# SCUT-CCNL/3DSIFT

Hardware: AMD Instinct MI355X
Metric: Mvoxels/s end-to-end KpSiftAlgorithm on 512^3 fp32 (higher is better)
Workload: dtype f32

## Files before the change

### 3dsift_amd/capi.py

```python
import ctypes as C
import os

import numpy as np

HERE = os.path.dirname(os.path.abspath(__file__))
LIB_PATH = os.environ.get("S3D_LIB") or os.path.join(HERE, "libsift3d_hip.so")
DESC = 768

KP_DTYPE = np.dtype(
    [
        ("x", "<f4"), ("y", "<f4"), ("z", "<f4"),
        ("scale", "<f4"),
        ("octave", "<i4"), ("level", "<i4"),
        ("rx", "<f4"), ("ry", "<f4"), ("rz", "<f4"),
        ("win", "<f4", (3,)),
        ("eigvalue", "<f4", (3,)),
        ("eigvector", "<f4", (9,)),
        ("Rotation", "<f4", (9,)),
        ("str_tensor", "<f4", (9,)),
    ]
)
assert KP_DTYPE.itemsize == 168

SYMBOLS = [
    "sift3d_default_params", "sift3d_create", "sift3d_destroy", "sift3d_run", "sift3d_run_async", "sift3d_run_async_after", "sift3d_wait", "sift3d_run_stages",
    "sift3d_stage_times", "sift3d_num_keypoints", "sift3d_get_keypoints", "sift3d_device_results",
    "sift3d_num_octaves", "sift3d_level_info", "sift3d_copy_level", "sift3d_copy_input", "sift3d_num_extrema",
    "sift3d_get_extrema", "sift3d_get_orientation_codes", "sift3d_gaussian_smooth", "sift3d_downsample", "sift3d_dog_sub", "sift3d_conv_axis",
    "sift3d_orient_keypoint", "sift3d_describe_keypoint", "sift3d_match",
    "sift3d_match_handles",
    "sift3d_default_detect_options", "sift3d_set_detect_options", "sift3d_get_detect_options", "sift3d_get_refined",
    "sift3d_default_ransac_options", "sift3d_fit_affine", "sift3d_fit_affine_local",
    "sift3d_fit_rigid", "sift3d_fit_rigid_local", "sift3d_fit_rotation",
    "sift3d_predict_positions", "sift3d_match_guided",
    "sift3d_default_icgn_options", "sift3d_icgn_init_from_fits", "sift3d_icgn",
    "sift3d_bspline_prefilter", "sift3d_icgn_bspline",
    "sift3d_icgn2_init_from_icgn", "sift3d_icgn2", "sift3d_strain_input_from_icgn2",
    "sift3d_default_search_options", "sift3d_zncc_search", "sift3d_icgn_init_from_search",
    "sift3d_default_strain_options", "sift3d_strain_input_from_icgn", "sift3d_strain",
    "sift3d_default_validate_options", "sift3d_validate_input_from_icgn", "sift3d_validate_input_from_icgn2", "sift3d_validate_displacements",
    "sift3d_validate_keep", "sift3d_icgn_init_from_validation", "sift3d_validate_stage_capacity",
    "sift3d_default_subset_options", "sift3d_subset_quality", "sift3d_subset_group_by_radius",
    "sift3d_icgn_masked", "sift3d_mask_from_level",
    "sift3d_device_count", "sift3d_error_string", "sift3d_last_error",
    "sift3d_dtype_bytes", "sift3d_create_typed", "sift3d_volume_to_device", "sift3d_test_ingest_launch",
    "sift3d_slab_min_halo", "sift3d_slab_arena_floats", "sift3d_slab_create", "sift3d_slab_buffer", "sift3d_slab_upload",
    "sift3d_slab_input_absmax", "sift3d_slab_input_scale", "sift3d_slab_level", "sift3d_slab_level_hw", "sift3d_slab_halo_planes",
    "sift3d_slab_sync", "sift3d_slab_get_dogmax", "sift3d_slab_set_dogmax", "sift3d_slab_detect", "sift3d_slab_describe",
    "sift3d_slab_decimate", "sift3d_slab_admits", "sift3d_slab_set_ghost", "sift3d_slab_min_halo_ghost", "sift3d_create_seeded", "sift3d_seed_upload", "sift3d_set_describe_partition",
    "sift3d_export_device", "sift3d_import_descriptors_device", "sift3d_run_partial_orientation",
    "sift3d_export_orientation_device", "sift3d_import_orientation_device", "sift3d_run_describe",
    "sift3d_set_stream", "sift3d_slab_export_dogmax_device", "sift3d_slab_import_dogmax_device", "sift3d_slab_decimate_async",
    "sift3d_slab_set_desc_partial", "sift3d_slab_min_halo_partial", "sift3d_slab_record_bytes", "sift3d_slab_desc_reach", "sift3d_slab_orient",
    "sift3d_slab_export_records", "sift3d_slab_describe_partial", "sift3d_slab_describe_finish", "sift3d_slab_orient_launch",
    "sift3d_slab_orient_count",
    "sift3d_slab_keypoints_launch", "sift3d_slab_keypoints_count", "sift3d_slab_describe_finish_launch", "sift3d_slab_describe_finish_count",
    "sift3d_seed_buffer", "sift3d_sharded_plan", "sift3d_slab_describe_launch", "sift3d_sharded_traffic",
    "sift3d_sharded_create", "sift3d_sharded_create_ex", "sift3d_sharded_run", "sift3d_sharded_num_keypoints", "sift3d_sharded_get_keypoints", "sift3d_sharded_info",
    "sift3d_sharded_error", "sift3d_sharded_destroy",
    "sift3d_test_hook", "sift3d_debug_counters", "sift3d_debug_face_lookup", "sift3d_match_times", "sift3d_debug_copy_bandwidth",
    "sift3d_match_warmup", "sift3d_test_staging_slice", "sift3d_test_slab_plan", "sift3d_test_sharded_time_rank",
]
HOOKS = {"dog_eager": 0, "glast_eager": 1, "det_serial": 2, "separable": 3, "desc_nocache": 4, "match_nodma": 5, "one_stream": 6,
         "desc_mass_shift": 7, "list_cap": 8, "peer_copy": 9, "desc_nosplit": 10, "march_tiles": 11, "desc_exact_cells": 12, "lazy_generic": 13, "sharded_fail_rank": 14,
         "ori_grid": 15}
ORIENT_WORDS = 34
DTYPES = {"float32": 0, "uint8": 1, "int8": 2, "uint16": 3, "int16": 4}
SHARDED_PARTIAL_WINDOWS = 1
SHARDED_WHOLE_WINDOWS = 2
SHARDED_COPY_TRANSPORT = 4
SHARDED_GHOST_OCTAVE0 = 8


class Params(C.Structure):
    _fields_ = [("num_kp_levels", C.c_int), ("sigma_default", C.c_float), ("sigma_n_default", C.c_float),
                ("peak_thresh", C.c_float), ("max_eig_thres", C.c_float), ("corner_thresh", C.c_float)]


class DetectOptions(C.Structure):
    _fields_ = [("neighbours", C.c_int), ("refine", C.c_int), ("max_offset", C.c_float), ("contrast_thresh", C.c_float),
                ("edge_ratio", C.c_float), ("reserved", C.c_int * 3)]


assert C.sizeof(DetectOptions) == 32

REFINED_DTYPE = np.dtype([("rx", "<f4"), ("ry", "<f4"), ("rz", "<f4"), ("scale", "<f4"), ("offset", "<f4", (4,)), ("contrast", "<f4")])
assert REFINED_DTYPE.itemsize == 36


class RansacOptions(C.Structure):
    _fields_ = [("iterations", C.c_int), ("inlier_thresh", C.c_float), ("seed", C.c_uint), ("refine", C.c_int), ("min_det", C.c_float),
                ("reserved", C.c_int * 3)]


assert C.sizeof(RansacOptions) == 32

FIT_DTYPE = np.dtype([("A", "<f8", (12,)), ("hyp", "<f8", (12,)), ("status", "<i4"), ("candidates", "<i4"), ("best_hypothesis", "<i4"),
                      ("best_count", "<i4"), ("inliers", "<i4"), ("rms", "<f4"), ("reserved", "<i4", (2,))])
assert FIT_DTYPE.itemsize == 224


class IcgnOptions(C.Structure):
    _fields_ = [("subset_radius", C.c_int), ("max_iterations", C.c_int), ("tolerance", C.c_float), ("interpolation", C.c_int),
                ("reserved", C.c_int * 4)]


assert C.sizeof(IcgnOptions) == 32

ICGN_DTYPE = np.dtype([("p", "<f8", (12,)), ("zncc", "<f8"), ("last_step", "<f8"), ("iterations", "<i4"), ("status", "<i4"),
                       ("reserved", "<i4", (2,))])
assert ICGN_DTYPE.itemsize == 128
ICGN2_DTYPE = np.dtype([("p", "<f8", (30,)), ("zncc", "<f8"), ("last_step", "<f8"), ("iterations", "<i4"), ("status", "<i4"),
                        ("reserved", "<i4", (2,))])
assert ICGN2_DTYPE.itemsize == 272


class SearchOptions(C.Structure):
    _fields_ = [("subset_radius", C.c_int), ("search_radius", C.c_int), ("reserved", C.c_int * 6)]


assert C.sizeof(SearchOptions) == 32

SEARCH_DTYPE = np.dtype([("d", "<i4", (3,)), ("status", "<i4"), ("zncc", "<f8"), ("zncc_second", "<f8"), ("candidates", "<i4"),
                         ("reserved", "<i4", (3,))])
assert SEARCH_DTYPE.itemsize == 48


class StrainOptions(C.Structure):
    _fields_ = [("radius", C.c_int), ("min_neighbours", C.c_int), ("measure", C.c_int), ("reserved", C.c_int * 5)]


assert C.sizeof(StrainOptions) == 32

STRAIN_DTYPE = np.dtype([("disp", "<f8", (3,)), ("G", "<f8", (9,)), ("E", "<f8", (6,)), ("principal", "<f8", (3,)), ("equivalent", "<f8"),
                         ("rms", "<f8"), ("neighbours", "<i4"), ("status", "<i4")])
assert STRAIN_DTYPE.itemsize == 192


class ValidateOptions(C.Structure):
    _fields_ = [("radius", C.c_int), ("min_neighbours", C.c_int), ("passes", C.c_int), ("reserved0", C.c_int), ("threshold", C.c_double),
                ("eps", C.c_double), ("reserved", C.c_int * 4)]


assert C.sizeof(ValidateOptions) == 48

VALIDATE_DTYPE = np.dtype([("median", "<f8", (3,)), ("mad", "<f8", (3,)), ("score", "<f8"), ("neighbours", "<i4"), ("status", "<i4"),
                           ("flagged", "<i4"), ("pass", "<i4")])
assert VALIDATE_DTYPE.itemsize == 72


class SubsetOptions(C.Structure):
    _fields_ = [("r_min", C.c_int), ("r_max", C.c_int), ("criterion", C.c_int), ("reserved0", C.c_int), ("threshold", C.c_double),
                ("level", C.c_double), ("fraction_min", C.c_double), ("reserved", C.c_int * 2)]


assert C.sizeof(SubsetOptions) == 48

SUBSET_DTYPE = np.dtype([("mean", "<f8"), ("dR", "<f8"), ("G", "<f8", (6,)), ("eig", "<f8", (3,)), ("radius", "<i4"), ("status", "<i4"),
                         ("feasible", "<i4"), ("material", "<i4")])
assert SUBSET_DTYPE.itemsize == 104


class SlabDesc(C.Structure):
    _fields_ = [("nx", C.c_int), ("ny", C.c_int), ("nz", C.c_int), ("z0", C.c_int), ("z1", C.c_int), ("halo", C.c_int),
                ("noct_total", C.c_int), ("octave", C.c_int)]


class Sift3dError(RuntimeError):
    pass


_lib = None
_fp = C.POINTER(C.c_float)
_ip = C.POINTER(C.c_int)


def lib():
    global _lib
    if _lib is None:
        if not os.path.exists(LIB_PATH):
            raise Sift3dError(f"{LIB_PATH} is missing: build it with `make -C 3dsift_amd/csrc` "
                              f"(or __graft_entry__.build()); there is no CPU fallback")
        try:
            import torch
        except ImportError:
            pass
        L = C.CDLL(LIB_PATH)
        L.sift3d_create.argtypes = [C.POINTER(C.c_void_p), C.c_void_p, C.c_int, C.c_int, C.c_int, C.POINTER(Params), C.c_int, C.c_int]
        L.sift3d_create_typed.argtypes = [C.POINTER(C.c_void_p), C.c_void_p, C.c_int, C.c_int, C.c_int, C.c_int, C.POINTER(Params), C.c_int, C.c_int]
        L.sift3d_dtype_bytes.argtypes = [C.c_int, _ip]
        L.sift3d_volume_to_device.argtypes = [C.c_void_p, C.c_int, C.c_int, C.c_int, C.c_int, C.c_int, C.c_int, C.c_void_p, C.POINTER(C.c_double)]
        L.sift3d_test_ingest_launch.argtypes = [C.c_int, _ip, _ip, _ip, _ip]
        L.sift3d_destroy.argtypes = [C.c_void_p]
        L.sift3d_run.argtypes = [C.c_void_p]
        L.sift3d_run_async.argtypes = [C.c_void_p]
        L.sift3d_wait.argtypes = [C.c_void_p]
        L.sift3d_run_stages.argtypes = [C.c_void_p, C.c_int]
        L.sift3d_stage_times.argtypes = [C.c_void_p, C.POINTER(C.c_double)]
        L.sift3d_num_keypoints.argtypes = [C.c_void_p, _ip]
        L.sift3d_get_keypoints.argtypes = [C.c_void_p, C.c_void_p, _fp]
        L.sift3d_device_results.argtypes = [C.c_void_p, C.POINTER(C.c_void_p), C.POINTER(C.c_void_p), _ip]
        L.sift3d_num_octaves.argtypes = [C.c_void_p, _ip]
        L.sift3d_level_info.argtypes = [C.c_void_p, C.c_int, C.c_int, _ip, _fp, _fp]
        L.sift3d_copy_level.argtypes = [C.c_void_p, C.c_int, C.c_int, _fp]
        L.sift3d_copy_input.argtypes = [C.c_void_p, _fp]
        L.sift3d_num_extrema.argtypes = [C.c_void_p, _ip]
        L.sift3d_get_extrema.argtypes = [C.c_void_p, C.c_void_p]
        L.sift3d_get_orientation_codes.argtypes = [C.c_void_p, _ip]
        L.sift3d_gaussian_smooth.argtypes = [_fp, C.c_int, C.c_int, C.c_int, C.c_float, _fp, C.c_int]
        L.sift3d_downsample.argtypes = [_fp, C.c_int, C.c_int, C.c_int, _fp, C.c_int, C.c_int, C.c_int, C.c_int]
        L.sift3d_dog_sub.argtypes = [_fp, _fp, C.c_size_t, _fp, C.c_int]
        L.sift3d_conv_axis.argtypes = [_fp, C.c_int, C.c_int, C.c_int, C.c_int, _fp, C.c_int, _fp, C.c_int]
        L.sift3d_orient_keypoint.argtypes = [_fp, C.c_int, C.c_int, C.c_int, C.c_float, C.c_void_p, C.c_float, C.c_float, C.c_float, C.c_int, _ip]
        L.sift3d_describe_keypoint.argtypes = [_fp, C.c_int, C.c_int, C.c_int, C.c_float, C.c_void_p, _fp, C.c_int]
        L.sift3d_match.argtypes = [C.c_void_p, C.c_void_p, C.c_int, C.c_void_p, C.c_void_p, C.c_int, C.c_double, C.c_int,
                                   C.c_int, C.c_int, _ip, _ip, _fp, _fp, _fp, _ip, C.POINTER(C.c_double)]
        L.sift3d_match_handles.argtypes = [C.c_void_p, C.c_void_p, C.c_double, C.c_int, _ip, _ip, _fp, _fp, _fp, _ip, C.POINTER(C.c_double)]
        L.sift3d_device_count.argtypes = [_ip]
        L.sift3d_default_detect_options.argtypes = [C.POINTER(DetectOptions)]
        L.sift3d_default_detect_options.restype = None
        L.sift3d_set_detect_options.argtypes = [C.c_void_p, C.POINTER(DetectOptions)]
        L.sift3d_get_detect_options.argtypes = [C.c_void_p, C.POINTER(DetectOptions)]
        L.sift3d_get_refined.argtypes = [C.c_void_p, C.c_void_p]
        L.sift3d_default_ransac_options.argtypes = [C.POINTER(RansacOptions)]
        L.sift3d_default_ransac_options.restype = None
        L.sift3d_fit_affine.argtypes = [C.c_void_p, C.c_int, C.POINTER(RansacOptions), C.c_int, C.c_int, C.c_void_p, C.c_void_p,
                                        C.POINTER(C.c_double)]
        L.sift3d_fit_affine_local.argtypes = [C.c_void_p, C.c_int, C.c_void_p, C.c_int, C.c_int, C.c_float, C.POINTER(RansacOptions), C.c_int,
                                              C.c_int, C.c_void_p, C.c_void_p, C.POINTER(C.c_double)]
        L.sift3d_fit_rigid.argtypes = [C.c_void_p, C.c_int, C.c_int, C.POINTER(RansacOptions), C.c_int, C.c_int, C.c_void_p, C.c_void_p,
                                       C.POINTER(C.c_double)]
        L.sift3d_fit_rigid_local.argtypes = [C.c_void_p, C.c_int, C.c_void_p, C.c_int, C.c_int, C.c_float, C.c_int, C.POINTER(RansacOptions),
                                             C.c_int, C.c_int, C.c_void_p, C.c_void_p, C.POINTER(C.c_double)]
        L.sift3d_fit_rotation.argtypes = [C.c_void_p, C.c_int, C.c_void_p, C.c_void_p, C.c_void_p]
        L.sift3d_predict_positions.argtypes = [C.c_void_p, C.c_int, C.c_void_p, C.c_int, C.c_void_p]
        L.sift3d_match_guided.argtypes = [C.c_void_p, C.c_void_p, C.c_int, C.c_void_p, C.c_void_p, C.c_int, C.c_void_p, C.c_float, C.c_double,
                                          C.c_int, C.c_int, C.c_int, _ip, _ip, _fp, _fp, _ip, _fp, _ip, C.POINTER(C.c_double)]
        L.sift3d_default_icgn_options.argtypes = [C.POINTER(IcgnOptions)]
        L.sift3d_default_icgn_options.restype = None
        L.sift3d_icgn_init_from_fits.argtypes = [C.c_void_p, C.c_void_p, C.c_int, C.c_void_p]
        L.sift3d_icgn.argtypes = [C.c_void_p, C.c_int, C.c_int, C.c_int, C.c_void_p, C.c_int, C.c_int, C.c_int, C.c_void_p, C.c_int, C.c_void_p,
                                  C.POINTER(IcgnOptions), C.c_int, C.c_int, C.c_void_p, C.POINTER(C.c_double)]
        L.sift3d_bspline_prefilter.argtypes = [C.c_void_p, C.c_int, C.c_int, C.c_int, C.c_void_p, C.c_int, C.c_int, C.POINTER(C.c_double)]
        L.sift3d_icgn_bspline.argtypes = [C.c_void_p, C.c_int, C.c_int, C.c_int, C.c_void_p, C.c_int, C.c_int, C.c_int, C.c_void_p, C.c_int,
                                          C.c_void_p, C.POINTER(IcgnOptions), C.c_int, C.c_int, C.c_int, C.c_void_p, C.POINTER(C.c_double)]
        L.sift3d_default_search_options.argtypes = [C.POINTER(SearchOptions)]
        L.sift3d_default_search_options.restype = None
        L.sift3d_zncc_search.argtypes = [C.c_void_p, C.c_int, C.c_int, C.c_int, C.c_void_p, C.c_int, C.c_int, C.c_int, C.c_void_p, C.c_int,
                                         C.c_void_p, C.POINTER(SearchOptions), C.c_int, C.c_int, C.c_void_p, C.POINTER(C.c_double)]
        L.sift3d_icgn2_init_from_icgn.argtypes = [C.c_void_p, C.c_int, C.c_void_p]
        L.sift3d_icgn2.argtypes = [C.c_void_p, C.c_int, C.c_int, C.c_int, C.c_void_p, C.c_int, C.c_int, C.c_int, C.c_void_p, C.c_int, C.c_void_p,
                                   C.POINTER(IcgnOptions), C.c_int, C.c_int, C.c_int, C.c_void_p, C.POINTER(C.c_double)]
        L.sift3d_strain_input_from_icgn2.argtypes = [C.c_void_p, C.c_int, C.c_double, C.c_int, C.c_void_p, C.c_void_p]
        L.sift3d_icgn_init_from_search.argtypes = [C.c_void_p, C.c_int, C.c_int, C.c_void_p]
        L.sift3d_default_strain_options.argtypes = [C.POINTER(StrainOptions)]
        L.sift3d_default_strain_options.restype = None
        L.sift3d_strain_input_from_icgn.argtypes = [C.c_void_p, C.c_int, C.c_double, C.c_int, C.c_void_p, C.c_void_p]
        L.sift3d_strain.argtypes = [C.c_void_p, C.c_void_p, C.c_void_p, C.c_int, C.POINTER(StrainOptions), C.c_int, C.c_int, C.c_void_p,
                                    C.POINTER(C.c_double)]
        L.sift3d_default_validate_options.argtypes = [C.POINTER(ValidateOptions)]
        L.sift3d_default_validate_options.restype = None
        L.sift3d_validate_input_from_icgn.argtypes = [C.c_void_p, C.c_int, C.c_double, C.c_int, C.c_void_p, C.c_void_p, C.c_void_p]
        L.sift3d_validate_input_from_icgn2.argtypes = [C.c_void_p, C.c_int, C.c_double, C.c_int, C.c_void_p, C.c_void_p, C.c_void_p]
        L.sift3d_validate_displacements.argtypes = [C.c_void_p, C.c_void_p, C.c_void_p, C.c_void_p, C.c_int, C.POINTER(ValidateOptions), C.c_int,
                                                    C.c_int, C.c_void_p, C.POINTER(C.c_double)]
        L.sift3d_validate_keep.argtypes = [C.c_void_p, C.c_void_p, C.c_int, C.c_void_p]
        L.sift3d_default_subset_options.argtypes = [C.POINTER(SubsetOptions)]
        L.sift3d_default_subset_options.restype = None
        L.sift3d_subset_quality.argtypes = [C.c_void_p, C.c_int, C.c_int, C.c_int, C.c_void_p, C.c_int, C.POINTER(SubsetOptions), C.c_int,
                                            C.c_int, C.c_void_p, C.POINTER(C.c_double)]
        L.sift3d_subset_group_by_radius.argtypes = [C.c_void_p, C.c_int, C.c_int, C.c_int, C.c_void_p, C.c_void_p, C.POINTER(C.c_int)]
        L.sift3d_icgn_init_from_validation.argtypes = [C.c_void_p, C.c_int, C.c_void_p, _ip]
        L.sift3d_icgn_masked.argtypes = [C.c_void_p, C.c_int, C.c_int, C.c_int, C.c_void_p, C.c_int, C.c_int, C.c_int, C.c_void_p, C.c_void_p,
                                         C.c_int, C.c_void_p, C.POINTER(IcgnOptions), C.c_float, C.c_int, C.c_int, C.c_int, C.c_void_p,
                                         C.c_void_p, C.POINTER(C.c_double)]
        L.sift3d_mask_from_level.argtypes = [C.c_void_p, C.c_int, C.c_int, C.c_int, C.c_double, C.c_void_p, C.c_int, C.c_int,
                                             C.POINTER(C.c_double)]
        L.sift3d_validate_stage_capacity.argtypes = [_ip]
        _sz = C.POINTER(C.c_size_t)
        L.sift3d_slab_min_halo.argtypes = [C.POINTER(Params), _ip]
        L.sift3d_slab_arena_floats.argtypes = [C.POINTER(SlabDesc), C.POINTER(Params), _sz]
        L.sift3d_slab_create.argtypes = [C.POINTER(C.c_void_p), C.POINTER(SlabDesc), C.POINTER(Params), C.c_int, C.c_void_p, C.c_size_t]
        L.sift3d_slab_buffer.argtypes = [C.c_void_p, C.c_int, C.c_int, _sz, _ip, _ip]
        L.sift3d_slab_upload.argtypes = [C.c_void_p, C.c_void_p, C.c_int, C.c_int, C.c_int]
        L.sift3d_slab_input_absmax.argtypes = [C.c_void_p, _fp]
        L.sift3d_slab_input_scale.argtypes = [C.c_void_p, C.c_float]
        L.sift3d_slab_level.argtypes = [C.c_void_p, C.c_int]
        L.sift3d_slab_halo_planes.argtypes = [C.c_void_p, C.c_int, _ip]
        L.sift3d_slab_level_hw.argtypes = [C.c_void_p, C.c_int, _ip]
        L.sift3d_slab_sync.argtypes = [C.c_void_p]
        L.sift3d_slab_get_dogmax.argtypes = [C.c_void_p, _fp]
        L.sift3d_slab_set_dogmax.argtypes = [C.c_void_p, _fp]
        L.sift3d_slab_detect.argtypes = [C.c_void_p]
        L.sift3d_slab_describe.argtypes = [C.c_void_p]
        L.sift3d_slab_set_desc_partial.argtypes = [C.c_void_p, C.c_int]
        L.sift3d_slab_min_halo_partial.argtypes = [C.POINTER(Params), _ip]
        L.sift3d_slab_record_bytes.argtypes = [_ip]
        L.sift3d_slab_desc_reach.argtypes = [C.c_void_p, _ip]
        L.sift3d_slab_orient.argtypes = [C.c_void_p]
        L.sift3d_slab_export_records.argtypes = [C.c_void_p, C.c_void_p]
        L.sift3d_slab_describe_partial.argtypes = [C.c_void_p, C.c_int, C.POINTER(C.c_void_p), _ip, C.POINTER(C.c_void_p), C.POINTER(C.c_void_p),
                                                   C.POINTER(C.c_void_p), _ip, _ip]
        L.sift3d_slab_describe_finish.argtypes = [C.c_void_p, C.c_void_p, C.c_int, C.c_int, C.POINTER(C.c_void_p), C.POINTER(C.c_void_p), C.c_void_p,
                                                  C.c_int, C.c_void_p, C.c_void_p, _ip]
        L.sift3d_slab_orient_launch.argtypes = [C.c_void_p]
        L.sift3d_slab_orient_count.argtypes = [C.c_void_p, _ip]
        L.sift3d_slab_decimate.argtypes = [C.c_void_p, C.c_void_p]
        L.sift3d_slab_decimate_async.argtypes = [C.c_void_p, C.c_void_p]
        L.sift3d_set_stream.argtypes = [C.c_void_p, C.c_void_p]
        L.sift3d_slab_export_dogmax_device.argtypes = [C.c_void_p, C.c_void_p]
        L.sift3d_slab_import_dogmax_device.argtypes = [C.c_void_p, C.c_void_p]
        L.sift3d_create_seeded.argtypes = [C.POINTER(C.c_void_p), C.c_int, C.c_int, C.c_int, C.c_int, C.c_int, C.POINTER(Params), C.c_int]
        L.sift3d_seed_upload.argtypes = [C.c_void_p, C.c_void_p, C.c_int]
        L.sift3d_set_describe_partition.argtypes = [C.c_void_p, C.c_int, C.c_int]
        L.sift3d_export_device.argtypes = [C.c_void_p, C.c_void_p, C.c_void_p]
        L.sift3d_run_partial_orientation.argtypes = [C.c_void_p]
        L.sift3d_export_orientation_device.argtypes = [C.c_void_p, C.c_void_p]
        L.sift3d_import_orientation_device.argtypes = [C.c_void_p, C.c_void_p]
        L.sift3d_run_describe.argtypes = [C.c_void_p]
        L.sift3d_import_descriptors_device.argtypes = [C.c_void_p, C.c_void_p]
        L.sift3d_sharded_create.argtypes = [C.POINTER(C.c_void_p), C.c_void_p, C.c_int, C.c_int, C.c_int, C.POINTER(Params), _ip, C.c_int, C.c_int, C.c_int]
        L.sift3d_sharded_create_ex.argtypes = [C.POINTER(C.c_void_p), C.c_void_p, C.c_int, C.c_int, C.c_int, C.POINTER(Params), _ip, C.c_int, C.c_int, C.c_int, C.c_uint]
        L.sift3d_sharded_run.argtypes = [C.c_void_p]
        L.sift3d_sharded_num_keypoints.argtypes = [C.c_void_p, _ip]
        L.sift3d_sharded_get_keypoints.argtypes = [C.c_void_p, C.c_void_p, _fp]
        L.sift3d_sharded_info.argtypes = [C.c_void_p, _ip, _ip, _ip, C.POINTER(C.c_double)]
        L.sift3d_sharded_error.argtypes = [C.c_void_p]
        L.sift3d_sharded_error.restype = C.c_char_p
        L.sift3d_sharded_destroy.argtypes = [C.c_void_p]
        L.sift3d_sharded_plan.argtypes = [C.c_void_p, _ip, _ip, _ip, _ip]
        L.sift3d_test_hook.argtypes = [C.c_int, C.c_int]
        L.sift3d_debug_counters.argtypes = [C.c_void_p, _ip]
        L.sift3d_debug_face_lookup.argtypes = [_fp, C.c_int, C.c_int, _ip, _fp, C.c_int]
        L.sift3d_debug_copy_bandwidth.argtypes = [C.c_size_t, C.c_int, C.c_int, C.POINTER(C.c_double)]
        L.sift3d_match_times.argtypes = [C.POINTER(C.c_double), C.POINTER(C.c_double)]
        L.sift3d_error_string.argtypes = [C.c_int]
        L.sift3d_error_string.restype = C.c_char_p
        L.sift3d_last_error.restype = C.c_char_p
        _lib = L
        for item in filter(None, os.environ.get("S3D_HOOKS", "").split(",")):
            k, _, v = item.partition("=")
            L.sift3d_test_hook(HOOKS[k.strip()], int(v or 1))
    return _lib


def _check(rc):
    if rc != 0:
        L = lib()
        raise Sift3dError(f"{L.sift3d_error_string(rc).decode()}: {L.sift3d_last_error().decode()}")


def _f(a):
    return a.ctypes.data_as(_fp)


def kernel_source_sha():
    import glob
    import hashlib
    h = hashlib.sha256()
    root = os.path.dirname(os.path.dirname(os.path.abspath(__file__)))
    files = sorted(glob.glob(os.path.join(root, "3dsift_amd", "csrc", "*.hip")) + glob.glob(os.path.join(root, "3dsift_amd", "csrc", "*.h")) +
                   glob.glob(os.path.join(root, "include", "*.h")))
    for f in files:
        h.update(os.path.basename(f).encode())
        h.update(open(f, "rb").read())
    return h.hexdigest()[:16]


class hook:

    def __init__(self, name, value):
        self.which, self.value = HOOKS[name], int(value)

    def __enter__(self):
        self.prev = lib().sift3d_test_hook(self.which, self.value)
        return self

    def __exit__(self, *exc):
        lib().sift3d_test_hook(self.which, self.prev)
        return False


def copy_bandwidth(nbytes=1 << 30, iters=5, device=0):
    g = C.c_double(0)
    _check(lib().sift3d_debug_copy_bandwidth(nbytes, iters, device, C.byref(g)))
    return g.value


def face_lookup(grad3, route=0, device=0):
    g = np.ascontiguousarray(grad3, np.float32).reshape(-1, 3)
    face = np.zeros(len(g), np.int32); bary = np.zeros((len(g), 3), np.float32)
    _check(lib().sift3d_debug_face_lookup(_f(g), len(g), int(route), face.ctypes.data_as(_ip), _f(bary), device))
    return face, bary


def default_detect_options():
    o = DetectOptions()
    lib().sift3d_default_detect_options(C.byref(o))
    return _options_dict(o)


def _options_dict(o):
    return {"neighbours": o.neighbours, "refine": bool(o.refine), "max_offset": o.max_offset, "contrast_thresh": o.contrast_thresh,
            "edge_ratio": o.edge_ratio}


def _options(cls, default_fn_name, names, what, opts):
    o = cls()
    getattr(lib(), default_fn_name)(C.byref(o))
    for k, v in opts.items():
        if k not in names:
            raise TypeError(f"unknown {what} option {k!r}")
        setattr(o, k, v)
    return o


RANSAC_OPTIONS = ("iterations", "inlier_thresh", "seed", "refine", "min_det")


def default_ransac_options():
    o = _ransac_options({})
    return {k: getattr(o, k) for k in RANSAC_OPTIONS}


def _ransac_options(opts):
    return _options(RansacOptions, "sift3d_default_ransac_options", RANSAC_OPTIONS, "RANSAC", opts)


def _is_dev(a):
    return hasattr(a, "data_ptr") and getattr(a, "is_cuda", False)


def _p(a):
    return C.c_void_p(a.ctypes.data)


def _table(a, dtype, width, like):
    if a is None:
        return None, 0, None
    shape = (-1, width) if width else (-1,)
    if _is_dev(like):
        import torch

        t = torch.as_tensor(a, dtype=getattr(torch, np.dtype(dtype).name), device=like.device).reshape(shape).contiguous()
        return C.c_void_p(t.data_ptr()), t.shape[0], t
    h = np.ascontiguousarray(a, dtype).reshape(shape)
    return _p(h), len(h), h


def _rows(a, width, name):
    if _is_dev(a):
        if str(a.dtype) != "torch.float32" or not a.is_contiguous() or (a.numel() and a.shape[-1] != width):
            raise ValueError(f"{name}: a contiguous float32 (n, {width}) device tensor is needed")
        return C.c_void_p(a.data_ptr()), a.numel() // width, a, 1
    h = np.ascontiguousarray(a, np.float32).reshape(-1, width)
    return _p(h), len(h), h, 0


def _volume(a, name, on_dev):
    if on_dev:
        if str(a.dtype) != "torch.float32" or not a.is_contiguous() or a.dim() != 3:
            raise ValueError(f"{name}: a contiguous float32 (nz, ny, nx) device tensor is needed")
        return C.c_void_p(a.data_ptr()), a
    h = np.ascontiguousarray(a, np.float32)
    if h.ndim != 3:
        raise ValueError(f"{name}: a (nz, ny, nx) volume is needed")
    return _p(h), h


def _dtype_code(dtype):
    if isinstance(dtype, (int, np.integer)):
        return int(dtype)
    name = str(dtype).replace("torch.", "")
    try:
        name = np.dtype(name).name
    except TypeError:
        pass
    if name not in DTYPES:
        raise ValueError(f"dtype {dtype}: one of {sorted(DTYPES)} is needed")
    return DTYPES[name]


def ingest_launch(dtype):
    v = [C.c_int(0) for _ in range(4)]
    _check(lib().sift3d_test_ingest_launch(_dtype_code(dtype), *[C.byref(x) for x in v]))
# ... 520 lines not shown

    def __init__(self, volume, num_kp_levels=3, sigma_default=1.6, sigma_n_default=1.15, peak_thresh=0.1,
                 max_eig_thres=0.9, corner_thresh=0.4, device=0, device_ptr=None, shape=None, keep_dtype=False, dtype=None):
        L = lib()
        self._h = C.c_void_p()
        p = Params(num_kp_levels, sigma_default, sigma_n_default, peak_thresh, max_eig_thres, corner_thresh)
        self.levels = num_kp_levels
        if device_ptr is not None:
            nz, ny, nx = shape
            self.shape = tuple(shape)
            if dtype is not None:
                _check(L.sift3d_create_typed(C.byref(self._h), C.c_void_p(device_ptr), _dtype_code(dtype), nx, ny, nz, C.byref(p), device, 1))
            else:
                _check(L.sift3d_create(C.byref(self._h), C.c_void_p(device_ptr), nx, ny, nz, C.byref(p), device, 1))
        elif keep_dtype and isinstance(volume, np.ndarray) and volume.dtype.name in DTYPES:
            vol = np.ascontiguousarray(volume)
            nz, ny, nx = vol.shape
            self.shape = vol.shape
            _check(L.sift3d_create_typed(C.byref(self._h), vol.ctypes.data_as(C.c_void_p), DTYPES[vol.dtype.name], nx, ny, nz, C.byref(p), device, 0))
        else:
            vol = np.ascontiguousarray(volume, dtype=np.float32)
            nz, ny, nx = vol.shape
            self.shape = vol.shape
            _check(L.sift3d_create(C.byref(self._h), vol.ctypes.data_as(C.c_void_p), nx, ny, nz, C.byref(p), device, 0))

    def set_stream(self, stream_handle):
        _check(lib().sift3d_set_stream(self._h, C.c_void_p(int(stream_handle or 0))))

    def close(self):
        if getattr(self, "_h", None) and self._h.value:
            lib().sift3d_destroy(self._h)
            self._h = C.c_void_p()

    def __del__(self):
        try:
            self.close()
        except Exception:
            pass

    def KpSiftAlgorithm(self):
        _check(lib().sift3d_run(self._h))
        return self

    def KpSiftAlgorithmAsync(self, after=None):
        if after is not None:
            _check(lib().sift3d_run_async_after(self._h, after._h))
        else:
            _check(lib().sift3d_run_async(self._h))
        return self

    def Wait(self):
        _check(lib().sift3d_wait(self._h))
        return self

    def run_stages(self, upto):
        _check(lib().sift3d_run_stages(self._h, int(upto)))
        return self

    def GetKeypoints(self, with_desc=True, out=None):
        n = C.c_int(0)
        _check(lib().sift3d_num_keypoints(self._h, C.byref(n)))
        if out is not None:
            kp, desc = out
            assert kp.dtype == KP_DTYPE and kp.shape == (n.value,) and desc.dtype == np.float32 and desc.shape == (n.value, DESC)
            assert kp.flags.c_contiguous and desc.flags.c_contiguous
        else:
            kp = np.zeros(n.value, KP_DTYPE)
            desc = np.zeros((n.value, DESC), np.float32)
        if n.value:
            _check(lib().sift3d_get_keypoints(self._h, kp.ctypes.data, _f(desc) if with_desc else None))
        return kp, desc

    @property
    def m_timer(self):
        t = (C.c_double * 8)()
        _check(lib().sift3d_stage_times(self._h, t))
        keys = ["d_TotalTime", "d_Allocation", "d_BuildGSS", "d_BuildDOG", "d_Detect", "d_AssignOrientation", "d_Extraction", "d_release"]
        return dict(zip(keys, list(t)))

    @property
    def num_octaves(self):
        n = C.c_int(0)
        _check(lib().sift3d_num_octaves(self._h, C.byref(n)))
        return n.value

    def level_info(self, is_dog, idx):
        d = np.zeros(3, np.int32); u = np.zeros(3, np.float32); s = np.zeros(1, np.float32)
        _check(lib().sift3d_level_info(self._h, int(is_dog), idx, d.ctypes.data_as(_ip), _f(u), _f(s)))
        return tuple(int(v) for v in d), tuple(float(v) for v in u), float(s[0])

    def level(self, is_dog, idx):
        (nx, ny, nz), _, _ = self.level_info(is_dog, idx)
        out = np.empty((nz, ny, nx), np.float32)
        _check(lib().sift3d_copy_level(self._h, int(is_dog), idx, _f(out)))
        return out

    def gss(self, octave, i):
        return self.level(0, octave * (self.levels + 3) + i)

    def dog(self, octave, i):
        return self.level(1, octave * (self.levels + 2) + i)

    def input(self):
        out = np.empty(self.shape, np.float32)
        _check(lib().sift3d_copy_input(self._h, _f(out)))
        return out

    def extrema(self):
        n = C.c_int(0)
        _check(lib().sift3d_num_extrema(self._h, C.byref(n)))
        out = np.zeros(n.value, KP_DTYPE)
        if n.value:
            _check(lib().sift3d_get_extrema(self._h, out.ctypes.data))
        return out

    def orientation_codes(self):
        n = C.c_int(0)
        _check(lib().sift3d_num_extrema(self._h, C.byref(n)))
        out = np.zeros(n.value, np.int32)
        if n.value:
            _check(lib().sift3d_get_orientation_codes(self._h, out.ctypes.data_as(_ip)))
        return out

    def device_results(self):
        d = C.c_void_p(); x = C.c_void_p(); n = C.c_int(0)
        _check(lib().sift3d_device_results(self._h, C.byref(d), C.byref(x), C.byref(n)))
        return d.value, x.value, n.value

    def export_device(self, desc_ptr, xyz_ptr=None):
        _check(lib().sift3d_export_device(self._h, C.c_void_p(int(desc_ptr)), C.c_void_p(int(xyz_ptr)) if xyz_ptr else None))

    def set_detect_options(self, neighbours=8, refine=False, max_offset=0.5, contrast_thresh=0.0, edge_ratio=0.0):
        o = DetectOptions(int(neighbours), int(refine), float(max_offset), float(contrast_thresh), float(edge_ratio))
        _check(lib().sift3d_set_detect_options(self._h, C.byref(o)))
        return self

    def detect_options(self):
        o = DetectOptions()
        _check(lib().sift3d_get_detect_options(self._h, C.byref(o)))
        return _options_dict(o)

    def refined(self):
        n = C.c_int(0)
        _check(lib().sift3d_num_keypoints(self._h, C.byref(n)))
        out = np.zeros(max(n.value, 1), REFINED_DTYPE)
        _check(lib().sift3d_get_refined(self._h, out.ctypes.data))
        return out[:n.value]

    def debug_counters(self):
        a = (C.c_int * 4)()
        _check(lib().sift3d_debug_counters(self._h, a))
        return {"list_regrows": a[0], "desc_second_passes": a[1], "match_exact_rows": a[2]}


def _params(kw):
    return Params(kw.get("num_kp_levels", 3), kw.get("sigma_default", 1.6), kw.get("sigma_n_default", 1.15),
                  kw.get("peak_thresh", 0.1), kw.get("max_eig_thres", 0.9), kw.get("corner_thresh", 0.4))


def slab_min_halo(**kw):
    p = _params(kw); h = C.c_int(0)
    _check(lib().sift3d_slab_min_halo(C.byref(p), C.byref(h)))
    return h.value


def slab_admits(nx, ny, nz, first_octave=True, **kw):
    p = _params(kw); ok = C.c_int(0)
    lib().sift3d_slab_admits.argtypes = [C.POINTER(Params), C.c_int, C.c_int, C.c_int, C.c_int, C.POINTER(C.c_int)]
    _check(lib().sift3d_slab_admits(C.byref(p), int(nx), int(ny), int(nz), int(bool(first_octave)), C.byref(ok)))
    return bool(ok.value)


def slab_min_halo_partial(**kw):
    p = _params(kw); h = C.c_int(0)
    _check(lib().sift3d_slab_min_halo_partial(C.byref(p), C.byref(h)))
    return h.value


def slab_record_words():
    n = C.c_int(0)
    _check(lib().sift3d_slab_record_bytes(C.byref(n)))
    assert n.value % 4 == 0
    return n.value // 4


class SeededCSIFT3D(CSIFT3D):

    def __init__(self, shape, octave_base, noct_total, device=0, **kw):
        self._h = C.c_void_p()
        p = _params(kw)
        self.levels = p.num_kp_levels
        self.shape = tuple(shape)
        nz, ny, nx = shape
        _check(lib().sift3d_create_seeded(C.byref(self._h), nx, ny, nz, octave_base, noct_total, C.byref(p), device))

    def seed(self, ptr, on_device=True):
        _check(lib().sift3d_seed_upload(self._h, C.c_void_p(int(ptr)), int(bool(on_device))))

    def seed_host(self, vol):
        vol = np.ascontiguousarray(vol, np.float32)
        _check(lib().sift3d_seed_upload(self._h, vol.ctypes.data_as(C.c_void_p), 0))

    def set_partition(self, rank, world):
        _check(lib().sift3d_set_describe_partition(self._h, rank, world))

    def run_partial_orientation(self):
        _check(lib().sift3d_run_partial_orientation(self._h))

    def export_orientation(self, ptr):
        _check(lib().sift3d_export_orientation_device(self._h, C.c_void_p(int(ptr))))

    def import_orientation(self, ptr):
        _check(lib().sift3d_import_orientation_device(self._h, C.c_void_p(int(ptr))))

    def run_describe(self):
        _check(lib().sift3d_run_describe(self._h))

    def num_extrema(self):
        n = C.c_int(0)
        _check(lib().sift3d_num_extrema(self._h, C.byref(n)))
        return n.value

    def import_descriptors(self, desc_ptr):
        _check(lib().sift3d_import_descriptors_device(self._h, C.c_void_p(int(desc_ptr))))


class SlabCSIFT3D(CSIFT3D):

    @staticmethod
    def arena_floats(nx, ny, nz, z0, z1, halo, noct_total, octave=0, **kw):
        d = SlabDesc(nx, ny, nz, z0, z1, halo, noct_total, octave); p = _params(kw); n = C.c_size_t(0)
        _check(lib().sift3d_slab_arena_floats(C.byref(d), C.byref(p), C.byref(n)))
        return n.value

    def __init__(self, nx, ny, nz, z0, z1, halo, noct_total, arena_ptr, arena_floats, device=0, octave=0, **kw):
        self._h = C.c_void_p()
        p = _params(kw)
        self.levels = p.num_kp_levels
        self.dims = (nx, ny, nz)
        self.z0, self.z1, self.halo = z0, z1, halo
        self.shape = (z1 - z0 + 2 * halo, ny, nx)
        self.octave = octave
        d = SlabDesc(nx, ny, nz, z0, z1, halo, noct_total, octave)
        _check(lib().sift3d_slab_create(C.byref(self._h), C.byref(d), C.byref(p), device, C.c_void_p(int(arena_ptr)), arena_floats))

    def buffer(self, kind, idx=0):
        off = C.c_size_t(0); pl = C.c_int(0); zo = C.c_int(0)
        _check(lib().sift3d_slab_buffer(self._h, kind, idx, C.byref(off), C.byref(pl), C.byref(zo)))
        return off.value, pl.value, zo.value

    def held_level(self, is_dog, idx):
        out = np.empty(self.shape, np.float32)
        _check(lib().sift3d_copy_level(self._h, int(is_dog), idx, _f(out)))
        return out

    def upload(self, planes, zg0, zg1, device_ptr=None):
        if device_ptr is not None:
            _check(lib().sift3d_slab_upload(self._h, C.c_void_p(int(device_ptr)), zg0, zg1, 1))
        else:
            a = np.ascontiguousarray(planes, np.float32)
            assert a.shape == (zg1 - zg0, self.dims[1], self.dims[0])
            _check(lib().sift3d_slab_upload(self._h, a.ctypes.data_as(C.c_void_p), zg0, zg1, 0))

    def input_absmax(self):
        m = C.c_float(0)
        _check(lib().sift3d_slab_input_absmax(self._h, C.byref(m)))
        return m.value

    def input_scale(self, gmax):
        _check(lib().sift3d_slab_input_scale(self._h, C.c_float(gmax)))

    def level_async(self, i):
        _check(lib().sift3d_slab_level(self._h, i))

    def level_hw(self, i):
        n = C.c_int(0)
        _check(lib().sift3d_slab_level_hw(self._h, i, C.byref(n)))
        return n.value

    def halo_planes(self, i):
        n = C.c_int(0)
        _check(lib().sift3d_slab_halo_planes(self._h, i, C.byref(n)))
        return n.value

    def sync(self):
        _check(lib().sift3d_slab_sync(self._h))

    def get_dogmax(self):
        a = np.zeros(8, np.float32)
        _check(lib().sift3d_slab_get_dogmax(self._h, _f(a)))
        return a[: self.levels + 2].copy()

    def set_dogmax(self, a):
        b = np.zeros(8, np.float32); b[: self.levels + 2] = a
        _check(lib().sift3d_slab_set_dogmax(self._h, _f(b)))

    def detect(self):
        _check(lib().sift3d_slab_detect(self._h))

    def describe(self):
        _check(lib().sift3d_slab_describe(self._h))

    def set_desc_partial(self, on=True):
        _check(lib().sift3d_slab_set_desc_partial(self._h, int(bool(on))))

    def desc_reach(self):
# ... 260 lines not shown
```

### 3dsift_amd/csrc/context.hip

```cpp
#include <float.h>
#include <math.h>
#include <stdlib.h>
#include <string.h>

#include <algorithm>
#include <atomic>
#include <mutex>
#include <thread>

#include "ctx_internal.h"

#pragma clang fp contract(off)

namespace s3d {

static thread_local std::string g_last_error;
void set_last_error(const std::string &s) { g_last_error = s; }

int set_device(int device) {
	int n = 0;
	if (hipGetDeviceCount(&n) != hipSuccess || n <= 0) {
		set_last_error("no HIP device visible: this library has no CPU fallback");
		return SIFT3D_ERR_NO_DEVICE;
	}
// ... 285 lines not shown
		}
		CHECKED(hipEventCreateWithFlags(&c->ev_seed[o], hipEventDisableTiming));
		CHECKED(hipEventCreateWithFlags(&c->ev_done[o], hipEventDisableTiming));
	}

	const size_t total = arena_floats_of(c);
	c->arena_floats = total;
	if (cfg.ext_arena) {
		if (cfg.ext_arena_floats < total) { set_last_error("caller arena too small"); sift3d_destroy(c); return SIFT3D_ERR_ARG; }
		c->arena = cfg.ext_arena;
		c->ext_arena = true;
	} else {
		CHECKED(hipMalloc(&c->arena, sizeof(float) * total));
	}
	float *p = c->arena;
	if (c->in_own) c->in.d = c->in_own;
	else { c->in.d = p; p += al64(c->in.n()); }
	c->tmpA.assign((size_t)std::max(1, c->noct), nullptr);
	c->tmpB.assign((size_t)std::max(1, c->noct), nullptr);
	for (int o = 0; o < c->noct && !c->slab; o++) {
		const size_t vo = al64(c->gss[(size_t)o * c->ng].n());
		c->tmpA[o] = p; p += vo;
		c->tmpB[o] = p; p += vo;
	}
	for (auto &L : c->gss) { L.d = p; p += al64(L.n()); }
	for (auto &L : c->dog) { L.d = p; p += al64(L.n()); }

	const size_t nwords = 1 + (size_t)std::max(1, c->noct * c->nd) + 8 + 1;
	CHECKED(hipMalloc(&c->d_words, sizeof(unsigned) * nwords));
	CHECKED(hipMemset(c->d_words, 0, sizeof(unsigned) * nwords));
	CHECKED(hipHostMalloc(&c->h_words, sizeof(unsigned) * 8, hipHostMallocDefault));
	CHECKED(hipMalloc(&c->d_slots_part, sizeof(unsigned) * slots_scratch_words()));
	c->d_inmax = c->d_words;
	c->d_dogmax = c->d_words + 1;
	c->d_total = c->d_words + 1 + std::max(1, c->noct * c->nd);
	c->d_nkp = c->d_total + 2;

	const int scan_planes = c->slab ? (c->own1 - c->own0) : cfg.nz;
	{
		const size_t kl = (size_t)c->p.num_kp_levels;
		const size_t words = kl * (size_t)scan_planes * cfg.ny * ((cfg.nx + 63) / 64);
		c->det_blocks = kl * (size_t)scan_planes * ((cfg.ny + 15) / 16);
		CHECKED(hipMalloc(&c->det.masks, sizeof(unsigned long long) * std::max<size_t>(words, 1)));
		CHECKED(hipMalloc(&c->det.block_counts, sizeof(unsigned) * std::max<size_t>(c->det_blocks, 1)));
		CHECKED(hipMalloc(&c->det.block_offsets, sizeof(unsigned) * std::max<size_t>(c->det_blocks, 1)));
	}
	c->det.total = c->d_total;
	{
		const bool det_serial = hook(SIFT3D_HOOK_DET_SERIAL) != 0;
		if (!c->slab && c->noct > 1 && !det_serial && c->ostream.size() > 1 && c->ostream[1] != c->stream) {
			const size_t kl = (size_t)c->p.num_kp_levels;
			c->det_o.assign((size_t)c->noct, DetectBufs{});
			size_t words = 0, blocks = 0;
			std::vector<size_t> woff((size_t)c->noct, 0), boff((size_t)c->noct, 0);
			for (int o = 1; o < c->noct; o++) {
				const Level &D = c->dog[(size_t)o * c->nd + 1];
				woff[(size_t)o] = words; boff[(size_t)o] = blocks;
				words += kl * (size_t)D.nz * D.ny * ((D.nx + 63) / 64);
				blocks += kl * (size_t)D.nz * ((D.ny + 15) / 16);
			}
			CHECKED(hipMalloc(&c->d_masks2, sizeof(unsigned long long) * std::max<size_t>(words, 1)));
			CHECKED(hipMalloc(&c->d_counts2, sizeof(unsigned) * std::max<size_t>(blocks, 1)));
			CHECKED(hipMalloc(&c->d_offsets2, sizeof(unsigned) * std::max<size_t>(blocks, 1)));
			for (int o = 1; o < c->noct; o++) {
				DetectBufs &b = c->det_o[(size_t)o];
				b.masks = c->d_masks2 + woff[(size_t)o]; b.block_counts = c->d_counts2 + boff[(size_t)o];
				b.block_offsets = c->d_offsets2 + boff[(size_t)o]; b.total = c->d_total;
			}
			CHECKED(hipEventCreateWithFlags(&c->ev_det_fork, hipEventDisableTiming));
			CHECKED(hipEventCreateWithFlags(&c->ev_det_join, hipEventDisableTiming));
			CHECKED(hipEventCreateWithFlags(&c->ev_det_fork2, hipEventDisableTiming));
			CHECKED(hipEventCreateWithFlags(&c->ev_det_join2, hipEventDisableTiming));
		}
	}

	std::vector<LevelRef> lr((size_t)std::max(1, c->noct + c->octave_base) * 8, LevelRef{nullptr, 0, 0, 0, 1.f, 0});
	for (int o = 0; o < c->noct; o++)
		for (int i = 0; i < c->ng && i < 8; i++) {
			const Level &L = c->gss[(size_t)o * c->ng + i];
			lr[(size_t)(o + c->octave_base) * 8 + i] = LevelRef{L.d, L.nx, L.ny, L.nz, L.unit, L.zoff};
		}
	CHECKED(hipMalloc(&c->d_levels, sizeof(LevelRef) * lr.size()));
	CHECKED(hipMemcpy(c->d_levels, lr.data(), sizeof(LevelRef) * lr.size(), hipMemcpyHostToDevice));
	rc = build_luts(c);
	if (rc) { sift3d_destroy(c); return rc; }
	FaceConst faces[kFaces];
	build_faces(faces);
	FaceSym sym;
	if (!build_facesym(faces, &sym)) { set_last_error("icosahedron symmetry table: no matching face"); sift3d_destroy(c); return SIFT3D_ERR_STATE; }
	CHECKED(upload_faces(faces, &sym));

	const size_t V0 = (size_t)cfg.nx * cfg.ny * scan_planes;
	unsigned cap = (unsigned)std::min<size_t>(std::max<size_t>(4096, V0 / 256), 4u << 20);
	if (hook(SIFT3D_HOOK_LIST_CAP) > 0) cap = (unsigned)hook(SIFT3D_HOOK_LIST_CAP);
	rc = alloc_lists(c, cap);
	if (rc) { sift3d_destroy(c); return rc; }
	CHECKED(hipStreamSynchronize(c->stream));
#undef CHECKED
	{
		static std::atomic<unsigned long long> loaded{0};
		const unsigned long long bit = 1ull << (device & 63);
		if (!(loaded.fetch_or(bit) & bit)) { preload_march_kernels(); preload_small_kernels(); preload_detect_kernels(); preload_orient_kernels(); preload_desc_kernels(); preload_match_kernels(); preload_ingest_kernels(); }
	}
	*out = c;
	return SIFT3D_OK;
}

int join_upload(sift3d_ctx *c) {
	if (c->uploader.joinable()) c->uploader.join();
	if (c->upload_rc != SIFT3D_OK) { set_last_error(c->upload_err); return c->upload_rc; }
	S3D_HIP(hipStreamSynchronize(c->up_stream));
	return SIFT3D_OK;
}

extern "C" int sift3d_create(sift3d_handle *out, const float *volume, int nx, int ny, int nz, const sift3d_params *params,
                             int device, int volume_on_device) {
	if (!out || !volume || nx <= 0 || ny <= 0 || nz <= 0) { set_last_error("sift3d_create: bad argument"); return SIFT3D_ERR_ARG; }
	if ((size_t)nx * ny * nz >= ((size_t)1 << 31)) { set_last_error("volume too large for int32 voxel indices"); return SIFT3D_ERR_ARG; }
	CreateCfg cfg;
	cfg.nx = nx; cfg.ny = ny; cfg.nz = nz;
	if (!volume_on_device) cfg.host_volume = volume;
	int rc = create_common(out, cfg, params, device);
	if (rc) return rc;
	sift3d_ctx *c = *out;
	const size_t V0 = (size_t)nx * ny * nz;
	hipError_t e = hipSuccess;
	if (volume_on_device) e = hipMemcpyAsync(c->in.d, volume, sizeof(float) * V0, hipMemcpyDeviceToDevice, c->stream);
	else if ((rc = join_upload(c)) != SIFT3D_OK) { sift3d_destroy(c); *out = nullptr; return rc; }
	if (e == hipSuccess) {
		unsigned *d_nonfinite = c->d_words + 1 + (size_t)std::max(1, c->noct * c->nd) + 8;
		launch_absmax(c->in.d, V0, c->d_inmax, c->stream, d_nonfinite);
		launch_scale_by_max(c->in.d, V0, c->d_inmax, c->stream);
		e = hipMemcpyAsync(&c->h_words[7], d_nonfinite, sizeof(unsigned), hipMemcpyDeviceToHost, c->stream);
		if (e == hipSuccess) e = hipStreamSynchronize(c->stream);
		if (e == hipSuccess && c->h_words[7] != 0) { c->nonfinite = true; c->use_fused = false; }
	}
	if (e == hipSuccess) e = hipGetLastError();
	if (e != hipSuccess) { set_last_error(hipGetErrorString(e)); sift3d_destroy(c); *out = nullptr; return SIFT3D_ERR_HIP; }
	return SIFT3D_OK;
}

#ifndef S3D_FUSED_MIN_DEFAULT
#define S3D_FUSED_MIN_DEFAULT 33
#endif
#ifndef S3D_FUSED_HALF
#define S3D_FUSED_HALF 1
#endif
#ifndef S3D_O0_TAIL_SLOTS_DEFAULT
#define S3D_O0_TAIL_SLOTS_DEFAULT 512
#endif
#ifndef S3D_BG_SLOTS_DEFAULT
#define S3D_BG_SLOTS_DEFAULT 256
#endif
static bool smooth_level(sift3d_ctx *c, int o, const float *src, const Level &dst, const Taps &t, const float *prev, float *dog,
                         unsigned *dogmax, int level = 0, const Level *half_out = nullptr, hipStream_t st_override = nullptr) {
	hipStream_t st = st_override ? st_override : c->ostream[o];
	static const int tail_slots = dev_tune_i("S3D_O0_TAIL_SLOTS", S3D_O0_TAIL_SLOTS_DEFAULT);
	static const int bg_slots = dev_tune_i("S3D_BG_SLOTS", S3D_BG_SLOTS_DEFAULT);
	static const int prio_mode = dev_tune_i("S3D_PRIO", 3);
	static const int bg1_slots = dev_tune_i("S3D_BG1_SLOTS", 0);
	const int prio = (prio_mode && c->noct > 1) ? (o >= 2 ? 2 : (o == 1 ? (prio_mode == 1 ? 1 : (prio_mode == 3 ? 2 : 0)) : 0)) : 0;
	const int plan_slots = c->noct > 1 ? (o == 0 ? (level > c->p.num_kp_levels ? tail_slots : 0) : (o == 1 && bg1_slots > 0 ? bg1_slots : bg_slots)) : 0;
	static const int fused_min = dev_tune_i("S3D_FUSED_MIN", S3D_FUSED_MIN_DEFAULT);
	if (c->use_fused && (prev == nullptr || prev == src) && std::min(dst.nx, dst.ny) >= fused_min) {
		MarchHalf hf;
		const bool want_half = S3D_FUSED_HALF && half_out != nullptr && march_half_ok(dst.nx, dst.ny, dst.zr_all());
		if (want_half) { hf.d = half_out->d; hf.nx = half_out->nx; hf.ny = half_out->ny; hf.nz = half_out->nz; }
		if (launch_march_level(src, dst.d, dog, dogmax, dst.nx, dst.ny, dst.zr_all(), t, st, plan_slots, prio, want_half ? &hf : nullptr))
			return want_half;
	}
	launch_conv_axis(0, src, c->tmpA[o], dst.nx, dst.ny, dst.nz, t, nullptr, nullptr, nullptr, st, c->nonfinite);
	launch_conv_axis(1, c->tmpA[o], c->tmpB[o], dst.nx, dst.ny, dst.nz, t, nullptr, nullptr, nullptr, st, c->nonfinite);
	launch_conv_axis(2, c->tmpB[o], dst.d, dst.nx, dst.ny, dst.nz, t, prev, dog, dogmax, st, c->nonfinite);
	return false;
}

void fill_detect_levels(const sift3d_ctx *c, int o, DetectLevels &DL) {
	memset(&DL, 0, sizeof(DL));
	const Level *G = &c->gss[(size_t)o * c->ng], *D = &c->dog[(size_t)o * c->nd];
	const int nl = c->nd - 2;
	for (int i = 1; i <= nl; i++) {
		DL.cur[i - 1] = D[i].d; DL.prev[i - 1] = D[i - 1].d; DL.next[i - 1] = D[i + 1].d;
		DL.absmax_bits[i - 1] = c->d_dogmax + (size_t)o * c->nd + i;
		DL.level_id[i - 1] = i;
		DL.scale[i - 1] = D[i].scale;
	}
	if (c->dog_elide) {
		DL.prev0_hi = G[1].d; DL.prev0_lo = G[0].d;
		DL.nextl_hi = G[c->nd].d; DL.nextl_lo = G[c->nd - 1].d;
		DL.nextl_slot = nl - 1;
		if (c->g_last_elide) { DL.nextl_hi = nullptr; DL.lazy_src = DL.nextl_lo; }
	}
}

static int run_prepare(sift3d_ctx *c, int &upto) {
	if (c->slab) { set_last_error("a z-slab context is driven stage by stage (sift3d_slab_*)"); return SIFT3D_ERR_STATE; }
	if (c->pending) { set_last_error("the handle has an asynchronous run in flight: call sift3d_wait first"); return SIFT3D_ERR_STATE; }
	int rc = set_device(c->device);
	if (rc) return rc;
	if (upto < 1) upto = 1;
	if (upto > 5) upto = 5;
	const bool dog_eager = hook(SIFT3D_HOOK_DOG_EAGER) != 0;
	c->dog_elide = !dog_eager && c->nd >= 3;
	const bool glast_eager = hook(SIFT3D_HOOK_GLAST_EAGER) != 0;
	c->g_last_elide = c->dog_elide && !glast_eager && c->use_fused && 2 * (2 * c->taps[c->ng - 1].hw + 1) <= kLazySlots;
	c->run_full = c->dopt.neighbours == 80 || c->dopt.refine != 0;
	c->run_refine = c->dopt.refine != 0;
	if (c->run_full) { c->dog_elide = false; c->g_last_elide = false; }
	c->g_last_built.assign((size_t)std::max(1, c->noct), 0);
	c->n_regrow = 0;
	return SIFT3D_OK;
}

static int run_enqueue(sift3d_ctx *c, int upto, bool part_orient) {
	int rc = set_device(c->device);
	if (rc) return rc;
	hipStream_t st = c->stream;
	if (c->run_refine && upto >= 4 && c->refined_cap < c->kp_cap) {
		hipFree(c->d_refined); c->d_refined = nullptr; c->refined_cap = 0;
		S3D_HIP(hipMalloc(&c->d_refined, sizeof(sift3d_refined) * (size_t)c->kp_cap));
		c->refined_cap = c->kp_cap;
	}
	if (c->dsplit_dirty && c->dsplit.gacc) {
		S3D_HIP(hipMemsetAsync(c->dsplit.gacc, 0, sizeof(int) * (size_t)c->dsplit.cap * (kDesc + 8 + 1), st));
		c->dsplit_dirty = false;
	}
	{
		if (c->gate) { S3D_HIP(hipStreamWaitEvent(st, c->gate, 0)); c->gate = nullptr; }
		S3D_HIP(hipMemsetAsync(c->d_dogmax, 0, sizeof(unsigned) * (size_t)(std::max(1, c->noct * c->nd) + 6), st));
		S3D_HIP(hipEventRecord(c->ev[0], st));
		S3D_HIP(hipEventRecord(c->ev_fork, st));
		std::vector<char> half_written((size_t)c->noct + 1, 0);
		int small_first = -1;
		SmallArgs sa;
		{
			static const int small_on = dev_tune_i("S3D_SMALL_OCT", 1);
			unsigned build_mask = 0, dog_mask = 0;
			int max_hw = 0;
			bool ok = small_on != 0 && c->use_fused && !c->slab && c->ng <= kSmallMaxLv;
			for (int i = 1; i < c->ng && ok; i++) {
				if (c->g_last_elide && i == c->ng - 1) continue;
				build_mask |= 1u << i;
				if (!(c->dog_elide && (i - 1 == 0 || i - 1 == c->nd - 1))) dog_mask |= 1u << (i - 1);
				const Taps &t = c->taps[i];
				for (int d = 1; d <= t.hw && ok; d++) ok = memcmp(&t.w[t.hw + d], &t.w[t.hw - d], sizeof(float)) == 0;
				max_hw = std::max(max_hw, t.hw);
			}
			if (ok && small_padded_hw(max_hw) > 0)
				for (int o = 0; o < c->noct; o++) {
					const Level &L = c->gss[(size_t)o * c->ng];
					if (c->noct - o <= kSmallMaxOct && small_octave_fits(L.nx, L.ny, L.nz, max_hw)) { small_first = o; break; }
				}
			for (int o = small_first; small_first >= 0 && o < c->noct; o++) {
				const Level &L = c->gss[(size_t)o * c->ng];
				if (!small_octave_fits(L.nx, L.ny, L.nz, max_hw)) small_first = -1;
			}
			if (small_first >= 0) {
				memset(&sa, 0, sizeof(sa));
				sa.noct = c->noct - small_first; sa.ng = c->ng; sa.nd = c->nd; sa.seed = c->p.num_kp_levels;
				sa.build_mask = build_mask; sa.dog_mask = dog_mask;
				sa.dogmax = c->d_dogmax + (size_t)small_first * c->nd;
				sa.hwp = small_padded_hw(max_hw);
				for (int i = 1; i < c->ng; i++) {
					const Taps &t = c->taps[i];
					if (t.hw > sa.hwp) continue;
					for (int k = 0; k <= sa.hwp; k++) sa.w[i][k] = k >= sa.hwp - t.hw ? t.w[k - (sa.hwp - t.hw)] : 0.0f;
				}
				for (int o = small_first; o < c->noct; o++) {
					SmallOct &so = sa.oct[o - small_first];
					const Level &L = c->gss[(size_t)o * c->ng];
					so.nx = L.nx; so.ny = L.ny; so.nz = L.nz;
					for (int i = 0; i < c->ng; i++) so.g[i] = c->gss[(size_t)o * c->ng + i].d;
					for (int i = 0; i < c->nd; i++) so.dog[i] = c->dog[(size_t)o * c->nd + i].d;
				}
			}
		}
		auto enqueue = [&](int o, bool head) -> int {
			static const int chain_mode = dev_tune_i("S3D_CHAIN", 1);
			const bool chain_on = chain_mode != 0;
			const bool chained = c->cstream != nullptr && chain_on && o >= 1 && (head || (small_first >= 0 && o >= small_first));
			hipStream_t so = chained ? c->cstream : c->ostream[(small_first >= 0 && o > small_first) ? small_first : o];
			const bool tail_moved = !head && small_first >= 3 && o == small_first - 1 && c->cstream == nullptr;
			if (tail_moved) so = c->ostream[o - 1];
			if (small_first >= 0 && o >= small_first) {
				if (head && o > 0) {
					S3D_HIP(hipStreamWaitEvent(so, c->ev_fork, 0));
					S3D_HIP(hipStreamWaitEvent(so, c->ev_seed[o - 1], 0));
				}
				if (head && o == small_first) {
					const Level &L = c->gss[(size_t)o * c->ng];
					if (o == 0) {
						if (!c->seeded) smooth_level(c, o, c->in.d, L, c->base_taps, nullptr, nullptr, nullptr);
					} else if (!half_written[(size_t)o]) {
						const Level &P = c->gss[(size_t)(o - 1) * c->ng + c->p.num_kp_levels];
						sa.parent = P.d; sa.pnx = P.nx; sa.pny = P.ny;
					}
					launch_small_octaves(sa, so);
				}
				if (head) S3D_HIP(hipEventRecord(c->ev_seed[o], so));
				if (!head && o > 0) S3D_HIP(hipEventRecord(c->ev_done[o], so));
				return SIFT3D_OK;
			}
			if (head && o > 0) {
				S3D_HIP(hipStreamWaitEvent(so, c->ev_fork, 0));
				S3D_HIP(hipStreamWaitEvent(so, c->ev_seed[o - 1], 0));
			}
			if (!head && o >= 1 && ((c->cstream != nullptr && chain_on) || tail_moved)) {
				S3D_HIP(hipStreamWaitEvent(so, c->ev_fork, 0));
				S3D_HIP(hipStreamWaitEvent(so, c->ev_seed[o], 0));
			}
			const int i0 = head ? 0 : c->p.num_kp_levels + 1, i1 = head ? c->p.num_kp_levels + 1 : c->ng;
			for (int i = i0; i < i1; i++) {
				const Level &L = c->gss[(size_t)o * c->ng + i];
				if (o == 0 && i == 0) {
					if (!c->seeded) smooth_level(c, o, c->in.d, L, c->base_taps, nullptr, nullptr, nullptr);
				} else if (i == 0) {
					const Level &P = c->gss[(size_t)(o - 1) * c->ng + c->p.num_kp_levels];
					if (!half_written[(size_t)o]) launch_downsample(P.d, P.nx, P.ny, L.d, L.nx, L.ny, L.nz, so);
				} else {
					const Level &P = c->gss[(size_t)o * c->ng + i - 1];
					const Level &D = c->dog[(size_t)o * c->nd + i - 1];
					if (c->g_last_elide && i == c->ng - 1) continue;
					const Level *half = (i == c->p.num_kp_levels && o + 1 < c->noct) ? &c->gss[(size_t)(o + 1) * c->ng] : nullptr;
					bool hw_ = false;
					if (c->dog_elide && (i - 1 == 0 || i - 1 == c->nd - 1)) hw_ = smooth_level(c, o, P.d, L, c->taps[i], nullptr, nullptr, nullptr, i, half, so);
					else hw_ = smooth_level(c, o, P.d, L, c->taps[i], P.d, D.d, c->d_dogmax + (size_t)o * c->nd + i - 1, i, half, so);
					if (half) half_written[(size_t)o + 1] = hw_ ? 1 : 0;
				}
				if (i == c->p.num_kp_levels) S3D_HIP(hipEventRecord(c->ev_seed[o], so));
			}
			if (!head && o > 0) S3D_HIP(hipEventRecord(c->ev_done[o], so));
			return SIFT3D_OK;
		};
		for (int o = 0; o <= c->noct; o++) {
			if (o < c->noct && (rc = enqueue(o, true)) != SIFT3D_OK) return rc;
			if (o >= 1 && (rc = enqueue(o - 1, false)) != SIFT3D_OK) return rc;
		}
		const bool two = upto >= 3 && c->det_o.size() > 1;
#ifndef S3D_DET_EARLY_DEFAULT
#define S3D_DET_EARLY_DEFAULT 1
#endif
		static const int det_early_mode = dev_tune_i("S3D_DET_EARLY", S3D_DET_EARLY_DEFAULT);
		const bool early = two && det_early_mode != 0 && c->noct > 1 && c->ostream.size() > 1 && c->ostream[1] != st;
		std::vector<DetectLevels> DLs((size_t)c->noct);
		const int nl = c->nd - 2;
		const Taps *lt = c->g_last_elide ? &c->taps[c->ng - 1] : nullptr;
		DetectOpts dopt;
		dopt.neighbours = c->dopt.neighbours; dopt.refine = c->dopt.refine;
		dopt.max_offset = c->dopt.max_offset; dopt.contrast_thresh = c->dopt.contrast_thresh; dopt.edge_ratio = c->dopt.edge_ratio;
		const DetectOpts *dop = c->run_full ? &dopt : nullptr;
		if (upto >= 3)
			for (int o = 0; o < c->noct; o++) fill_detect_levels(c, o, DLs[(size_t)o]);
		hipStream_t sb = two ? c->ostream[1] : st;
		if (early) {
			const Level &C0 = c->dog[(size_t)0 * c->nd + 1];
			S3D_HIP(hipEventRecord(c->ev_det_fork, st));
			launch_detect_mark(DLs[0], nl, C0.nx, C0.ny, C0.zr_all(), c->p.peak_thresh, 0 + c->octave_base, c->det, st, lt, dop);
			S3D_HIP(hipStreamWaitEvent(sb, c->ev_det_fork, 0));
			for (int o = 1; o < c->noct; o++) S3D_HIP(hipStreamWaitEvent(sb, c->ev_done[o], 0));
			S3D_HIP(hipEventRecord(c->ev[1], sb));
			S3D_HIP(hipEventRecord(c->ev[2], sb));
		} else {
			for (int o = 1; o < c->noct; o++) S3D_HIP(hipStreamWaitEvent(st, c->ev_done[o], 0));
			S3D_HIP(hipEventRecord(c->ev[1], st));
			S3D_HIP(hipEventRecord(c->ev[2], st));
		}
		if (upto >= 3) {
			if (two && !early) { S3D_HIP(hipEventRecord(c->ev_det_fork, st)); S3D_HIP(hipStreamWaitEvent(sb, c->ev_det_fork, 0)); }
			bool join2 = false;
			if (two) {
				hipStream_t sc = (c->noct > 2 && c->ostream.size() > 2 && c->ostream[2] != st && c->ostream[2] != sb) ? c->ostream[2] : sb;
				const bool own = early && sc != sb;
				if (sc != sb && !own) { S3D_HIP(hipEventRecord(c->ev_det_fork2, sb)); S3D_HIP(hipStreamWaitEvent(sc, c->ev_det_fork2, 0)); }
				for (int o = 1; o < c->noct; o++) {
					const Level &C = c->dog[(size_t)o * c->nd + 1];
					if (own && o >= 2) S3D_HIP(hipStreamWaitEvent(sc, c->ev_done[o], 0));
					launch_detect_mark(DLs[(size_t)o], nl, C.nx, C.ny, C.zr_all(), c->p.peak_thresh, o + c->octave_base, c->det_o[(size_t)o], o == 1 ? sb : sc, lt, dop);
				}
				S3D_HIP(hipEventRecord(c->ev_det_join, sb));
				join2 = sc != sb;
				if (join2) S3D_HIP(hipEventRecord(c->ev_det_join2, sc));
			}
			const bool all = two && c->noct <= 8;
			std::vector<DetectEmitItem> rest;
			for (int o = 0; o < c->noct; o++) {
				const Level &C = c->dog[(size_t)o * c->nd + 1];
				const DetectBufs &b = (two && o > 0) ? c->det_o[(size_t)o] : c->det;
				if (!(two && o > 0) && !(early && o == 0)) launch_detect_mark(DLs[(size_t)o], nl, C.nx, C.ny, C.zr_all(), c->p.peak_thresh, o + c->octave_base, b, st, lt, dop);
				if (two && o == 1) {
					S3D_HIP(hipStreamWaitEvent(st, c->ev_det_join, 0));
					if (join2) S3D_HIP(hipStreamWaitEvent(st, c->ev_det_join2, 0));
				}
				if (two && (o > 0 || all) && c->noct - 1 <= 8) rest.push_back(DetectEmitItem{&DLs[(size_t)o], nl, C.nx, C.ny, C.zr_all(), o + c->octave_base, &b});
				else launch_detect_emit(DLs[(size_t)o], nl, C.nx, C.ny, C.zr_all(), o + c->octave_base, b, c->d_ext, c->ext_cap, st);
			}
			if (!rest.empty()) launch_detect_emit_multi(rest.data(), (int)rest.size(), c->d_ext, c->ext_cap, c->d_total, st);
		}
		S3D_HIP(hipEventRecord(c->ev[3], st));
		if (upto >= 4) {
			launch_orient(c->d_ext, c->d_codes, c->d_total, c->ext_cap, c->d_levels, c->d_luts, c->d_lutpool, c->p.max_eig_thres,
			              c->p.corner_thresh, part_orient ? c->part_rank : 0, part_orient ? c->part_world : 1, c->d_order, c->d_nkp + 3, st);
			launch_slots(c->d_ext, c->d_codes, c->d_total, c->ext_cap, c->d_nkp, c->d_order, c->kp_cap, c->d_slots_part, st);
		}
		S3D_HIP(hipEventRecord(c->ev[4], st));
		if (upto >= 5) {
			launch_describe(c->d_ext, c->d_total, c->ext_cap, c->d_levels, c->d_luts, c->d_lutpool, c->d_desc, c->kp_cap, c->part_rank,
			                c->part_world, c->d_order, c->d_nkp, c->d_nkp + 1, st, c->desc_lut_lds, &c->dsplit);
		}
		if (upto >= 4) launch_finalize(c->d_ext, c->d_total, c->ext_cap, upto >= 5, c->d_kpout, c->d_xyz, c->kp_cap, st);
		if (upto >= 4 && c->run_refine) {
			DogTable T;
			memset(&T, 0, sizeof(T));
			T.octave_base = c->octave_base;
			for (int o = 0; o < c->noct && o < kDogTabOct; o++) {
				const Level &D0 = c->dog[(size_t)o * c->nd];
				T.nx[o] = D0.nx; T.ny[o] = D0.ny;
				for (int i = 0; i < c->nd && i < kDogTabLv; i++) T.d[o][i] = c->dog[(size_t)o * c->nd + i].d;
			}
			launch_refine(c->d_ext, c->d_total, c->ext_cap, c->kp_cap, T, c->p.num_kp_levels, c->d_refined, st);
		}
		S3D_HIP(hipEventRecord(c->ev[5], st));
		S3D_HIP(hipMemcpyAsync(c->h_words, c->d_total, sizeof(unsigned) * 5, hipMemcpyDeviceToHost, st));
	}
	return SIFT3D_OK;
}

static int run_finish(sift3d_ctx *c, int upto, bool &again) {
	again = false;
	int rc = set_device(c->device);
	if (rc) return rc;
	hipStream_t st = c->stream;
	{
		unsigned *host_words = c->h_words;
		S3D_HIP(hipStreamSynchronize(st));
		S3D_HIP(hipGetLastError());
		if (host_words[1] != 0 || host_words[0] > c->ext_cap) {
			const unsigned need = std::max(host_words[0], c->ext_cap) * 2u;
			rc = alloc_lists(c, need);
			if (rc) return rc;
			c->n_regrow++;
			again = true;
			return SIFT3D_OK;
		}
		c->n_ext = host_words[0];
		c->n_kp = upto >= 4 ? host_words[2] : 0;
		c->n_desc_redo = upto >= 5 ? (int)host_words[4] : 0;
		c->stage = upto;
		c->last_refine = c->run_refine && upto >= 4;
		float ms = 0;
		auto dt = [&](int a, int b) { hipEventElapsedTime(&ms, c->ev[a], c->ev[b]); return (double)ms * 1e-3; };
		c->times[0] = dt(0, 5); c->times[1] = 0; c->times[2] = dt(0, 1); c->times[3] = dt(1, 2);
		c->times[4] = dt(2, 3); c->times[5] = dt(3, 4); c->times[6] = dt(4, 5); c->times[7] = 0;
		return SIFT3D_OK;
	}
}

static int run_complete(sift3d_ctx *c, int upto, bool part_orient) {
	for (int attempt = 0; attempt < 8; attempt++) {
		bool again = false;
		int rc = run_finish(c, upto, again);
		if (rc) return rc;
		if (!again) return SIFT3D_OK;
		if ((rc = run_enqueue(c, upto, part_orient)) != SIFT3D_OK) return rc;
	}
	(void)hipStreamSynchronize(c->stream);
	set_last_error("extrema list kept overflowing");
	return SIFT3D_ERR_CAPACITY;
}

int run_impl(sift3d_ctx *c, int upto, bool part_orient) {
	int rc = run_prepare(c, upto);
	if (rc) return rc;
	if ((rc = run_enqueue(c, upto, part_orient)) == SIFT3D_OK) rc = run_complete(c, upto, part_orient);
	if (rc) c->dsplit_dirty = true;
	return rc;
}

extern "C" int sift3d_run(sift3d_handle c) {
	if (!c) return SIFT3D_ERR_ARG;
	return run_impl(c, 5);
}

// ... 24 lines not shown
	return rc;
}

extern "C" int sift3d_run_stages(sift3d_handle c, int upto) {
	if (!c) return SIFT3D_ERR_ARG;
	return run_impl(c, upto);
}

extern "C" int sift3d_stage_times(sift3d_handle c, double t[8]) {
	if (!c || !t) return SIFT3D_ERR_ARG;
	if (c->pending) { int wrc = sift3d_wait(c); if (wrc) return wrc; }
	if (c->stage < 1) return SIFT3D_ERR_STATE;
	memcpy(t, c->times, sizeof(double) * 8);
	return SIFT3D_OK;
}

extern "C" int sift3d_num_keypoints(sift3d_handle c, int *n) {
	if (!c || !n) return SIFT3D_ERR_ARG;
	if (c->pending) { int wrc = sift3d_wait(c); if (wrc) return wrc; }
	*n = (c->stage >= 4) ? (int)c->n_kp : 0;
	return SIFT3D_OK;
}

extern "C" int sift3d_get_keypoints(sift3d_handle c, sift3d_keypoint *out, float *desc) {
	if (!c) return SIFT3D_ERR_ARG;
	if (c->pending) { int wrc = sift3d_wait(c); if (wrc) return wrc; }
	if (c->stage < 4 || c->n_kp == 0) return SIFT3D_OK;
	int rc = set_device(c->device);
	if (rc) return rc;
	if (desc && c->stage < 5) return SIFT3D_ERR_STATE;
	D2HSeg sg[2];
	int ns = 0;
	if (out) sg[ns++] = D2HSeg{out, c->d_kpout, sizeof(sift3d_keypoint) * (size_t)c->n_kp};
	if (desc) sg[ns++] = D2HSeg{desc, c->d_desc, sizeof(float) * kDesc * (size_t)c->n_kp};
	return staged_d2h_v(sg, ns, c->device, c->own_stream);
}

extern "C" int sift3d_device_results(sift3d_handle c, const float **d_desc, const float **d_xyz, int *n) {
	if (!c) return SIFT3D_ERR_ARG;
	if (c->pending) { int wrc = sift3d_wait(c); if (wrc) return wrc; }
	if (c->stage < 5) return SIFT3D_ERR_STATE;
	if (d_desc) *d_desc = c->d_desc;
	if (d_xyz) *d_xyz = c->d_xyz;
	if (n) *n = (int)c->n_kp;
	return SIFT3D_OK;
}

extern "C" int sift3d_match_handles(sift3d_handle ref, sift3d_handle tar, double thresHold, int mode, int *gIdx, int *sIdx, float *gDist,
                                    float *sDist, float *pairs6, int *npairs, double *seconds) {
	if (!ref || !tar) return SIFT3D_ERR_ARG;
	int rc;
	if (ref->pending && (rc = sift3d_wait(ref)) != SIFT3D_OK) return rc;
	if (tar->pending && (rc = sift3d_wait(tar)) != SIFT3D_OK) return rc;
	if (ref->stage < 5 || tar->stage < 5) { set_last_error("sift3d_match_handles: both extractors must have run"); return SIFT3D_ERR_STATE; }
	const int n = (int)ref->n_kp, m = (int)tar->n_kp;
	const float *td = tar->d_desc, *tx = tar->d_xyz;
	if ((tar->device != ref->device || hook(SIFT3D_HOOK_PEER_COPY)) && m > 0) {
		if ((rc = set_device(ref->device)) != SIFT3D_OK) return rc;
		const size_t need = (size_t)m * (kDesc + 3);
		if (need > ref->peer_floats) {
			if (ref->d_peer) (void)hipFree(ref->d_peer);
			ref->d_peer = nullptr; ref->peer_floats = 0;
			S3D_HIP(hipMalloc(&ref->d_peer, sizeof(float) * (need + need / 4)));
			ref->peer_floats = need + need / 4;
		}
		S3D_HIP(hipMemcpyPeer(ref->d_peer, ref->device, tar->d_desc, tar->device, sizeof(float) * (size_t)m * kDesc));
		S3D_HIP(hipMemcpyPeer(ref->d_peer + (size_t)m * kDesc, ref->device, tar->d_xyz, tar->device, sizeof(float) * (size_t)m * 3));
		td = ref->d_peer; tx = ref->d_peer + (size_t)m * kDesc;
	}
	return sift3d_match(ref->d_desc, ref->d_xyz, n, td, tx, m, thresHold, mode, 1, ref->device, gIdx, sIdx, gDist, sDist, pairs6, npairs, seconds);
}

extern "C" int sift3d_set_detect_options(sift3d_handle c, const sift3d_detect_options *o) {
	if (!c || !o) { set_last_error("sift3d_set_detect_options: null argument"); return SIFT3D_ERR_ARG; }
	if (c->slab || c->seeded) { set_last_error("sift3d_set_detect_options: only plain single-volume handles (sift3d_create) take detection options"); return SIFT3D_ERR_ARG; }
	if (c->pending) { set_last_error("sift3d_set_detect_options: the handle has an asynchronous run in flight: call sift3d_wait first"); return SIFT3D_ERR_STATE; }
	if (o->neighbours != 8 && o->neighbours != 80) { set_last_error("sift3d_set_detect_options: neighbours must be 8 or 80"); return SIFT3D_ERR_ARG; }
	if (o->refine != 0 && o->refine != 1) { set_last_error("sift3d_set_detect_options: refine must be 0 or 1"); return SIFT3D_ERR_ARG; }
	if (!isfinite(o->max_offset) || !isfinite(o->contrast_thresh) || !isfinite(o->edge_ratio)) {
		set_last_error("sift3d_set_detect_options: thresholds must be finite");
		return SIFT3D_ERR_ARG;
	}
	if (o->reserved[0] || o->reserved[1] || o->reserved[2]) { set_last_error("sift3d_set_detect_options: reserved words must be 0"); return SIFT3D_ERR_ARG; }
	if (c->noct > kDogTabOct || c->nd > kDogTabLv) { set_last_error("sift3d_set_detect_options: too many octaves / levels for the refinement table"); return SIFT3D_ERR_ARG; }
	c->dopt = *o;
	return SIFT3D_OK;
}

extern "C" int sift3d_get_detect_options(sift3d_handle c, sift3d_detect_options *o) {
	if (!c || !o) return SIFT3D_ERR_ARG;
	*o = c->dopt;
	return SIFT3D_OK;
}

extern "C" int sift3d_get_refined(sift3d_handle c, sift3d_refined *out) {
	if (!c || !out) return SIFT3D_ERR_ARG;
	if (c->pending) { int wrc = sift3d_wait(c); if (wrc) return wrc; }
	if (!c->last_refine || c->stage < 4) { set_last_error("sift3d_get_refined: the last completed run did not refine its keypoints"); return SIFT3D_ERR_STATE; }
	if (c->n_kp == 0) return SIFT3D_OK;
	int rc = set_device(c->device);
	if (rc) return rc;
	return staged_d2h(out, c->d_refined, sizeof(sift3d_refined) * (size_t)c->n_kp, c->device, c->own_stream);
}

extern "C" int sift3d_num_octaves(sift3d_handle c, int *n) {
	if (!c || !n) return SIFT3D_ERR_ARG;
	*n = c->noct;
	return SIFT3D_OK;
}

static const Level *pick_level(sift3d_ctx *c, int is_dog, int idx) {
	const std::vector<Level> &P = is_dog ? c->dog : c->gss;
	if (idx < 0 || (size_t)idx >= P.size()) return nullptr;
	return &P[idx];
}

extern "C" int sift3d_level_info(sift3d_handle c, int is_dog, int idx, int dims3[3], float units3[3], float *scale) {
	if (!c) return SIFT3D_ERR_ARG;
	const Level *L = pick_level(c, is_dog, idx);
	if (!L) return SIFT3D_ERR_ARG;
	if (dims3) { dims3[0] = L->nx; dims3[1] = L->ny; dims3[2] = L->nz; }
	if (units3) units3[0] = units3[1] = units3[2] = L->unit;
	if (scale) *scale = L->scale;
	return SIFT3D_OK;
}

extern "C" int sift3d_copy_level(sift3d_handle c, int is_dog, int idx, float *out) {
	if (!c || !out) return SIFT3D_ERR_ARG;
	if (c->pending) { int wrc = sift3d_wait(c); if (wrc) return wrc; }
	if (c->stage < 1) return SIFT3D_ERR_STATE;
	const Level *L = pick_level(c, is_dog, idx);
	if (!L) return SIFT3D_ERR_ARG;
	int rc = set_device(c->device);
	if (rc) return rc;
	if (c->g_last_elide && c->slab) {
		const int i = is_dog ? idx % c->nd : idx % c->ng;
		if (((is_dog && i == c->nd - 1) || (!is_dog && i == c->ng - 1)) && (c->g_last_built.empty() || !c->g_last_built[0])) {
			const Level &G = c->gss[c->ng - 1];
			if (!launch_march_level(c->gss[c->ng - 2].d, G.d, nullptr, nullptr, G.nx, G.ny, G.zr(c->own0 - G.zoff, c->own1 - G.zoff), c->taps[c->ng - 1],
			                        c->stream)) return SIFT3D_ERR_STATE;
			S3D_HIP(hipStreamSynchronize(c->stream));
			c->g_last_built.assign(1, 1);
		}
	}
	if (c->g_last_elide && !c->slab) {
		const int o = is_dog ? idx / c->nd : idx / c->ng, i = is_dog ? idx % c->nd : idx % c->ng;
		if (((is_dog && i == c->nd - 1) || (!is_dog && i == c->ng - 1)) && !c->g_last_built[(size_t)o]) {
			const Level &G = c->gss[(size_t)o * c->ng + c->ng - 1], &P = c->gss[(size_t)o * c->ng + c->ng - 2];
			smooth_level(c, o, P.d, G, c->taps[c->ng - 1], nullptr, nullptr, nullptr, c->ng - 1);
			S3D_HIP(hipStreamSynchronize(c->ostream[o]));
			c->g_last_built[(size_t)o] = 1;
		}
	}
	if (is_dog && c->dog_elide && (idx % c->nd == 0 || idx % c->nd == c->nd - 1)) {
		const int o = idx / c->nd, i = idx % c->nd;
		launch_dog_from_gss(c->gss[(size_t)o * c->ng + i + 1].d, c->gss[(size_t)o * c->ng + i].d, L->d, L->n(), c->stream);
		S3D_HIP(hipStreamSynchronize(c->stream));
	}
	return staged_d2h(out, L->d, sizeof(float) * L->n(), c->device, c->own_stream);
}

extern "C" int sift3d_copy_input(sift3d_handle c, float *out) {
	if (!c || !out) return SIFT3D_ERR_ARG;
	int rc = set_device(c->device);
	if (rc) return rc;
	return staged_d2h(out, c->in.d, sizeof(float) * c->in.n(), c->device, c->own_stream);
}

extern "C" int sift3d_num_extrema(sift3d_handle c, int *n) {
	if (!c || !n) return SIFT3D_ERR_ARG;
	if (c->pending) { int wrc = sift3d_wait(c); if (wrc) return wrc; }
	*n = c->stage >= 3 ? (int)c->n_ext : 0;
	return SIFT3D_OK;
}

static int fetch_ext(sift3d_ctx *c, std::vector<DevKp> &h) {
	int rc = set_device(c->device);
	if (rc) return rc;
	h.resize(c->n_ext);
	if (c->n_ext) S3D_HIP(hipMemcpy(h.data(), c->d_ext, sizeof(DevKp) * (size_t)c->n_ext, hipMemcpyDeviceToHost));
	return SIFT3D_OK;
}

extern "C" int sift3d_get_extrema(sift3d_handle c, sift3d_keypoint *out) {
	if (!c || !out) return SIFT3D_ERR_ARG;
	if (c->pending) { int wrc = sift3d_wait(c); if (wrc) return wrc; }
	if (c->stage < 3) return SIFT3D_ERR_STATE;
	std::vector<DevKp> h;
	int rc = fetch_ext(c, h);
	if (rc) return rc;
	for (size_t i = 0; i < h.size(); i++) {
		sift3d_keypoint &o = out[i];
		memset(&o, 0, sizeof(o));
		o.x = (float)h[i].x; o.y = (float)h[i].y; o.z = (float)h[i].z;
		o.scale = h[i].scale; o.octave = h[i].octave; o.level = h[i].level;
		o.rx = o.ry = o.rz = -1.0f;
		memcpy(o.win, h[i].win, sizeof(o.win));
		memcpy(o.eigvalue, h[i].eigvalue, sizeof(o.eigvalue));
		memcpy(o.eigvector, h[i].eigvector, sizeof(o.eigvector));
		memcpy(o.Rotation, h[i].rot, sizeof(o.Rotation));
		memcpy(o.str_tensor, h[i].st, sizeof(o.str_tensor));
	}
	return SIFT3D_OK;
}

extern "C" int sift3d_get_orientation_codes(sift3d_handle c, int *codes) {
	if (!c || !codes) return SIFT3D_ERR_ARG;
	if (c->pending) { int wrc = sift3d_wait(c); if (wrc) return wrc; }
	if (c->stage < 4) return SIFT3D_ERR_STATE;
	std::vector<DevKp> h;
	int rc = fetch_ext(c, h);
	if (rc) return rc;
	for (size_t i = 0; i < h.size(); i++) codes[i] = h[i].code;
	return SIFT3D_OK;
}

}
```

### 3dsift_amd/csrc/ctx_internal.h

```cpp
#pragma once

#include <string>
#include <thread>
#include <vector>

#include "sift3d_internal.h"

using s3d::DescSplit; using s3d::DetectBufs; using s3d::DevKp; using s3d::Level; using s3d::LevelRef; using s3d::Taps; using s3d::WinLut;


struct sift3d_ctx {
	int device = 0;
	hipStream_t stream = nullptr;
	hipStream_t own_stream = nullptr;
	sift3d_params p{};
	int nx = 0, ny = 0, nz = 0;
	int noct = 0, ng = 0, nd = 0;
	int octave_base = 0;
	bool seeded = false;
	bool slab = false;
	int own0 = 0, own1 = 0, halo = 0;
	bool dog_elide = false;
	bool g_last_elide = false;
	std::vector<char> g_last_built;
	unsigned *d_prov = nullptr;
	bool desc_lut_lds = true;
	bool ext_arena = false;
	int part_rank = 0, part_world = 1;

	float *arena = nullptr;
	float *in_own = nullptr;
	void *in_raw = nullptr;
	hipStream_t up_stream = nullptr;
	std::thread uploader;
	int upload_rc = SIFT3D_OK;
	std::string upload_err;
	size_t arena_floats = 0;
	Level in;
	std::vector<Level> gss, dog;
	std::vector<float *> tmpA, tmpB;
	std::vector<hipStream_t> ostream;
	hipStream_t cstream = nullptr;
	std::vector<hipEvent_t> ev_seed, ev_done;
	hipEvent_t ev_fork = nullptr;
	unsigned *d_words = nullptr;
	unsigned *d_slots_part = nullptr;
	unsigned *h_words = nullptr;
	unsigned *d_inmax = nullptr, *d_dogmax = nullptr, *d_total = nullptr, *d_nkp = nullptr;
	DetectBufs det{};
	size_t det_blocks = 0;
	std::vector<DetectBufs> det_o;
	unsigned long long *d_masks2 = nullptr;
	unsigned *d_counts2 = nullptr, *d_offsets2 = nullptr, *d_prov2 = nullptr;
	hipEvent_t ev_det_fork = nullptr, ev_det_join = nullptr, ev_det_fork2 = nullptr, ev_det_join2 = nullptr;
	DevKp *d_ext = nullptr;
	int *d_codes = nullptr, *d_order = nullptr;
	unsigned ext_cap = 0, kp_cap = 0;
	LevelRef *d_levels = nullptr;
	WinLut *d_luts = nullptr;
	float *d_lutpool = nullptr;
	sift3d_keypoint *d_kpout = nullptr;
	float *d_desc = nullptr, *d_xyz = nullptr;
	DescSplit dsplit{};
	bool ghost = false;
	bool desc_partial = false;
	bool dsplit_dirty = false;
	float *d_peer = nullptr;
	size_t peer_floats = 0;

	std::vector<Taps> taps;
	Taps base_taps{};

	sift3d_detect_options dopt{};
	bool run_full = false, run_refine = false, last_refine = false;
	sift3d_refined *d_refined = nullptr;
	unsigned refined_cap = 0;

	bool nonfinite = false;
	bool use_fused = true;
	int n_regrow = 0, n_desc_redo = 0;

	int stage = 0;
	bool pending = false;
	hipEvent_t gate = nullptr;
	unsigned n_ext = 0, n_kp = 0;
	hipEvent_t ev[8] = {};
	double times[8] = {};
};

struct CreateCfg {
	int nx = 0, ny = 0, nz = 0;
	int octave_base = 0;
	int noct_total = -1;
	bool seeded = false;
	bool slab = false;
	int z0 = 0, z1 = 0, halo = 0;
	const void *host_volume = nullptr;
	int host_dtype = SIFT3D_DT_F32;
	float *ext_arena = nullptr;
	size_t ext_arena_floats = 0;
};

namespace s3d {
bool build_taps(float sigma, Taps &t);
void level_sigmas(const sift3d_params &p, std::vector<float> &sig, float &base_sigma);
void build_faces(FaceConst *F);
bool build_facesym(const FaceConst *F, FaceSym *S);
bool append_lut(std::vector<float> &pool, WinLut &L, int which, float sigma, float radius, float u, float scale);
int set_device(int device);
int alloc_lists(sift3d_ctx *c, unsigned ext_cap);
float level_scale(const sift3d_params &p, int octave, int s);
void plan_pyramid(sift3d_ctx *c, int noct_total);
void fill_detect_levels(const sift3d_ctx *c, int o, DetectLevels &DL);
int upload_luts(sift3d_ctx *c, const std::vector<WinLut> &luts, std::vector<float> &pool);
std::vector<WinLut> blank_luts(const sift3d_ctx *c);
size_t arena_floats_of(const sift3d_ctx *c);
int create_common(sift3d_handle *out, const CreateCfg &cfg, const sift3d_params *params, int device);
int join_upload(sift3d_ctx *c);
int run_impl(sift3d_ctx *c, int upto, bool part_orient = false);
}
```

### 3dsift_amd/csrc/kernels_detect.hip

```cpp
#include <stdio.h>
#include <string.h>
#include <stdlib.h>

#include <algorithm>

#include "sift3d_internal.h"

namespace s3d {

#ifndef S3D_DET_ROWS
#define S3D_DET_ROWS 32
#endif
#ifndef S3D_DET_QUEUE
#define S3D_DET_QUEUE 640
#endif
#ifndef S3D_DETDIAG
#define S3D_DETDIAG 0
#endif
#ifndef S3D_DET_LEAN
#define S3D_DET_LEAN 1
#endif
#ifndef S3D_DET_XPRE
#define S3D_DET_XPRE 0
#endif
// ... 45 lines not shown
		const bool in_q = lane < n;
		const int e = first + (in_q ? lane : 0);
		const uint2 qe = q[e];
		const float v = __uint_as_float(qe.x);
		const unsigned id = qe.y;
		const int rr = (int)((id >> 12) & 15), xw = (int)((id >> 6) & 63), bit = (int)(id & 63);
		static_assert(kRows / 4 <= 16, "four bits for the row of a wave");
		const int xq = (seg0 + xw) * 64 + bit;
		const bool act = in_q && xq >= 1 && xq <= nx - 2;
		const size_t i = plane0 + sy * (size_t)(r_lo + rr) + (size_t)xq;
		const size_t ic = act ? i : sz * (size_t)z + sy + 1;
		const float n0 = lazy_prev ? (L.prev0_hi[ic] - L.prev0_lo[ic]) * (-1.0f) : prev[ic];
		const bool pre = lean;
		const bool dmax = (id >> 16) & 1u;
		float n1 = 0.f, n2 = 0.f, n3 = 0.f, n4 = 0.f;
		if (!pre) { n1 = cur[ic - 1]; n2 = cur[ic + 1]; n3 = cur[ic + sy]; n4 = cur[ic - sy]; }
		const float n5 = cur[ic + sz], n6 = cur[ic - sz];
		if (lazy_g) {
			const bool mn7 = pre ? (!dmax && v < n0 && v < n5 && v < n6) : (v < n0 && v < n1 && v < n2 && v < n3 && v < n4 && v < n5 && v < n6);
			const bool mx7 = pre ? (dmax && v > n0 && v > n5 && v > n6) : (v > n0 && v > n1 && v > n2 && v > n3 && v > n4 && v > n5 && v > n6);
			const bool park = act && (mn7 || mx7);
			const unsigned long long pm = __ballot(park);
			if (pm) {
				unsigned base = 0;
				if (lane == 0) base = atomicAdd(prov_count, (unsigned)__popcll(pm));
				base = (unsigned)__builtin_amdgcn_readfirstlane((int)base);
				if (park) {
					const unsigned slot = base + (unsigned)__popcll(pm & lt);
					if (slot < prov_cap) prov[slot] = (unsigned)i | (mx7 ? 0x80000000u : 0u);
					else total[1] = 1u;
				}
			}
			return;
		}
		const float n7 = lazy_next ? (L.nextl_hi[ic] - L.nextl_lo[ic]) * (-1.0f) : next[ic];
		const bool mn = pre ? (!dmax && v < n0 && v < n5 && v < n6 && v < n7) : (v < n0 && v < n1 && v < n2 && v < n3 && v < n4 && v < n5 && v < n6 && v < n7);
		const bool mx = pre ? (dmax && v > n0 && v > n5 && v > n6 && v > n7) : (v > n0 && v > n1 && v > n2 && v > n3 && v > n4 && v > n5 && v > n6 && v > n7);
		if (act && (mn || mx)) atomicOr(&mloc[rr * segw + xw], 1ull << bit);
	};
	unsigned cnt = 0;
	for (int seg0 = 0; seg0 < wpr; seg0 += 64) {
		const int seg1 = min(wpr, seg0 + 64);
		if (lean && z_in) {
			const int ry_a = max(r_lo, 1 - y0), ry_b = min(r_hi, ny - 1 - y0);
			const int nws = seg1 - seg0;
			const float *__restrict__ pl = cur + sz * (size_t)z + (size_t)seg0 * 64;
			auto word = [&](float v, float u, float d, float xl, float xr, int wseg, unsigned idrow) {
				const float hi = fmaxf(fmaxf(u, d), fmaxf(xl, xr)), lo = fminf(fminf(u, d), fminf(xl, xr));
				const bool gmax = v > hi;
				const bool c = fabsf(v) > thr && (gmax || v < lo) && !((S3D_DETDIAG & 2) && v != 12345.678f);
				const unsigned long long m = __ballot(c);
				if (c) {
					const unsigned pos = __builtin_amdgcn_mbcnt_hi((unsigned)(m >> 32), __builtin_amdgcn_mbcnt_lo((unsigned)m, (unsigned)qn));
					q[pos] = make_uint2(__float_as_uint(v), idrow | (gmax ? 0x10000u : 0u) | (unsigned)(wseg << 6) | (unsigned)lane);
				}
				qn += (int)__popcll(m);
			};
			const unsigned omax = (unsigned)(nx - 1 - seg0 * 64);
			for (int w0 = 0; w0 < nws && ry_a < ry_b; w0 += kBatch) {
				unsigned off[kBatch];
#pragma unroll
				for (int bb = 0; bb < kBatch; bb++) off[bb] = min((unsigned)(min(w0 + bb, nws - 1) * 64 + lane), omax);
				const int eoff = (lane & 1) ? (int)min((unsigned)((w0 + kBatch) * 64), omax) : w0 * 64 - 1;
				float up[kBatch], mid[kBatch], emid;
				{
					const float *ra = pl + sy * (size_t)(y0 + ry_a - 1), *rb = ra + sy;
#pragma unroll
					for (int bb = 0; bb < kBatch; bb++) { up[bb] = ra[off[bb]]; mid[bb] = rb[off[bb]]; }
					emid = rb[eoff];
				}
				for (int ry = ry_a; ry < ry_b; ry++) {
					const float *rd = pl + sy * (size_t)(y0 + ry + 1);
					float dn[kBatch], xl[kBatch], xr[kBatch];
#pragma unroll
					for (int bb = 0; bb < kBatch; bb++) dn[bb] = rd[off[bb]];
					const float edn = rd[eoff];
#pragma unroll
					for (int bb = 0; bb < kBatch; bb++) {
						const int le = __builtin_amdgcn_readlane(__float_as_int(bb == 0 ? emid : mid[bb > 0 ? bb - 1 : 0]), bb == 0 ? 0 : 63);
						const int re = __builtin_amdgcn_readlane(__float_as_int(bb == kBatch - 1 ? emid : mid[bb < kBatch - 1 ? bb + 1 : 0]), bb == kBatch - 1 ? 1 : 0);
						xl[bb] = __int_as_float(__builtin_amdgcn_update_dpp(le, __float_as_int(mid[bb]), 0x138 , 0xf, 0xf, false));
						xr[bb] = __int_as_float(__builtin_amdgcn_update_dpp(re, __float_as_int(mid[bb]), 0x130 , 0xf, 0xf, false));
					}
					const unsigned idrow = (unsigned)((ry - r_lo) << 12);
#pragma unroll
					for (int bb = 0; bb < kBatch; bb++)
						if (w0 + bb < nws) word(mid[bb], up[bb], dn[bb], xl[bb], xr[bb], w0 + bb, idrow);
					while (qn >= 64) {
						qn -= 64;
						evaluate(qn, 64, seg0);
					}
#pragma unroll
					for (int bb = 0; bb < kBatch; bb++) { up[bb] = mid[bb]; mid[bb] = dn[bb]; }
					emid = edn;
				}
			}
		}
		for (int ry = r_lo; !lean && ry < r_hi; ry++) {
			const int y = y0 + ry;
			const bool y_in = z_in && y >= 1 && y <= ny - 2;
			const size_t rowbase = sy * (size_t)y + sz * (size_t)z;
			for (int xw0 = seg0; xw0 < seg1; xw0 += kBatch) {
				float val[kBatch], vxm[kBatch], vxp[kBatch];
				bool in[kBatch];
#pragma unroll
				for (int bb = 0; bb < kBatch; bb++) {
					const int x = (xw0 + bb) * 64 + lane;
					in[bb] = y_in && xw0 + bb < seg1 && x >= 1 && x <= nx - 2;
					const float *a = cur + (in[bb] ? rowbase + (size_t)x : sz * (size_t)z + 1);
					val[bb] = a[0];
					if (S3D_DET_XPRE) { vxm[bb] = a[-1]; vxp[bb] = a[1]; }
				}
#pragma unroll
				for (int bb = 0; bb < kBatch; bb++) {
					const float v = val[bb];
					const bool xext = !S3D_DET_XPRE || (((int)(v > vxm[bb]) & (int)(v > vxp[bb])) | ((int)(v < vxm[bb]) & (int)(v < vxp[bb]))) != 0;
					const bool c = in[bb] && (v > thr || v < -thr) && xext && !((S3D_DETDIAG & 2) && v != 12345.678f);
					const unsigned long long m = __ballot(c);
					if (c) {
						const int pos = qn + (int)__popcll(m & lt);
						q[pos] = make_uint2(__float_as_uint(v), (unsigned)(((ry - r_lo) << 12) | ((xw0 + bb - seg0) << 6) | lane));
					}
					qn += (int)__popcll(m);
					if (kQueue < 63 + kBatch * 64 && qn >= 64) {
						qn -= 64;
						evaluate(qn, 64, seg0);
					}
				}
				while (qn >= 64) {
					qn -= 64;
					evaluate(qn, 64, seg0);
				}
			}
		}
		if (qn > 0) evaluate(0, qn, seg0);
		qn = 0;
		for (int ry = r_lo; ry < r_hi; ry++) {
			unsigned long long *mrow = masks + ((size_t)(lvl * nz + zi) * ny + (y0 + ry)) * wpr;
			for (int xw = seg0 + lane; xw < seg1; xw += 64) {
				const unsigned long long m = mloc[(ry - r_lo) * segw + xw - seg0];
				mrow[xw] = m;
				cnt += (unsigned)__popcll(m);
				mloc[(ry - r_lo) * segw + xw - seg0] = 0ull;
			}
		}
	}
#pragma unroll
	for (int o = 32; o > 0; o >>= 1) cnt += __shfl_xor(cnt, o, 64);
	if (lane == 0) s_cnt[wid] = cnt;
	__syncthreads();
	if (threadIdx.x == 0) block_counts[b] = s_cnt[0] + s_cnt[1] + s_cnt[2] + s_cnt[3];
}

__device__ __forceinline__ void lazy_tap_src(int p, int d, int n, int &lo, int &hi, float &frac, bool interior) {
	if (interior) { lo = hi = p - d; frac = 0.0f; return; }
	const int dim_end = n - 1;
	float c = (float)p - (float)d * 1.0f;
	if (c < 0.0f) c = -1.0f * c;
	else if (c >= (float)dim_end) c = (float)(2 * dim_end) - c - 0.1f;
	lo = (int)c;
	frac = c - (float)lo;
	hi = lo + 1;
	lo = min(max(lo, 0), dim_end);
	hi = min(max(hi, 0), dim_end);
}
static_assert(kLazySlots / 2 - 1 == 25, "k_lazy_next's wide instantiation covers kLazySlots");
constexpr int kLwN = 17, kLwPieces = kLwN * kLwN * 5, kLwInstr = (kLwPieces + 63) / 64, kLwFloats = kLwInstr * 256, kLwWaves = 2;
__global__ void __launch_bounds__(64 * kLwWaves) k_lazy_wave(DetectLevels L, Taps t, int nx, int ny, ZRange zr, int nyb,
                                                            const unsigned *__restrict__ prov, const unsigned *__restrict__ prov_count,
                                                            unsigned prov_cap, unsigned long long *__restrict__ masks,
                                                            unsigned *__restrict__ block_counts) {
	__shared__ __attribute__((aligned(1024))) float s_buf[kLwWaves][kLwFloats];
	constexpr int H = 8, N = kLwN;
	const int lane = threadIdx.x & 63, wid = __builtin_amdgcn_readfirstlane((int)(threadIdx.x >> 6));
	float *blk = s_buf[wid];
	const unsigned lds_base = (unsigned)(size_t)blk;
	const unsigned count = min(*prov_count, prov_cap);
	const int lvl = L.nextl_slot;
	const float *__restrict__ src = L.lazy_src;
	const float *__restrict__ cur = L.cur[lvl];
	const int wpr = (nx + 63) >> 6, nzs = zr.zo1 - zr.zo0, nzg = zr.nzg;
	const size_t sy = (size_t)nx, sz = (size_t)nx * ny;
	unsigned voff[kLwInstr];
#pragma unroll
	for (int j = 0; j < kLwInstr; j++) {
		const int p = min(64 * j + lane, kLwPieces - 1), row = p / 5, q = p - 5 * row, zi = row / N, yi = row - zi * N;
		voff[j] = (unsigned)(((size_t)zi * sz + (size_t)yi * sy + (size_t)(4 * q)) * sizeof(float));
	}
	const unsigned nwaves = gridDim.x * kLwWaves;
	for (unsigned e = blockIdx.x * kLwWaves + (unsigned)wid; e < count; e += nwaves) {
		const unsigned ent = prov[e];
		const size_t ic = (size_t)(ent & 0x7FFFFFFFu);
		const bool as_max = (ent >> 31) != 0;
		const int zl = (int)(ic / sz), rem = (int)(ic - (size_t)zl * sz), y = rem / nx, x = rem - y * nx;
		const int zg = zl + zr.zoff;
		if (!(x >= H && x <= nx - 2 - H && y >= H && y <= ny - 2 - H && zg >= H && zg <= nzg - 2 - H)) continue;
		const int shift = min(max(0, x + 11 - (nx - 1)), x - H);
		const float *base = src + ic - (size_t)H * sz - (size_t)H * sy - (size_t)(H + shift);
#pragma unroll
		for (int j = 0; j < kLwInstr; j++) {
			unsigned keep;
			asm volatile("s_mov_b32 %0, m0\n\ts_mov_b32 m0, %3\n\ts_nop 0\n\tglobal_load_lds_dwordx4 %1, %2\n\ts_mov_b32 m0, %0"
			             : "=&s"(keep) : "v"(voff[j]), "s"(base), "s"(lds_base + 1024u * (unsigned)j) : "memory");
		}
		const float centre = src[ic], v = cur[ic];
		asm volatile("s_waitcnt vmcnt(0)" ::: "memory");
		__builtin_amdgcn_wave_barrier();
#pragma unroll
		for (int rq = 0; rq < (N * N + 63) / 64; rq++) {
			const int row = min(lane + 64 * rq, N * N - 1);
			const float *r = blk + row * 20 + shift;
			float acc = 0.0f;
#pragma unroll
			for (int k = 0; k < N; k++) acc = acc + t.w[k] * r[2 * H - k];
			if (lane + 64 * rq < N * N) blk[row * 20] = acc;
		}
		__builtin_amdgcn_fence(__ATOMIC_RELEASE, "wavefront");
		__builtin_amdgcn_wave_barrier();
		__builtin_amdgcn_fence(__ATOMIC_ACQUIRE, "wavefront");
		{
			const int pl = min(lane, N - 1);
			const float *c = blk + pl * N * 20;
			float acc = 0.0f;
#pragma unroll
			for (int k = 0; k < N; k++) acc = acc + t.w[k] * c[(2 * H - k) * 20];
			__builtin_amdgcn_fence(__ATOMIC_RELEASE, "wavefront");
			__builtin_amdgcn_wave_barrier();
			if (lane < N) blk[pl * N * 20] = acc;
		}
		__builtin_amdgcn_fence(__ATOMIC_RELEASE, "wavefront");
		__builtin_amdgcn_wave_barrier();
		__builtin_amdgcn_fence(__ATOMIC_ACQUIRE, "wavefront");
		{
			float acc = 0.0f;
#pragma unroll
			for (int k = 0; k < N; k++) acc = acc + t.w[k] * blk[(2 * H - k) * N * 20];
			const float n7 = (acc - centre) * (-1.0f);
			if (lane == 0 && (as_max ? (v > n7) : (v < n7))) {
				const int zi = zl - zr.zo0;
				atomicOr(&masks[((size_t)(lvl * nzs + zi) * ny + y) * wpr + (x >> 6)], 1ull << (x & 63));
				atomicAdd(&block_counts[(lvl * nzs + zi) * nyb + y / kRows], 1u);
			}
		}
		__builtin_amdgcn_fence(__ATOMIC_RELEASE, "wavefront");
		__builtin_amdgcn_wave_barrier();
	}
}

template <int kLT>
__global__ void __launch_bounds__(256) k_lazy_next(DetectLevels L, Taps t, int nx, int ny, ZRange zr, int nyb,
                                                   const unsigned *__restrict__ prov, const unsigned *__restrict__ prov_count,
                                                   unsigned prov_cap, unsigned long long *__restrict__ masks,
                                                   unsigned *__restrict__ block_counts, int skip_interior) {
	constexpr int kLR = kLT + 1;
	constexpr int kLP = kLR + 1;
	__shared__ float s_blk[kLR * kLR * kLP];
	__shared__ float s_x[kLR * kLR];
	__shared__ float s_y[kLR];
	__shared__ float s_w[kMaxTaps];
	__shared__ int s_lo[3][kLT], s_hi[3][kLT];
	__shared__ float s_fr[3][kLT];
	__shared__ int s_rng[6];
	const int hw = t.hw, nt = 2 * hw + 1, tid = threadIdx.x;
	for (int i = tid; i < nt; i += 256) s_w[i] = t.w[i];
	const unsigned count = min(*prov_count, prov_cap);
	const int lvl = L.nextl_slot;
	const float *__restrict__ src = L.lazy_src;
	const float *__restrict__ cur = L.cur[lvl];
	const int wpr = (nx + 63) >> 6, nzs = zr.zo1 - zr.zo0, nzg = zr.nzg;
	const size_t sy = (size_t)nx, sz = (size_t)nx * ny;
	__shared__ unsigned s_list[256];
	__shared__ unsigned s_nlist;
	for (unsigned e0 = blockIdx.x; e0 < count; e0 += 256 * gridDim.x) {
	__syncthreads();
	if (tid == 0) s_nlist = 0u;
	__syncthreads();
	if (e0 + (unsigned)tid * gridDim.x < count) {
		const unsigned ent = prov[e0 + (unsigned)tid * gridDim.x];
		const size_t ic = (size_t)(ent & 0x7FFFFFFFu);
		const int zl = (int)(ic / sz), rem = (int)(ic - (size_t)zl * sz), y = rem / nx, x = rem - y * nx;
		const int zg = zl + zr.zoff;
		const bool inner = x >= hw && x <= nx - 2 - hw && y >= hw && y <= ny - 2 - hw && zg >= hw && zg <= nzg - 2 - hw;
		if (!(skip_interior && inner)) s_list[atomicAdd(&s_nlist, 1u)] = ent;
	}
	__syncthreads();
	const unsigned nlist = s_nlist;
	for (unsigned li = 0; li < nlist; li++) {
		const unsigned ent = s_list[li];
		const size_t ic = (size_t)(ent & 0x7FFFFFFFu);
		const bool as_max = (ent >> 31) != 0;
		const int zl = (int)(ic / sz), rem = (int)(ic - (size_t)zl * sz), y = rem / nx, x = rem - y * nx;
		const int zg = zl + zr.zoff;
		const bool ix = x >= hw && x <= nx - 2 - hw, iy = y >= hw && y <= ny - 2 - hw, iz = zg >= hw && zg <= nzg - 2 - hw;
		__syncthreads();
		if (tid < 3 * nt) {
			const int ax = tid / nt, k = tid - ax * nt;
			int lo, hi; float fr;
			if (ax == 0) lazy_tap_src(x, k - hw, nx, lo, hi, fr, ix);
			else if (ax == 1) lazy_tap_src(y, k - hw, ny, lo, hi, fr, iy);
			else lazy_tap_src(zg, k - hw, nzg, lo, hi, fr, iz);
			s_lo[ax][k] = lo; s_hi[ax][k] = hi; s_fr[ax][k] = fr;
		}
		__syncthreads();
		if (tid < 3) {
			int mn = 1 << 30, mxv = -1;
			for (int k = 0; k < nt; k++) { mn = min(mn, s_lo[tid][k]); mxv = max(mxv, s_hi[tid][k]); }
// ... 84 lines not shown
		for (unsigned q = 0; q < 8; q++)
			if (q * 4 < chunk) {
				const uint4 c4 = *reinterpret_cast<const uint4 *>(block_counts + lo + 4 * q);
				cnt[4 * q] = c4.x; cnt[4 * q + 1] = c4.y; cnt[4 * q + 2] = c4.z; cnt[4 * q + 3] = c4.w;
				sum += c4.x + c4.y + c4.z + c4.w;
			}
	} else {
		for (unsigned i = lo; i < hi; i++) sum += block_counts[i];
	}
	unsigned v = sum;
	const int lane = t & 63, wid = t >> 6;
#pragma unroll
	for (int o = 1; o < 64; o <<= 1) {
		unsigned u = __shfl_up(v, o, 64);
		if (lane >= o) v += u;
	}
	if (lane == 63) s_wave[wid] = v;
	__syncthreads();
	if (t == 0) {
		unsigned a = 0;
		for (int w = 0; w < 16; w++) { unsigned c = s_wave[w]; s_wave[w] = a; a += c; }
	}
	__syncthreads();
	const unsigned incl = v + s_wave[wid];
	unsigned run = base + (incl - sum);
	if (vec) {
#pragma unroll
		for (unsigned q = 0; q < 8; q++)
			if (q * 4 < chunk) {
				uint4 o4;
				o4.x = run; run += cnt[4 * q]; o4.y = run; run += cnt[4 * q + 1]; o4.z = run; run += cnt[4 * q + 2]; o4.w = run; run += cnt[4 * q + 3];
				*reinterpret_cast<uint4 *>(block_offsets + lo + 4 * q) = o4;
			}
	} else {
		for (unsigned i = lo; i < hi; i++) { block_offsets[i] = run; run += block_counts[i]; }
	}
	__syncthreads();
	if (t == 1023) s_wave[0] = base + incl;
	__syncthreads();
	const unsigned nbase = s_wave[0];
	__syncthreads();
	return nbase;
}

__global__ void __launch_bounds__(1024) k_scan(const unsigned *__restrict__ block_counts, unsigned *__restrict__ block_offsets,
                                               unsigned nblocks, unsigned *__restrict__ total) {
	__shared__ unsigned s_wave[16];
	const unsigned nb = scan_octave(block_counts, block_offsets, nblocks, total[0], s_wave);
	if (threadIdx.x == 0) total[0] = nb;
}

struct EmitOct {
	const unsigned long long *masks;
	const unsigned *counts;
	unsigned *offsets;
	int nx, ny, nyb, octave;
	ZRange zr;
	unsigned nblocks, block0;
	int level_id[kMaxKpLevels];
	float scale[kMaxKpLevels];
};
struct EmitMulti { EmitOct o[8]; int n; };
__global__ void __launch_bounds__(1024) k_scan_multi(EmitMulti M, unsigned *__restrict__ total) {
	__shared__ unsigned s_wave[16];
	unsigned base = total[0];
	__syncthreads();
	for (int k = 0; k < M.n; k++) base = scan_octave(M.o[k].counts, M.o[k].offsets, M.o[k].nblocks, base, s_wave);
	if (threadIdx.x == 0) total[0] = base;
}

__device__ __forceinline__ void emit_block(int b, const unsigned long long *__restrict__ masks, const unsigned *__restrict__ block_offsets, int nx,
                                           int ny, const ZRange &zr, int nyb, int octave, const int *level_id, const float *scale,
                                           DevKp *__restrict__ out, unsigned cap, unsigned *__restrict__ total, unsigned *s_wave) {
	const int nz = zr.zo1 - zr.zo0;
	const int yb = b % nyb, zi = (b / nyb) % nz, lvl = b / (nyb * nz);
	const int z = zr.zo0 + zi + zr.zoff;
	const int wpr = (nx + 63) >> 6;
	const int y0 = yb * kRows;
	const int nwords = min(kRows, ny - y0) * wpr;
	const int lane = threadIdx.x & 63, wid = threadIdx.x >> 6;
	unsigned running = block_offsets[b];
	for (int w0 = 0; w0 < nwords; w0 += kThreads) {
		const int wi = w0 + threadIdx.x;
		unsigned long long m = 0;
		int y = 0, xw = 0;
		if (wi < nwords) {
			const int ry = wi / wpr;
			xw = wi - ry * wpr;
			y = y0 + ry;
			m = masks[((size_t)(lvl * nz + zi) * ny + y) * wpr + xw];
		}
		const unsigned c = (unsigned)__popcll(m);
		unsigned v = c;
#pragma unroll
		for (int o = 1; o < 64; o <<= 1) {
			unsigned u = __shfl_up(v, o, 64);
			if (lane >= o) v += u;
		}
		__syncthreads();
		if (lane == 63) s_wave[wid] = v;
		__syncthreads();
		unsigned before = v - c;
		for (int w = 0; w < wid; w++) before += s_wave[w];
		const unsigned all = s_wave[0] + s_wave[1] + s_wave[2] + s_wave[3];
		unsigned pos = running + before;
		while (m) {
			const int bit = __ffsll((long long)m) - 1;
			m &= m - 1;
			if (pos < cap) {
				DevKp k;
				k.x = xw * 64 + bit; k.y = y; k.z = z;
				k.octave = octave; k.level = level_id[lvl]; k.scale = scale[lvl]; k.code = 0; k.slot = -1;
#pragma unroll
				for (int j = 0; j < 3; j++) { k.win[j] = 0.f; k.eigvalue[j] = 0.f; }
#pragma unroll
				for (int j = 0; j < 9; j++) { k.eigvector[j] = 0.f; k.rot[j] = 0.f; k.st[j] = 0.f; }
				out[pos] = k;
			} else {
				total[1] = 1u;
			}
			pos++;
		}
		running += all;
	}
}

__global__ void __launch_bounds__(kThreads) k_emit(const unsigned long long *__restrict__ masks,
                                                   const unsigned *__restrict__ block_offsets, int nx, int ny, ZRange zr, int nyb,
                                                   int octave, DetectLevels L, DevKp *__restrict__ out, unsigned cap,
                                                   unsigned *__restrict__ total) {
	__shared__ unsigned s_wave[kThreads / 64];
	emit_block((int)blockIdx.x, masks, block_offsets, nx, ny, zr, nyb, octave, L.level_id, L.scale, out, cap, total, s_wave);
}

__global__ void __launch_bounds__(kThreads) k_emit_multi(EmitMulti M, DevKp *__restrict__ out, unsigned cap, unsigned *__restrict__ total) {
	__shared__ unsigned s_wave[kThreads / 64];
	int k = 0;
	while (k + 1 < M.n && blockIdx.x >= M.o[k + 1].block0) k++;
	const EmitOct &E = M.o[k];
	emit_block((int)(blockIdx.x - E.block0), E.masks, E.offsets, E.nx, E.ny, E.zr, E.nyb, E.octave, E.level_id, E.scale, out, cap, total, s_wave);
}

void launch_detect_mark(const DetectLevels &L, int nlevels, int nx, int ny, const ZRange &zr, float peak_thresh, int octave,
                        const DetectBufs &b, hipStream_t st, const Taps *lazy_taps, const DetectOpts *opt) {
	if (opt) { launch_mark_full(L, nlevels, nx, ny, zr, kRows, peak_thresh, *opt, b, st); return; }
	const int nyb = (ny + kRows - 1) / kRows;
	const int nzl = zr.zo1 - zr.zo0;
	if (nzl <= 0) return;
	const unsigned nblocks = (unsigned)(nlevels * nzl * nyb);
	if (nblocks == 0) return;
	const bool lazy = L.lazy_src != nullptr && lazy_taps != nullptr && b.prov != nullptr;
	if (lazy) (void)hipMemsetAsync(b.prov_count, 0, sizeof(unsigned), st);
	const size_t mask_lds = sizeof(unsigned long long) * (kThreads / 64) * (kRows / 4) * (size_t)std::min((nx + 63) >> 6, 64);
	hipLaunchKernelGGL(k_mark, dim3(nblocks), dim3(kThreads), mask_lds, st, L, nx, ny, zr, nyb, peak_thresh, b.masks, b.block_counts, b.prov,
	                   b.prov_count, b.prov_cap, b.total);
	if (lazy) {
		const bool wave_form = lazy_taps->hw == 8 && !hook(SIFT3D_HOOK_LAZY_GENERIC) && (size_t)nx * (size_t)ny * 17u * sizeof(float) < ((size_t)1 << 32);
		auto grid = [&](unsigned full, unsigned per_wg) { return dim3(std::max(1u, std::min(full, (nblocks + per_wg - 1) / per_wg))); };
		if (wave_form)
			hipLaunchKernelGGL(k_lazy_wave, grid(256 * 3, kLwWaves), dim3(64 * kLwWaves), 0, st, L, *lazy_taps, nx, ny, zr, nyb, b.prov, b.prov_count, b.prov_cap,
			                   b.masks, b.block_counts);
		if (2 * lazy_taps->hw + 1 <= 17)
			hipLaunchKernelGGL(k_lazy_next<17>, grid(wave_form ? 1536 : 1024, 1), dim3(256), 0, st, L, *lazy_taps, nx, ny, zr, nyb, b.prov, b.prov_count, b.prov_cap,
			                   b.masks, b.block_counts, wave_form ? 1 : 0);
		else
			hipLaunchKernelGGL(k_lazy_next<25>, grid(512, 1), dim3(256), 0, st, L, *lazy_taps, nx, ny, zr, nyb, b.prov, b.prov_count, b.prov_cap,
			                   b.masks, b.block_counts, 0);
	}
}

void launch_detect_emit(const DetectLevels &L, int nlevels, int nx, int ny, const ZRange &zr, int octave, const DetectBufs &b, DevKp *out,
                        unsigned cap, hipStream_t st) {
	const int nyb = (ny + kRows - 1) / kRows;
	const int nzl = zr.zo1 - zr.zo0;
	if (nzl <= 0) return;
	const unsigned nblocks = (unsigned)(nlevels * nzl * nyb);
	if (nblocks == 0) return;
	hipLaunchKernelGGL(k_scan, dim3(1), dim3(1024), 0, st, b.block_counts, b.block_offsets, nblocks, b.total);
	hipLaunchKernelGGL(k_emit, dim3(nblocks), dim3(kThreads), 0, st, b.masks, b.block_offsets, nx, ny, zr, nyb, octave, L, out, cap,
	                   b.total);
}

void launch_detect_emit_multi(const DetectEmitItem *items, int n, DevKp *out, unsigned cap, unsigned *total, hipStream_t st) {
	EmitMulti M;
	memset(&M, 0, sizeof(M));
	unsigned blocks = 0;
	for (int k = 0; k < n && M.n < 8; k++) {
		const DetectEmitItem &it = items[k];
		const int nyb = (it.ny + kRows - 1) / kRows, nzl = it.zr.zo1 - it.zr.zo0;
		if (nzl <= 0) continue;
		const unsigned nblocks = (unsigned)(it.nlevels * nzl * nyb);
		if (nblocks == 0) continue;
		EmitOct &E = M.o[M.n++];
		E.masks = it.b->masks; E.counts = it.b->block_counts; E.offsets = it.b->block_offsets;
		E.nx = it.nx; E.ny = it.ny; E.nyb = nyb; E.octave = it.octave; E.zr = it.zr; E.nblocks = nblocks; E.block0 = blocks;
		for (int l = 0; l < kMaxKpLevels; l++) { E.level_id[l] = it.L->level_id[l]; E.scale[l] = it.L->scale[l]; }
		blocks += nblocks;
	}
	if (M.n == 0) return;
	hipLaunchKernelGGL(k_scan_multi, dim3(1), dim3(1024), 0, st, M, total);
	hipLaunchKernelGGL(k_emit_multi, dim3(blocks), dim3(kThreads), 0, st, M, out, cap, total);
}

void launch_detect_octave(const DetectLevels &L, int nlevels, int nx, int ny, const ZRange &zr, float peak_thresh, int octave,
                          const DetectBufs &b, DevKp *out, unsigned cap, hipStream_t st, const Taps *lazy_taps) {
	launch_detect_mark(L, nlevels, nx, ny, zr, peak_thresh, octave, b, st, lazy_taps);
	launch_detect_emit(L, nlevels, nx, ny, zr, octave, b, out, cap, st);
}

void preload_detect_kernels() { hipFuncAttributes a; (void)hipFuncGetAttributes(&a, reinterpret_cast<const void *>(&k_scan)); }

}
```

### 3dsift_amd/csrc/kernels_march.hip

```cpp
#include <string.h>
#include <stdlib.h>
#include <algorithm>

#include "sift3d_internal.h"

namespace s3d {

constexpr int kMarchMaxHW = 8;
struct MTaps { float w[2 * kMarchMaxHW + 1]; };
struct MEdge { float f[3][kMarchMaxHW + 1]; };
typedef float mf4 __attribute__((ext_vector_type(4)));
typedef float mf2 __attribute__((ext_vector_type(2)));

template <int HW, int TX_ = 32>
struct MCfg {
	static constexpr int TX = TX_, TY = 32, NT = TX * 8, NW = NT / 64;
	static constexpr int SEG = TX / 8;
	static constexpr int RPW = 64 / SEG;
	static constexpr int HX = ((HW + 3) / 4) * 4;
	static constexpr int W = TX + 2 * HX, W4 = W / 4;
	static constexpr int ROWS = TY + 2 * HW;
	static constexpr int NITEMS = ROWS * W4;
	static constexpr int NWI = (NITEMS + 63) / 64;
	static constexpr int NDMA = (NWI + NW - 1) / NW;
// ... 172 lines not shown
		const bool emit = j >= 1 && p_loc >= zc0 && p_loc < zc1 && own;
		mf4 cen = {0.f, 0.f, 0.f, 0.f};
		if (DOG && !CR) {
			if (j >= 1) cen = cenb[(j & 1) * C::NT + tid];
			const int pn = min(max(p_loc - 1, 0), nz - 1);
			if (!(S3D_MDIAG & 1)) m_dma16(src + (size_t)sz * (size_t)pn, out_voff, lds_cen + (unsigned)(((j + 1) & 1) * C::NT * 16));
		}
		if (j + 1 < nsteps) issue_dma(j + 1);

		constexpr int KG = kMarchYG, NTAP = 2 * HW + 1;
		constexpr bool YPRE = HW <= 6;
		mf4 ypre[KG];
		if (YPRE) {
			const float *yc0 = xb + (buf ^ 1) * C::XB_F;
#pragma unroll
			for (int i = 0; i < KG; i++) if (!((S3D_MDIAG & 128) && i > 0)) ypre[i] = *reinterpret_cast<const mf4 *>(yc0 + ((i < NTAP && (i & 1)) ? ycol_o : ycol) + (i < NTAP ? 2 * HW - i : 0) * C::XP);
			__builtin_amdgcn_sched_barrier(0);
		}
		if (j < nsteps) {
			const int role = (wid + j) & (C::NW - 1);
			const bool xhelp = role == C::NR;
			const bool xact = xhelp ? act_h : (((amask >> role) & 1) != 0);
			const bool xmirror = !xhelp && (((mmask >> role) & 1) != 0);
			const int xseg = xhelp ? xseg_h : xseg_r;
			const int xbase_e = xhelp ? xbe_h : xbe_r + role * (C::RPW * C::W4 * 4), xbase_o = xhelp ? xbo_h : xbo_r + role * (C::RPW * C::W4 * 4);
			const int xout = xout_r + role * (C::RPW * C::XP);
			static_assert((C::XP & (C::XP - 1)) == 0 && (C::SEG - 1) * 8 + 4 < C::XP, "row index = offset / XP");
			const int xout_m = xout + 2 * C::XP * HW - 2 * (xout & ~(C::XP - 1));
			float o[8] = {0.f, 0.f, 0.f, 0.f, 0.f, 0.f, 0.f, 0.f};
			if (xact) {
				const float *tb = tile + buf * C::TILE_F;
				float win[C::WN4 * 4];
#pragma unroll
				for (int k = 0; k < C::WN4; k++) {
					if ((S3D_MDIAG & 256) && k > 0) { win[4 * k] = win[0]; win[4 * k + 1] = win[1]; win[4 * k + 2] = win[2]; win[4 * k + 3] = win[3]; continue; }
					const mf4 f = *reinterpret_cast<const mf4 *>(tb + ((k & 1) ? xbase_o : xbase_e) + 4 * k);
					win[4 * k] = f.x; win[4 * k + 1] = f.y; win[4 * k + 2] = f.z; win[4 * k + 3] = f.w;
				}
				if (left_f && xseg == 0) {
#pragma unroll
					for (int k = 1; k <= HW; k++) win[C::WOFF + HW - k] = win[C::WOFF + HW + k];
				}
				if (right_f && xseg == C::SEG - 1) {
					float e[HW + 1];
#pragma unroll
					for (int k = 0; k <= HW; k++) {
						const float f = s_ef[k];
						e[k] = (1.0f - f) * win[C::WOFF + HW + 6 - k] + f * win[C::WOFF + HW + 7 - k];
					}
#pragma unroll
					for (int k = 0; k <= HW; k++) win[C::WOFF + HW + 7 + k] = e[k];
				}
				if (HW == 8 && right_f && xseg == C::SEG - 2) {
					const float f = s_ef[0];
					win[C::WOFF + HW + 15] = (1.0f - f) * win[C::WOFF + HW + 14] + f * win[C::WOFF + HW + 15];
				}
#pragma unroll
				for (int d = -HW; d <= HW; d++) {
					if ((S3D_MDIAG & 16) && d != 0) continue;
#pragma unroll
					for (int jo = 0; jo < 8; jo++) o[jo] = o[jo] + t.w[d + HW] * win[C::WOFF + jo + HW - d];
				}
				if (!xhelp) {
					float *xo = xb + buf * C::XB_F;
					*reinterpret_cast<mf4 *>(xo + xout) = mf4{o[0], o[1], o[2], o[3]};
					*reinterpret_cast<mf4 *>(xo + xout + xhi_r) = mf4{o[4], o[5], o[6], o[7]};
					if (xmirror) {
						*reinterpret_cast<mf4 *>(xo + xout_m) = mf4{o[0], o[1], o[2], o[3]};
						*reinterpret_cast<mf4 *>(xo + xout_m + xhi_r) = mf4{o[4], o[5], o[6], o[7]};
					}
				}
			}
			if (bottom_f && xhelp) {
				float a[8];
#pragma unroll
				for (int jo = 0; jo < 8; jo++) a[jo] = __shfl_up(o[jo], C::SEG, 64);
				const int jr = lane / C::SEG;
				if (xact && jr >= 1) {
					const int k = HW + 1 - jr;
					const float f = s_ef[kMarchMaxHW + 1 + k];
					const int erow = C::TY - 1 + HW + k;
					const bool esw = C::XSW && (erow & 1);
					float *xe = xb + buf * C::XB_F + erow * C::XP + xseg * 8 + (esw ? 4 : 0);
					*reinterpret_cast<mf4 *>(xe) = mf4{(1.0f - f) * a[0] + f * o[0], (1.0f - f) * a[1] + f * o[1], (1.0f - f) * a[2] + f * o[2],
					                                   (1.0f - f) * a[3] + f * o[3]};
					*reinterpret_cast<mf4 *>(xe + (esw ? -4 : 4)) = mf4{(1.0f - f) * a[4] + f * o[4], (1.0f - f) * a[5] + f * o[5], (1.0f - f) * a[6] + f * o[6],
					                                       (1.0f - f) * a[7] + f * o[7]};
				}
			}
		}

		int nst = 0;
		if (j >= 1) {
			const float *yc = xb + (buf ^ 1) * C::XB_F;
			float v[4] = {0.f, 0.f, 0.f, 0.f};
			{
				mf4 cur[KG], nxt[KG];
#pragma unroll
				for (int i = 0; i < KG; i++) cur[i] = YPRE ? ypre[i] : *reinterpret_cast<const mf4 *>(yc + ((i < NTAP && (i & 1)) ? ycol_o : ycol) + (i < NTAP ? 2 * HW - i : 0) * C::XP);
#pragma unroll
				for (int g0 = 0; g0 < NTAP; g0 += KG) {
#pragma unroll
					for (int i = 0; i < KG; i++)
						if (g0 + KG + i < NTAP && !(S3D_MDIAG & 128)) nxt[i] = *reinterpret_cast<const mf4 *>(yc + (((g0 + KG + i) & 1) ? ycol_o : ycol) + (2 * HW - (g0 + KG + i)) * C::XP);
#pragma unroll
					for (int i = 0; i < KG; i++)
						if (g0 + i < NTAP && !((S3D_MDIAG & 32) && (g0 + i) % 4 != 0)) {
							const float tap = t.w[g0 + i];
							v[0] = v[0] + tap * cur[i].x; v[1] = v[1] + tap * cur[i].y; v[2] = v[2] + tap * cur[i].z; v[3] = v[3] + tap * cur[i].w;
						}
#pragma unroll
					for (int i = 0; i < KG; i++) cur[i] = nxt[i];
				}
			}
			if (e_out >= dim_end) {
				const float f = s_ef[2 * (kMarchMaxHW + 1) + min(e_out - dim_end, HW)];
#pragma unroll
				for (int c = 0; c < 4; c++) {
					const float xn = v[c];
					v[c] = (1.0f - f) * prevx[c] + f * xn;
					prevx[c] = xn;
				}
			}
			float out[4];
			if (ZSYM) {
				float m[HW + 1][4];
#pragma unroll
				for (int k = 0; k <= HW; k++)
#pragma unroll
					for (int c = 0; c < 4; c++) m[k][c] = t.w[k] * v[c];
#pragma unroll
				for (int c = 0; c < 4; c++) out[c] = A[2 * HW - 1][c] + m[0][c];
#pragma unroll
				for (int s = 2 * HW - 1; s >= 1; s--) {
#pragma unroll
					for (int c = 0; c < 4; c++) A[s][c] = A[s - 1][c] + m[s <= HW ? s : 2 * HW - s][c];
				}
#pragma unroll
				for (int c = 0; c < 4; c++) A[0][c] = 0.0f + m[0][c];
			} else {
#pragma unroll
			for (int c = 0; c < 4; c++) out[c] = A[2 * HW - 1][c] + t.w[2 * HW] * v[c];
#pragma unroll
			for (int s = 2 * HW - 1; s >= 1; s--) {
				if ((S3D_MDIAG & 64) && s != HW) continue;
#pragma unroll
				for (int c = 0; c < 4; c++) A[s][c] = A[s - 1][c] + t.w[s] * v[c];
			}
#pragma unroll
			for (int c = 0; c < 4; c++) A[0][c] = 0.0f + t.w[0] * v[c];
			}

			if (DOG && CR && !(S3D_MDIAG & 512)) cen = cring[(j % KL) * C::NT + tid];
			nst = __any(emit && !((S3D_MDIAG & 2) && out[0] != 12345.678f)) ? (DOG ? 2 : 1) : 0;
			if (half != nullptr && (p_loc & 1) == 0) {
				const int hy = (y0 + ty) >> 1, hx = (x0 + 4 * xq) >> 1, hz = p_loc >> 1;
				const bool hs = emit && ((y0 + ty) & 1) == 0 && hy < hny && hx < hnx && hz < hnz;
				if (__any(hs)) {
					nst += 1;
					if (hs) {
						const unsigned hoff = (unsigned)((hz * hny + hy) * hnx + hx) * 4u;
						if (hx + 1 < hnx) asm volatile("global_store_dwordx2 %0, %1, %2\n\ts_nop 1" ::"v"(hoff), "v"(mf2{out[0], out[2]}), "s"(half));
						else asm volatile("global_store_dword %0, %1, %2\n\ts_nop 1" ::"v"(hoff), "v"(out[0]), "s"(half));
					}
				}
			}
			if (emit && !((S3D_MDIAG & 2) && out[0] != 12345.678f)) {
				float *gb = dst + (size_t)sz * (size_t)p_loc;
				m_store16(gb, out_voff, mf4{out[0], out[1], out[2], out[3]});
				if (DOG) {
					float dg[4];
					dg[0] = (out[0] - cen.x) * (-1.0f); dg[1] = (out[1] - cen.y) * (-1.0f);
					dg[2] = (out[2] - cen.z) * (-1.0f); dg[3] = (out[3] - cen.w) * (-1.0f);
					m_store16(dog + (size_t)sz * (size_t)p_loc, out_voff, mf4{dg[0], dg[1], dg[2], dg[3]});
#pragma unroll
					for (int c = 0; c < 4; c++) mx = m_absmax(mx, dg[c]);
				}
			}
		}
		if (DOG && CR && j < nsteps && !(S3D_MDIAG & 512)) {
			const mf4 fresh = *reinterpret_cast<const mf4 *>(tile + buf * C::TILE_F + park_off);
			if (KR == 0) cring[(j % KL) * C::NT + tid] = fresh;
			else {
				cring[(j % KL) * C::NT + tid] = creg[KR - 1];
#pragma unroll
				for (int i = KR - 1; i >= 1; i--) creg[i] = creg[i - 1];
				creg[0] = fresh;
			}
		}

		if (S3D_MDIAG & 4) {}
		else if (nst == 3) m_wait_vmcnt<3>();
		else if (nst == 2) m_wait_vmcnt<2>();
		else if (nst == 1) m_wait_vmcnt<1>();
		else m_wait_vmcnt<0>();
		m_barrier();
	}

	if (DOG) {
#pragma unroll
		for (int o = 32; o > 0; o >>= 1) mx = fmaxf(mx, __shfl_xor(mx, o, 64));
		if (lane == 0) s_red[wid] = mx;
		__syncthreads();
		if (tid == 0) {
			float r = fmaxf(fmaxf(s_red[0], s_red[1]), fmaxf(s_red[2], s_red[3]));
			if (C::NW == 8) r = fmaxf(r, fmaxf(fmaxf(s_red[4], s_red[5]), fmaxf(s_red[6], s_red[7])));
			if (r > 0.0f) atomicMax(dogmax, __float_as_uint(r));
		}
	}
}

static void march_edge_fractions(int n, int hw, float *f) {
	const int dim_end = n - 1;
	for (int k = 0; k <= hw; k++) {
		const float c = (float)(dim_end + k);
		const float cc = (float)(2 * dim_end) - c - 0.1f;
		const int lo = (int)cc;
		f[k] = cc - (float)lo;
	}
}

template <int HW>
static void launch_march_hw(const float *src, float *dst, float *dog, unsigned *dogmax, int nx, int ny, const ZRange &zr, const Taps &tg,
                            hipStream_t st, int plan_slots, int prio, const MarchHalf &hf) {
	using C = MCfg<HW>;
	MTaps t;
	for (int i = 0; i < 2 * kMarchMaxHW + 1; i++) t.w[i] = i < 2 * HW + 1 ? tg.w[i] : 0.0f;
	const int nzo = zr.zo1 - zr.zo0;
	if (nzo <= 0) return;
	const int ntx = (nx + C::TX - 1) / C::TX, nty = (ny + C::TY - 1) / C::TY, ntiles = ntx * nty;
	constexpr bool kHasCR = HW <= kMarchCrMaxHW;
	const int ramp = 2 * HW + 1;
	const int sat = (dog && kHasCR) ? 3 : march_occ<HW, false>();
	auto plan = [&](int cap, int &cz_out) {
		if (plan_slots > 0) cap = std::min(cap, plan_slots);
		double best = 1e300;
		cz_out = nzo;
		for (int n = 1; n <= nzo && n <= 64; n++) {
			const int czn = (nzo + n - 1) / n, nch = (nzo + czn - 1) / czn;
			long left = (long)ntiles * nch;
			double cost = 0.0;
			while (left > 0) {
				const long r = std::min<long>(left, cap);
				cost += (double)(czn + ramp) * std::max(1.0, (double)r / (256.0 * sat));
				left -= r;
			}
			if (cost < best - 1e-9) { best = cost; cz_out = czn; }
		}
		return best;
	};
	constexpr int kOcc = march_occ<HW, false>();
	int cz3 = nzo, cz4 = nzo;
	const double cost3 = plan(256 * (dog && kHasCR ? 3 : kOcc), cz3), cost4 = plan(256 * (dog && kHasCR ? 4 : kOcc + 1), cz4);
	const bool small_bg = plan_slots > 0 && ntiles <= kMarchBgRinglessTiles;
	const bool use_cr = dog && kHasCR && !small_bg && !(cost4 * 1.12 < cost3);
	const int cz = (dog && kHasCR) ? (use_cr ? cz3 : cz4) : (cost4 < cost3 ? cz4 : cz3);
	const int nchunks = (nzo + cz - 1) / cz;
	MEdge ef;
	memset(&ef, 0, sizeof(ef));
	march_edge_fractions(nx, HW, ef.f[0]);
	march_edge_fractions(ny, HW, ef.f[1]);
	march_edge_fractions(zr.nzg, HW, ef.f[2]);
	const dim3 grid((unsigned)(ntiles * nchunks)), block(C::NT);
	if (dog && use_cr) hipLaunchKernelGGL((k_march_level<HW, true, kHasCR>), grid, block, 0, st, src, dst, dog, dogmax, nx, ny, zr, t, ef, ntx, nty, cz, prio, hf.d, hf.nx, hf.ny, hf.nz);
	else if (dog) hipLaunchKernelGGL((k_march_level<HW, true, false>), grid, block, 0, st, src, dst, dog, dogmax, nx, ny, zr, t, ef, ntx, nty, cz, prio, hf.d, hf.nx, hf.ny, hf.nz);
	else hipLaunchKernelGGL((k_march_level<HW, false, false>), grid, block, 0, st, src, dst, dog, dogmax, nx, ny, zr, t, ef, ntx, nty, cz, prio, hf.d, hf.nx, hf.ny, hf.nz);
}

static bool march_wide_ok(int nx, int ny, int nzo, int hw, int plan_slots) {
	const int mode = hook(SIFT3D_HOOK_MARCH_TILES);
	static const int wide_tail = dev_tune_i("S3D_WIDE_TAIL", 0);
	if (mode == 2 || (plan_slots > 0 && !(wide_tail && plan_slots >= 512)) || hw < 2 || hw > 6) return false;
	if (!(nx == 64 || nx >= 64 + ((hw + 3) / 4) * 4)) return false;
	const int ntiles = ((nx + 63) / 64) * ((ny + 31) / 32);
	return mode == 1 || (ntiles >= kMarchWideMinTiles && nzo / std::max(1, 512 / ntiles) >= 24);
}
template <int HW>
static void launch_march_wide(const float *src, float *dst, float *dog, unsigned *dogmax, int nx, int ny, const ZRange &zr, const Taps &tg,
                              hipStream_t st, int prio, const MarchHalf &hf) {
	using C = MCfg<HW, 64>;
	MTaps t;
	for (int i = 0; i < 2 * kMarchMaxHW + 1; i++) t.w[i] = i < 2 * HW + 1 ? tg.w[i] : 0.0f;
	const int nzo = zr.zo1 - zr.zo0;
	if (nzo <= 0) return;
	const int ntx = (nx + C::TX - 1) / C::TX, nty = (ny + C::TY - 1) / C::TY, ntiles = ntx * nty;
	const int ramp = 2 * HW + 1, cap = 512;
	int cz = nzo;
	{
		double best = 1e300;
		for (int n = 1; n <= nzo && n <= 64; n++) {
			const int czn = (nzo + n - 1) / n, nch = (nzo + czn - 1) / czn;
			long left = (long)ntiles * nch;
			double cost = 0.0;
			while (left > 0) {
				const long r = std::min<long>(left, cap);
				cost += (double)(czn + ramp) * std::max(1.0, (double)r / (double)cap);
				left -= r;
			}
			if (cost < best - 1e-9) { best = cost; cz = czn; }
		}
	}
	const int nchunks = (nzo + cz - 1) / cz;
	MEdge ef;
	memset(&ef, 0, sizeof(ef));
	march_edge_fractions(nx, HW, ef.f[0]);
	march_edge_fractions(ny, HW, ef.f[1]);
	march_edge_fractions(zr.nzg, HW, ef.f[2]);
	const dim3 grid((unsigned)(ntiles * nchunks)), block(C::NT);
	constexpr int kKR = HW == 4 ? 1 : (HW == 5 ? 3 : 0);
	if (!dog) hipLaunchKernelGGL((k_march_level<HW, false, false, 64, 0>), grid, block, 0, st, src, dst, dog, dogmax, nx, ny, zr, t, ef, ntx, nty, cz, prio, hf.d, hf.nx, hf.ny, hf.nz);
	else if (HW <= 5) hipLaunchKernelGGL((k_march_level<HW, true, (HW <= 5), 64, kKR>), grid, block, 0, st, src, dst, dog, dogmax, nx, ny, zr, t, ef, ntx, nty, cz, prio, hf.d, hf.nx, hf.ny, hf.nz);
	else hipLaunchKernelGGL((k_march_level<HW, true, false, 64, 0>), grid, block, 0, st, src, dst, dog, dogmax, nx, ny, zr, t, ef, ntx, nty, cz, prio, hf.d, hf.nx, hf.ny, hf.nz);
}

bool march_half_ok(int nx, int ny, const ZRange &zr) { return (nx & 3) == 0 && zr.zoff == 0 && zr.nz == zr.nzg; }

bool march_applicable(int nx, int ny, int nzg, const Taps &t) {
	const int hx = ((t.hw + 3) / 4) * 4;
	if (!(nx == 32 || nx >= 32 + hx) || !(ny == 32 || ny >= 32 + t.hw) || nzg < 2 * t.hw + 2) return false;
	if (!(t.hw >= 2 && t.hw <= kMarchMaxHW)) return false;
	for (int d = 1; d <= t.hw; d++) if (memcmp(&t.w[t.hw + d], &t.w[t.hw - d], sizeof(float)) != 0) return false;
	return true;
}

bool launch_march_level(const float *src, float *dst, float *dog, unsigned *dogmax, int nx, int ny, const ZRange &zr, const Taps &t,
                        hipStream_t st, int plan_slots, int prio, const MarchHalf *half) {
	MarchHalf hf;
	if (half && half->d && march_half_ok(nx, ny, zr)) hf = *half;
	else if (half && half->d) return false;
	if (!march_applicable(nx, ny, zr.nzg, t)) return false;
	if (march_wide_ok(nx, ny, zr.zo1 - zr.zo0, t.hw, plan_slots)) {
		switch (t.hw) {
		case 2: launch_march_wide<2>(src, dst, dog, dogmax, nx, ny, zr, t, st, prio, hf); return true;
		case 3: launch_march_wide<3>(src, dst, dog, dogmax, nx, ny, zr, t, st, prio, hf); return true;
		case 4: launch_march_wide<4>(src, dst, dog, dogmax, nx, ny, zr, t, st, prio, hf); return true;
		case 5: launch_march_wide<5>(src, dst, dog, dogmax, nx, ny, zr, t, st, prio, hf); return true;
		case 6: launch_march_wide<6>(src, dst, dog, dogmax, nx, ny, zr, t, st, prio, hf); return true;
		default: break;
		}
	}
	switch (t.hw) {
	case 2: launch_march_hw<2>(src, dst, dog, dogmax, nx, ny, zr, t, st, plan_slots, prio, hf); return true;
	case 3: launch_march_hw<3>(src, dst, dog, dogmax, nx, ny, zr, t, st, plan_slots, prio, hf); return true;
	case 4: launch_march_hw<4>(src, dst, dog, dogmax, nx, ny, zr, t, st, plan_slots, prio, hf); return true;
	case 5: launch_march_hw<5>(src, dst, dog, dogmax, nx, ny, zr, t, st, plan_slots, prio, hf); return true;
	case 6: launch_march_hw<6>(src, dst, dog, dogmax, nx, ny, zr, t, st, plan_slots, prio, hf); return true;
	case 7: launch_march_hw<7>(src, dst, dog, dogmax, nx, ny, zr, t, st, plan_slots, prio, hf); return true;
	case 8: launch_march_hw<8>(src, dst, dog, dogmax, nx, ny, zr, t, st, plan_slots, prio, hf); return true;
	default: return false;
	}
}

void preload_march_kernels() { hipFuncAttributes a; (void)hipFuncGetAttributes(&a, reinterpret_cast<const void *>(&k_march_level<2, false, false>)); }

}
```

### 3dsift_amd/csrc/sift3d_internal.h

```cpp
#pragma once

#include <hip/hip_runtime.h>
#include <stdint.h>

#include <string>
#include <vector>

#include "../../include/sift3d_hip.h"
#include "../../include/sift3d_hip_test.h"

#pragma clang fp contract(off)

namespace s3d {

#ifndef S3D_MAX_HW
#define S3D_MAX_HW 64
#endif
constexpr int kMaxHW = S3D_MAX_HW;
constexpr int kMaxTaps = 2 * kMaxHW + 1;
constexpr int kDesc = SIFT3D_DESC_NUMEL;
constexpr int kFaces = 20;

struct Taps {
	int hw;
	float w[kMaxTaps];
};

struct EdgeFrac {
	float f[3][kMaxHW + 1];
};

struct ZRange {
	int nz;
	int zoff;
	int nzg;
	int zo0, zo1;
};
inline ZRange whole(int nz) { return ZRange{nz, 0, nz, 0, nz}; }

struct Level {
	float *d = nullptr;
	int nx = 0, ny = 0, nz = 0;
	float unit = 1.f;
	float scale = 0.f;
	int bz = 0;
	int zoff = 0;
	int planes() const { return bz ? bz : nz; }
	size_t n() const { return (size_t)nx * ny * planes(); }
	ZRange zr(int zo0, int zo1) const { return ZRange{planes(), zoff, nz, zo0, zo1}; }
	ZRange zr_all() const { return ZRange{planes(), zoff, nz, 0, planes()}; }
};

struct DevKp {
	int x, y, z;
	int octave, level;
	float scale;
	int code;
	int slot;
	float win[3];
	float eigvalue[3];
	float eigvector[9];
	float rot[9];
	float st[9];
};

struct FaceConst {
	float e1[3], e2[3], t[3], q[3];
	float qe2;
	int idx[3];
	float centre[3];
};

struct WinLut {
	int off;
	int len;
	int nin;
	float radius;
	float sigma;
	float fix_scale;
	float wsum;
	int list_off, list_R;
};
constexpr int kMaxDescLut = 1536;

struct FaceSym {
	int face[32];
	int vert[32][3];
	int slot[32][3];
};

void launch_absmax(const float *src, size_t n, unsigned *d_max_bits, hipStream_t st, unsigned *d_nonfinite = nullptr);
void launch_scale_by_max(float *data, size_t n, const unsigned *d_max_bits, hipStream_t st);
void launch_dog_from_gss(const float *hi, const float *lo, float *dog, size_t n, hipStream_t st);
void launch_conv_axis(int axis, const float *src, float *dst, int nx, int ny, int nz, const Taps &t,
                      const float *prev, float *dog, unsigned *d_dogmax, hipStream_t st, bool exact = false);
struct MarchHalf { float *d = nullptr; int nx = 0, ny = 0, nz = 0; };
bool march_half_ok(int nx, int ny, const ZRange &zr);
bool march_applicable(int nx, int ny, int nzg, const Taps &t);
bool launch_march_level(const float *src, float *dst, float *dog, unsigned *dogmax, int nx, int ny, const ZRange &zr, const Taps &t,
                        hipStream_t st, int plan_slots = 0, int prio = 0, const MarchHalf *half = nullptr);
void launch_copy16(const float *src, float *dst, size_t nfloats, hipStream_t st);
constexpr int kCopySegs = 32, kMaxMergePtrs = 16;
struct CopySegs { const float *src[kCopySegs]; float *dst[kCopySegs]; size_t floats[kCopySegs]; int n = 0; };
struct MaxMerge { const float *in[kMaxMergePtrs]; float *out[kMaxMergePtrs]; int nin = 0, nout = 0, n = 0; };
void launch_copy_segments(const CopySegs &a, hipStream_t st);
void launch_max_merge(const MaxMerge &a, hipStream_t st);
constexpr int kSmallMaxOct = 4, kSmallMaxLv = 8;
struct SmallOct { float *g[kSmallMaxLv]; float *dog[kSmallMaxLv]; int nx, ny, nz; };
struct SmallArgs {
	SmallOct oct[kSmallMaxOct];
	int noct, ng, nd, seed;
	unsigned build_mask, dog_mask;
	unsigned *dogmax;
	int hwp;
	float w[kSmallMaxLv][9];
	const float *parent;
	int pnx, pny;
};
bool small_octave_fits(int nx, int ny, int nz, int max_hw);
int small_padded_hw(int max_hw);
void launch_small_octaves(const SmallArgs &a, hipStream_t st);
void launch_downsample(const float *src, int snx, int sny, float *dst, int nx, int ny, int nz, hipStream_t st);

struct DetectBufs {
	unsigned long long *masks;
	unsigned *block_counts;
	unsigned *block_offsets;
	unsigned *total;
	unsigned *prov = nullptr;
	unsigned *prov_count = nullptr;
	unsigned prov_cap = 0;
};
constexpr int kMaxKpLevels = 5;
struct DetectLevels {
	const float *cur[kMaxKpLevels], *prev[kMaxKpLevels], *next[kMaxKpLevels];
	const float *prev0_hi, *prev0_lo;
	const float *nextl_hi, *nextl_lo;
	int nextl_slot;
	const float *lazy_src;
	const unsigned *absmax_bits[kMaxKpLevels];
	int level_id[kMaxKpLevels];
	float scale[kMaxKpLevels];
};
constexpr int kLazySlots = 52;
struct DetectOpts {
	int neighbours = 8, refine = 0;
	float max_offset = 0.5f, contrast_thresh = 0.0f, edge_ratio = 0.0f;
};
void launch_detect_mark(const DetectLevels &L, int nlevels, int nx, int ny, const ZRange &zr, float peak_thresh, int octave,
                        const DetectBufs &b, hipStream_t st, const Taps *lazy_taps, const DetectOpts *opt = nullptr);
void launch_mark_full(const DetectLevels &L, int nlevels, int nx, int ny, const ZRange &zr, int rows, float peak_thresh, const DetectOpts &opt,
                      const DetectBufs &b, hipStream_t st);
constexpr int kDogTabOct = 12, kDogTabLv = 8;
struct DogTable {
	const float *d[kDogTabOct][kDogTabLv];
	int nx[kDogTabOct], ny[kDogTabOct];
	int octave_base;
};
void launch_detect_emit(const DetectLevels &L, int nlevels, int nx, int ny, const ZRange &zr, int octave, const DetectBufs &b, DevKp *out,
                        unsigned cap, hipStream_t st);
struct DetectEmitItem { const DetectLevels *L; int nlevels, nx, ny; ZRange zr; int octave; const DetectBufs *b; };
void launch_detect_emit_multi(const DetectEmitItem *items, int n, DevKp *out, unsigned cap, unsigned *total, hipStream_t st);
void launch_detect_octave(const DetectLevels &L, int nlevels, int nx, int ny, const ZRange &zr, float peak_thresh, int octave,
                          const DetectBufs &b, DevKp *out, unsigned cap, hipStream_t st, const Taps *lazy_taps = nullptr);

#ifdef __HIPCC__
typedef const float __attribute__((address_space(1))) *gfloat_p;
__device__ __forceinline__ gfloat_p as_global(const float *p) { return (gfloat_p)p; }
#endif

struct LevelRef {
	const float *d;
	int nx, ny, nz;
	float unit;
	int zoff;
};
void launch_orient(DevKp *kps, int *codes, const unsigned *d_count, unsigned cap, const LevelRef *d_levels ,
                   const WinLut *d_luts, const float *d_lutpool, float max_eig, float corner, int part_rank, int part_world,
                   int *redo_list , unsigned *redo_count,
                   hipStream_t st);
constexpr int kOrientWords = 34;
void launch_orient_pack(const DevKp *kps, const unsigned *d_count, unsigned cap, int *dst, int part_rank, int part_world, hipStream_t st);
void launch_orient_unpack(DevKp *kps, int *codes, const unsigned *d_count, unsigned cap, const int *src, hipStream_t st);
size_t slots_scratch_words();
void launch_slots(DevKp *kps, const int *codes, const unsigned *d_count, unsigned cap, unsigned *d_nkp, int *order, unsigned kp_cap,
                  unsigned *scratch, hipStream_t st);

hipError_t upload_faces(const FaceConst *faces, const FaceSym *sym);
struct DescSplit {
	int *gacc = nullptr;
	float *gmass = nullptr;
	unsigned *gdone = nullptr;
	unsigned cap = 0;
};
constexpr int kDescSegs = 6;
struct DescSeg {
	const DevKp *recs = nullptr;
	const float *units = nullptr;
	int *hist = nullptr;
	float *mass = nullptr;
	unsigned first = 0, n = 0;
	int o0 = 0, o1 = 0;
};
struct DescPartial {
	int zc0 = 0, zc1 = 0, nseg = 0;
	int H[8] = {0, 0, 0, 0, 0, 0, 0, 0};
	DescSeg seg[kDescSegs];
};
void launch_export_records(const DevKp *ext, const int *order, unsigned n, DevKp *dst, hipStream_t st);
void launch_describe_partial(const LevelRef *d_levels, const WinLut *d_luts, const float *d_lutpool, const DescPartial &pp,
                             unsigned *d_work , hipStream_t st, bool lut_in_lds = true);
void launch_describe_finish(const DevKp *recs, unsigned n, const LevelRef *d_levels, const WinLut *d_luts, int nparts, const int *const *d_hist, const float *const *d_mass,
                            const float *d_units, bool final_round, float *d_desc, int *d_redo, float *d_units_next, unsigned *d_counters,
                            hipStream_t st);
void launch_describe(const DevKp *kps, const unsigned *d_count, unsigned cap, const LevelRef *d_levels,
                     const WinLut *d_luts, const float *d_lutpool, float *d_desc, unsigned kp_cap, int part_rank, int part_world,
                     const int *order, const unsigned *d_nkp, unsigned *d_work ,
                     hipStream_t st, bool lut_in_lds = true, const DescSplit *split = nullptr);
void launch_face_lookup(const float *d_g3, int n, int route, int *d_face, float *d_bary3, hipStream_t st);
void launch_refine(const DevKp *kps, const unsigned *d_count, unsigned cap, unsigned kp_cap, const DogTable &T, int num_kp_levels,
                   sift3d_refined *out, hipStream_t st);
void launch_finalize(const DevKp *kps, const unsigned *d_count, unsigned cap, int transposed,
                     sift3d_keypoint *d_out, float *d_xyz, unsigned kp_cap, hipStream_t st);

struct MatchGuard {
	float *s4; const float *a_n2; const unsigned *b_n2max; int *redo;
	bool small_offsets = false;
};
int match_rows_device(const float *d_a, const int *d_row_ids, int nrows, const float *d_b, int m, int *d_cand ,
                      void *d_part, float *d_gd, float *d_sd, int *d_gi, int *d_si, const MatchGuard &g, hipStream_t st);
int match_redo_rows();
void launch_describe_overflow(const DevKp *kps, unsigned k, const LevelRef *d_levels, const WinLut *d_luts, const float *d_lutpool, float *d_desc,
                              hipStream_t st);
int onekp_second_passes();

uint32_t ransac_seed(uint32_t seed);
void launch_ransac_global(const float *d_pairs, int n, int H, uint32_t s, double tau2, double min_det, int refine, double *d_hyp, int *d_count,
                          sift3d_affine_fit *d_out, unsigned char *d_mask, hipStream_t st);
void launch_ransac_local(const float *d_pairs, int n, const float *d_pts, int m, int k, float r2, int H, uint32_t s, double tau2, double min_det,
                         int refine, sift3d_affine_fit *d_out, int *d_nbrs, hipStream_t st);
void launch_ransac_score(const float *d_pairs, int n, int H, const double *d_hyp, double tau2, int *d_count, hipStream_t st);

void launch_rigid_global(const float *d_pairs, int n, int H, uint32_t s, double tau2, double min_det, int model, int refine, double *d_hyp,
                         int *d_count, sift3d_affine_fit *d_out, unsigned char *d_mask, hipStream_t st);
void launch_rigid_local(const float *d_pairs, int n, const float *d_pts, int m, int k, float r2, int H, uint32_t s, double tau2, double min_det,
                        int model, int refine, sift3d_affine_fit *d_out, int *d_nbrs, hipStream_t st);

struct IcgnVol {
	const float *d;
	int nx, ny, nz;
};
size_t icgn_state_bytes();
void launch_icgn(IcgnVol R, IcgnVol T, const int *d_pts, int m, const double *d_init, int r, int max_it, double tol, int kind, void *d_state,
                 sift3d_icgn_result *d_out, hipStream_t st);
struct IcgnMask {
	const unsigned char *act;
	int *n;
	float min_fraction;
};
void launch_icgn_masked(IcgnVol R, IcgnVol T, const int *d_pts, int m, const double *d_init, int r, int max_it, double tol, int kind, void *d_state,
                        sift3d_icgn_result *d_out, IcgnMask M, hipStream_t st);

void launch_mask_active(const unsigned char *d_mask, int nx, int ny, int nz, unsigned char *d_act, hipStream_t st);
void launch_mask_threshold(const float *d_vol, size_t n, double level, unsigned char *d_mask, hipStream_t st);

size_t icgn2_state_bytes();
void launch_icgn2(IcgnVol R, IcgnVol T, const int *d_pts, int m, const double *d_init, int r, int max_it, double tol, int kind, void *d_state,
                  sift3d_icgn2_result *d_out, hipStream_t st);

bool bspline_prefilter_fits(int nx, int ny, int nz);
void launch_bspline_prefilter(const float *d_src, int nx, int ny, int nz, float *d_dst, float *d_tmp, hipStream_t st);

int search_groups(int m);
size_t search_score_bytes(int m, int s);
void launch_zncc_search(IcgnVol R, IcgnVol T, const int *d_pts, int m, const int *d_guess, int r, int s, double *d_scores,
                        sift3d_search_result *d_out, hipStream_t st);

struct SubsetParams {
	int r_min, r_max, criterion;
	double threshold, level, fraction_min;
};
void launch_subset_quality(IcgnVol R, const int *d_pts, int m, SubsetParams P, sift3d_subset_result *d_out, hipStream_t st);

struct PoiIndex;

void launch_strain_fit(const int *d_pts, const double *d_disp, int m, const PoiIndex &ix, int radius, int min_nb, int measure,
                       sift3d_strain_result *d_out, hipStream_t st);

struct ValidateParams {
	int radius, min_nb;
	double threshold, eps;
};
// ... 43 lines not shown
```

Baseline: 19950.

## Skip storing interior DoG levels; detect extrema directly from Gaussian pairs

When every Gaussian level of an octave goes through the fused march kernel, the march kernel now computes only the DoG absmax and no longer writes the interior DoG volumes. A new detection kernel (k_mark_g) rebuilds DoG values on the fly by subtracting adjacent Gaussian levels with 16-byte loads. Any DoG level that is later read is rebuilt on demand, and if the march kernel declines a level the stored path is used instead. This removes the DoG write traffic and the matching reads, at the cost of reading two Gaussian volumes per level during detection, plus extra fallback logic.

```diff
diff --git a/3dsift_amd/capi.py b/3dsift_amd/capi.py
--- a/3dsift_amd/capi.py
+++ b/3dsift_amd/capi.py
@@ -58,12 +58,12 @@
     "sift3d_seed_buffer", "sift3d_sharded_plan", "sift3d_slab_describe_launch", "sift3d_sharded_traffic",
     "sift3d_sharded_create", "sift3d_sharded_create_ex", "sift3d_sharded_run", "sift3d_sharded_num_keypoints", "sift3d_sharded_get_keypoints", "sift3d_sharded_info",
     "sift3d_sharded_error", "sift3d_sharded_destroy",
-    "sift3d_test_hook", "sift3d_debug_counters", "sift3d_debug_face_lookup", "sift3d_match_times", "sift3d_debug_copy_bandwidth",
+    "sift3d_test_hook", "sift3d_debug_counters", "sift3d_test_dog_unstored", "sift3d_debug_face_lookup", "sift3d_match_times", "sift3d_debug_copy_bandwidth",
     "sift3d_match_warmup", "sift3d_test_staging_slice", "sift3d_test_slab_plan", "sift3d_test_sharded_time_rank",
 ]
 HOOKS = {"dog_eager": 0, "glast_eager": 1, "det_serial": 2, "separable": 3, "desc_nocache": 4, "match_nodma": 5, "one_stream": 6,
          "desc_mass_shift": 7, "list_cap": 8, "peer_copy": 9, "desc_nosplit": 10, "march_tiles": 11, "desc_exact_cells": 12, "lazy_generic": 13, "sharded_fail_rank": 14,
-         "ori_grid": 15}
+         "ori_grid": 15, "dog_stored": 16}
 ORIENT_WORDS = 34
 DTYPES = {"float32": 0, "uint8": 1, "int8": 2, "uint16": 3, "int16": 4}
 SHARDED_PARTIAL_WINDOWS = 1
@@ -331,6 +331,8 @@
         L.sift3d_sharded_plan.argtypes = [C.c_void_p, _ip, _ip, _ip, _ip]
         L.sift3d_test_hook.argtypes = [C.c_int, C.c_int]
         L.sift3d_debug_counters.argtypes = [C.c_void_p, _ip]
+        if hasattr(L, "sift3d_test_dog_unstored"):
+            L.sift3d_test_dog_unstored.argtypes = [C.c_void_p, C.POINTER(C.c_uint)]
         L.sift3d_debug_face_lookup.argtypes = [_fp, C.c_int, C.c_int, _ip, _fp, C.c_int]
         L.sift3d_debug_copy_bandwidth.argtypes = [C.c_size_t, C.c_int, C.c_int, C.POINTER(C.c_double)]
         L.sift3d_match_times.argtypes = [C.POINTER(C.c_double), C.POINTER(C.c_double)]
@@ -1157,6 +1159,11 @@
         _check(lib().sift3d_debug_counters(self._h, a))
         return {"list_regrows": a[0], "desc_second_passes": a[1], "match_exact_rows": a[2]}
 
+    def dog_unstored_octaves(self):
+        m = C.c_uint(0)
+        _check(lib().sift3d_test_dog_unstored(self._h, C.byref(m)))
+        return [o for o in range(32) if (m.value >> o) & 1]
+
 
 def _params(kw):
     return Params(kw.get("num_kp_levels", 3), kw.get("sigma_default", 1.6), kw.get("sigma_n_default", 1.15),
diff --git a/3dsift_amd/csrc/context.hip b/3dsift_amd/csrc/context.hip
--- a/3dsift_amd/csrc/context.hip
+++ b/3dsift_amd/csrc/context.hip
@@ -461,8 +461,16 @@
 #ifndef S3D_BG_SLOTS_DEFAULT
 #define S3D_BG_SLOTS_DEFAULT 256
 #endif
+static int fused_min_dim() {
+	static const int fused_min = dev_tune_i("S3D_FUSED_MIN", S3D_FUSED_MIN_DEFAULT);
+	return fused_min;
+}
+static bool level_marches(const sift3d_ctx *c, const Level &dst, const Taps &t) {
+	return c->use_fused && std::min(dst.nx, dst.ny) >= fused_min_dim() && march_applicable(dst.nx, dst.ny, dst.zr_all().nzg, t);
+}
 static bool smooth_level(sift3d_ctx *c, int o, const float *src, const Level &dst, const Taps &t, const float *prev, float *dog,
-                         unsigned *dogmax, int level = 0, const Level *half_out = nullptr, hipStream_t st_override = nullptr) {
+                         unsigned *dogmax, int level = 0, const Level *half_out = nullptr, hipStream_t st_override = nullptr,
+                         bool dog_max_only = false, bool *declined = nullptr) {
 	hipStream_t st = st_override ? st_override : c->ostream[o];
 	static const int tail_slots = dev_tune_i("S3D_O0_TAIL_SLOTS", S3D_O0_TAIL_SLOTS_DEFAULT);
 	static const int bg_slots = dev_tune_i("S3D_BG_SLOTS", S3D_BG_SLOTS_DEFAULT);
@@ -470,14 +478,15 @@
 	static const int bg1_slots = dev_tune_i("S3D_BG1_SLOTS", 0);
 	const int prio = (prio_mode && c->noct > 1) ? (o >= 2 ? 2 : (o == 1 ? (prio_mode == 1 ? 1 : (prio_mode == 3 ? 2 : 0)) : 0)) : 0;
 	const int plan_slots = c->noct > 1 ? (o == 0 ? (level > c->p.num_kp_levels ? tail_slots : 0) : (o == 1 && bg1_slots > 0 ? bg1_slots : bg_slots)) : 0;
-	static const int fused_min = dev_tune_i("S3D_FUSED_MIN", S3D_FUSED_MIN_DEFAULT);
+	const int fused_min = fused_min_dim();
 	if (c->use_fused && (prev == nullptr || prev == src) && std::min(dst.nx, dst.ny) >= fused_min) {
 		MarchHalf hf;
 		const bool want_half = S3D_FUSED_HALF && half_out != nullptr && march_half_ok(dst.nx, dst.ny, dst.zr_all());
 		if (want_half) { hf.d = half_out->d; hf.nx = half_out->nx; hf.ny = half_out->ny; hf.nz = half_out->nz; }
-		if (launch_march_level(src, dst.d, dog, dogmax, dst.nx, dst.ny, dst.zr_all(), t, st, plan_slots, prio, want_half ? &hf : nullptr))
+		if (launch_march_level(src, dst.d, dog_max_only ? nullptr : dog, dogmax, dst.nx, dst.ny, dst.zr_all(), t, st, plan_slots, prio, want_half ? &hf : nullptr))
 			return want_half;
 	}
+	if (dog_max_only && declined) *declined = true;
 	launch_conv_axis(0, src, c->tmpA[o], dst.nx, dst.ny, dst.nz, t, nullptr, nullptr, nullptr, st, c->nonfinite);
 	launch_conv_axis(1, c->tmpA[o], c->tmpB[o], dst.nx, dst.ny, dst.nz, t, nullptr, nullptr, nullptr, st, c->nonfinite);
 	launch_conv_axis(2, c->tmpB[o], dst.d, dst.nx, dst.ny, dst.nz, t, prev, dog, dogmax, st, c->nonfinite);
@@ -499,6 +508,11 @@
 		DL.nextl_hi = G[c->nd].d; DL.nextl_lo = G[c->nd - 1].d;
 		DL.nextl_slot = nl - 1;
 		if (c->g_last_elide) { DL.nextl_hi = nullptr; DL.lazy_src = DL.nextl_lo; }
+	}
+	if ((size_t)o < c->oct_gpairs.size() && c->oct_gpairs[(size_t)o]) {
+		DL.gpairs = 1;
+		for (int k = 0; k <= nl; k++) DL.g[k] = G[k + 1].d;
+		DL.park_val = D[nl].d;
 	}
 }
 
@@ -584,6 +598,15 @@
 				}
 			}
 		}
+		c->oct_gpairs.assign((size_t)std::max(1, c->noct), 0);
+		if (c->dog_elide && !c->run_full && !c->slab && !c->seeded && (c->nd - 2 == 2 || c->nd - 2 == 3) && !hook(SIFT3D_HOOK_DOG_STORED))
+			for (int o = 0; o < c->noct && (small_first < 0 || o < small_first); o++) {
+				bool all = true;
+				for (int i = 1; i < c->ng && all; i++)
+					if (!(c->g_last_elide && i == c->ng - 1)) all = level_marches(c, c->gss[(size_t)o * c->ng + i], c->taps[i]);
+				c->oct_gpairs[(size_t)o] = all ? 1 : 0;
+			}
+		std::vector<char> gp_declined((size_t)c->noct + 1, 0);
 		auto enqueue = [&](int o, bool head) -> int {
 			static const int chain_mode = dev_tune_i("S3D_CHAIN", 1);
 			const bool chain_on = chain_mode != 0;
@@ -633,10 +656,22 @@
 					const Level *half = (i == c->p.num_kp_levels && o + 1 < c->noct) ? &c->gss[(size_t)(o + 1) * c->ng] : nullptr;
 					bool hw_ = false;
 					if (c->dog_elide && (i - 1 == 0 || i - 1 == c->nd - 1)) hw_ = smooth_level(c, o, P.d, L, c->taps[i], nullptr, nullptr, nullptr, i, half, so);
-					else hw_ = smooth_level(c, o, P.d, L, c->taps[i], P.d, D.d, c->d_dogmax + (size_t)o * c->nd + i - 1, i, half, so);
+					else {
+						bool declined = false;
+						hw_ = smooth_level(c, o, P.d, L, c->taps[i], P.d, D.d, c->d_dogmax + (size_t)o * c->nd + i - 1, i, half, so, c->oct_gpairs[(size_t)o] != 0, &declined);
+						if (declined) gp_declined[(size_t)o] |= (char)(1 << (i - 1));
+					}
 					if (half) half_written[(size_t)o + 1] = hw_ ? 1 : 0;
 				}
 				if (i == c->p.num_kp_levels) S3D_HIP(hipEventRecord(c->ev_seed[o], so));
+			}
+			if (!head && c->oct_gpairs[(size_t)o] && gp_declined[(size_t)o]) {
+				for (int j = 1; j <= c->nd - 2; j++)
+					if (!((gp_declined[(size_t)o] >> j) & 1)) {
+						const Level &D = c->dog[(size_t)o * c->nd + j];
+						launch_dog_from_gss(c->gss[(size_t)o * c->ng + j + 1].d, c->gss[(size_t)o * c->ng + j].d, D.d, D.n(), so);
+					}
+				c->oct_gpairs[(size_t)o] = 0;
 			}
 			if (!head && o > 0) S3D_HIP(hipEventRecord(c->ev_done[o], so));
 			return SIFT3D_OK;
@@ -967,7 +1002,8 @@
 			c->g_last_built[(size_t)o] = 1;
 		}
 	}
-	if (is_dog && c->dog_elide && (idx % c->nd == 0 || idx % c->nd == c->nd - 1)) {
+	const bool oct_unstored = is_dog && !c->slab && (size_t)(idx / c->nd) < c->oct_gpairs.size() && c->oct_gpairs[(size_t)(idx / c->nd)] != 0;
+	if (is_dog && ((c->dog_elide && (idx % c->nd == 0 || idx % c->nd == c->nd - 1)) || oct_unstored)) {
 		const int o = idx / c->nd, i = idx % c->nd;
 		launch_dog_from_gss(c->gss[(size_t)o * c->ng + i + 1].d, c->gss[(size_t)o * c->ng + i].d, L->d, L->n(), c->stream);
 		S3D_HIP(hipStreamSynchronize(c->stream));
diff --git a/3dsift_amd/csrc/ctx_internal.h b/3dsift_amd/csrc/ctx_internal.h
--- a/3dsift_amd/csrc/ctx_internal.h
+++ b/3dsift_amd/csrc/ctx_internal.h
@@ -23,6 +23,7 @@
 	bool dog_elide = false;
 	bool g_last_elide = false;
 	std::vector<char> g_last_built;
+	std::vector<char> oct_gpairs;
 	unsigned *d_prov = nullptr;
 	bool desc_lut_lds = true;
 	bool ext_arena = false;
diff --git a/3dsift_amd/csrc/kernels_detect.hip b/3dsift_amd/csrc/kernels_detect.hip
--- a/3dsift_amd/csrc/kernels_detect.hip
+++ b/3dsift_amd/csrc/kernels_detect.hip
@@ -221,6 +221,197 @@
 	if (threadIdx.x == 0) block_counts[b] = s_cnt[0] + s_cnt[1] + s_cnt[2] + s_cnt[3];
 }
 
+constexpr int kGBatch = 4;
+__device__ __forceinline__ float g_max3(float a, float b, float c) { float r; asm("v_max3_f32 %0, %1, %2, %3" : "=v"(r) : "v"(a), "v"(b), "v"(c)); return r; }
+__device__ __forceinline__ float g_min3(float a, float b, float c) { float r; asm("v_min3_f32 %0, %1, %2, %3" : "=v"(r) : "v"(a), "v"(b), "v"(c)); return r; }
+typedef float gf4 __attribute__((ext_vector_type(4), aligned(4)));
+template <int NL>
+__global__ void __launch_bounds__(kThreads) k_mark_g(DetectLevels L, int nx, int ny, ZRange zr, int nyb, float peak_thresh,
+                                                     unsigned long long *__restrict__ masks, unsigned *__restrict__ block_counts,
+                                                     unsigned *__restrict__ prov, unsigned *__restrict__ prov_count, unsigned prov_cap,
+                                                     unsigned *__restrict__ total) {
+	constexpr int KB = kGBatch, RW = kRows / 4;
+	constexpr int kQ = 64 + KB * 64;
+	static_assert(NL >= 2 && NL <= 3 && NL <= kMaxKpLevels, "two bits for the level slot; the first and the last slot differ");
+	static_assert(KB == 4, "a lane holds the four voxels of one 16-byte load");
+	__shared__ unsigned s_cnt[NL][kThreads / 64];
+	__shared__ uint2 s_q[kThreads / 64][kQ];
+	extern __shared__ unsigned long long s_mask_dyn[];
+	const int segw = min((nx + 63) >> 6, 64);
+	const int b = blockIdx.x;
+	const int nz = zr.zo1 - zr.zo0;
+	const int yb = b % nyb, zi = b / nyb;
+	const int z = zr.zo0 + zi, zg = z + zr.zoff;
+	const bool lazy_g = L.lazy_src != nullptr;
+	float thr[NL];
+#pragma unroll
+	for (int l = 0; l < NL; l++) thr[l] = peak_thresh * __uint_as_float(*L.absmax_bits[l]);
+	const int wpr = (nx + 63) >> 6;
+	const int lane = threadIdx.x & 63, wid = threadIdx.x >> 6;
+	const size_t sy = (size_t)nx, sz = (size_t)nx * ny;
+	const bool z_in = (zg >= 1 && zg <= zr.nzg - 2);
+	const int y0 = yb * kRows;
+	const int nrows = min(kRows, ny - y0);
+	const int swid = __builtin_amdgcn_readfirstlane(wid);
+	const int r_lo = swid * RW, r_hi = min(nrows, (swid + 1) * RW);
+	uint2 *q = s_q[swid];
+	unsigned long long *mloc = s_mask_dyn + (size_t)swid * NL * RW * segw;
+	for (int i = lane; i < NL * RW * segw; i += 64) mloc[i] = 0ull;
+	const unsigned long long lt = (1ull << lane) - 1ull;
+	const size_t plane0 = sz * (size_t)z + sy * (size_t)y0;
+	int qn = 0;
+	unsigned cnt[NL];
+#pragma unroll
+	for (int l = 0; l < NL; l++) cnt[l] = 0;
+	for (int seg0 = 0; seg0 < wpr; seg0 += 64) {
+		const int seg1 = min(wpr, seg0 + 64);
+		auto evaluate = [&](int first, int n) {
+			const bool in_q = lane < n;
+			const uint2 qe = q[first + (in_q ? lane : 0)];
+			const float v = __uint_as_float(qe.x);
+			const unsigned id = qe.y;
+			const int l = (int)((id >> 17) & 3), rr = (int)((id >> 12) & 15), xw = (int)((id >> 6) & 63), bit = (int)(id & 63);
+			const bool dmax = (id >> 16) & 1u;
+			const int xq = (seg0 + xw) * 64 + bit;
+			const bool act = in_q && xq >= 1 && xq <= nx - 2;
+			const size_t i = plane0 + sy * (size_t)(r_lo + rr) + (size_t)xq;
+			const size_t ic = act ? i : sz * (size_t)z + sy + 1;
+			const float *glo = L.g[0], *ghi = L.g[1];
+#pragma unroll
+			for (int k = 1; k < NL; k++)
+				if (l == k) { glo = L.g[k]; ghi = L.g[k + 1]; }
+			if (S3D_DETDIAG & 1) return;
+			const float n5 = (ghi[ic + sz] - glo[ic + sz]) * (-1.0f);
+			bool ok = dmax ? v > n5 : v < n5;
+			if (ok) {
+				const float n6 = (ghi[ic - sz] - glo[ic - sz]) * (-1.0f);
+				ok = ok && (dmax ? v > n6 : v < n6);
+			}
+			const bool last = l == NL - 1;
+			if (l == 0 && (ok)) {
+				const float n0 = (L.prev0_hi[ic] - L.prev0_lo[ic]) * (-1.0f);
+				ok = ok && (dmax ? v > n0 : v < n0);
+			}
+			if (last && !lazy_g && (ok)) {
+				const float n7 = (L.nextl_hi[ic] - L.nextl_lo[ic]) * (-1.0f);
+				ok = ok && (dmax ? v > n7 : v < n7);
+			}
+			if (lazy_g) {
+				const bool park = act && ok && last;
+				const unsigned long long pm = __ballot(park);
+				if (pm) {
+					unsigned base = 0;
+					if (lane == 0) base = atomicAdd(prov_count, (unsigned)__popcll(pm));
+					base = (unsigned)__builtin_amdgcn_readfirstlane((int)base);
+					if (park) {
+						const unsigned slot = base + (unsigned)__popcll(pm & lt);
+						L.park_val[i] = v;
+						if (slot < prov_cap) prov[slot] = (unsigned)i | (dmax ? 0x80000000u : 0u);
+						else total[1] = 1u;
+					}
+				}
+				if (last) return;
+			}
+			if (act && ok) atomicOr(&mloc[(l * RW + rr) * segw + xw], 1ull << bit);
+		};
+		if (z_in) {
+			const int ry_a = max(r_lo, 1 - y0), ry_b = min(r_hi, ny - 1 - y0);
+			const int nws = seg1 - seg0;
+			const size_t pbase = sz * (size_t)z + (size_t)seg0 * 64;
+			const float *eb = L.g[NL];
+#pragma unroll
+			for (int k = 0; k < NL; k++)
+				if ((lane >> 1) == k) eb = L.g[k];
+			eb += pbase;
+			auto word = [&](int l, float sv, float hi, float lo, unsigned idv) {
+				const int gmax = (int)(sv < lo), gmin = (int)(sv > hi);
+				const bool c = ((int)(fabsf(sv) > thr[l]) & (gmax | gmin)) != 0;
+				const unsigned long long m = __builtin_amdgcn_ballot_w64(c);
+				if (c) {
+					const unsigned pos = __builtin_amdgcn_mbcnt_hi((unsigned)(m >> 32), __builtin_amdgcn_mbcnt_lo((unsigned)m, (unsigned)qn));
+					q[pos] = make_uint2(__float_as_uint(sv * (-1.0f)), idv | ((unsigned)l << 17) | (gmax ? 0x10000u : 0u));
+				}
+				qn += (int)__popcll(m);
+			};
+			const int omax = nx - 1 - seg0 * 64;
+			for (int w0 = 0; w0 < nws && ry_a < ry_b; w0 += KB) {
+				const int x0 = w0 * 64 + 4 * lane;
+				const unsigned off = (unsigned)min(x0, omax);
+				const int eoff = (lane & 1) ? min((w0 + KB) * 64, omax) : w0 * 64 - 1;
+				auto load_row = [&](int row, float (&dv)[NL][KB], float &ed, bool edge) {
+					const size_t ro = pbase + sy * (size_t)(y0 + row);
+					gf4 gv[NL + 1];
+#pragma unroll
+					for (int k = 0; k <= NL; k++) gv[k] = *reinterpret_cast<const gf4 *>(L.g[k] + ro + off);
+					float ge = 0.0f;
+					if (edge) ge = (eb + sy * (size_t)(y0 + row))[eoff];
+#pragma unroll
+					for (int l = 0; l < NL; l++) {
+						dv[l][0] = gv[l + 1].x - gv[l].x; dv[l][1] = gv[l + 1].y - gv[l].y;
+						dv[l][2] = gv[l + 1].z - gv[l].z; dv[l][3] = gv[l + 1].w - gv[l].w;
+					}
+					if (edge) ed = __shfl_down(ge, 2, 64) - ge;
+				};
+				float up[NL][KB], mid[NL][KB], emid = 0.0f, enone = 0.0f;
+				load_row(ry_a - 1, up, enone, false);
+				load_row(ry_a, mid, emid, true);
+				for (int ry = ry_a; ry < ry_b; ry++) {
+					float dn[NL][KB], edn = 0.0f;
+					load_row(ry + 1, dn, edn, true);
+					const unsigned idrow = (unsigned)((ry - r_lo) << 12) | (unsigned)x0;
+#pragma unroll
+					for (int l = 0; l < NL; l++) {
+						const int le = __builtin_amdgcn_readlane(__float_as_int(emid), 2 * l), re = __builtin_amdgcn_readlane(__float_as_int(emid), 2 * l + 1);
+						const float xlo = __int_as_float(__builtin_amdgcn_update_dpp(le, __float_as_int(mid[l][KB - 1]), 0x138 , 0xf, 0xf, false));
+						const float xhi = __int_as_float(__builtin_amdgcn_update_dpp(re, __float_as_int(mid[l][0]), 0x130 , 0xf, 0xf, false));
+#pragma unroll
+						for (int cc = 0; cc < KB; cc++) {
+							const float xl = cc > 0 ? mid[l][cc > 0 ? cc - 1 : 0] : xlo, xr = cc < KB - 1 ? mid[l][cc < KB - 1 ? cc + 1 : 0] : xhi;
+							const float sa = l > 0 ? mid[l > 0 ? l - 1 : 0][cc] : mid[l < NL - 1 ? l + 1 : 0][cc];
+							float hi = g_max3(g_max3(up[l][cc], dn[l][cc], xl), xr, sa), lo = g_min3(g_min3(up[l][cc], dn[l][cc], xl), xr, sa);
+							if (l > 0 && l < NL - 1) { hi = g_max3(hi, mid[l < NL - 1 ? l + 1 : 0][cc], hi); lo = g_min3(lo, mid[l < NL - 1 ? l + 1 : 0][cc], lo); }
+							word(l, mid[l][cc], hi, lo, idrow + (unsigned)cc);
+						}
+						while (qn >= 64) {
+							qn -= 64;
+							evaluate(qn, 64);
+						}
+					}
+#pragma unroll
+					for (int l = 0; l < NL; l++)
+#pragma unroll
+						for (int cc = 0; cc < KB; cc++) { up[l][cc] = mid[l][cc]; mid[l][cc] = dn[l][cc]; }
+					emid = edn;
+				}
+			}
+		}
+		if (qn > 0) evaluate(0, qn);
+		qn = 0;
+#pragma unroll
+		for (int l = 0; l < NL; l++)
+			for (int ry = r_lo; ry < r_hi; ry++) {
+				unsigned long long *mrow = masks + ((size_t)(l * nz + zi) * ny + (y0 + ry)) * wpr;
+				for (int xw = seg0 + lane; xw < seg1; xw += 64) {
+					const unsigned long long m = mloc[(l * RW + ry - r_lo) * segw + xw - seg0];
+					mrow[xw] = m;
+					cnt[l] += (unsigned)__popcll(m);
+					mloc[(l * RW + ry - r_lo) * segw + xw - seg0] = 0ull;
+				}
+			}
+	}
+#pragma unroll
+	for (int l = 0; l < NL; l++) {
+#pragma unroll
+		for (int o = 32; o > 0; o >>= 1) cnt[l] += __shfl_xor(cnt[l], o, 64);
+		if (lane == 0) s_cnt[l][wid] = cnt[l];
+	}
+	__syncthreads();
+	if (threadIdx.x < NL) {
+		const int l = (int)threadIdx.x;
+		block_counts[(l * nz + zi) * nyb + yb] = s_cnt[l][0] + s_cnt[l][1] + s_cnt[l][2] + s_cnt[l][3];
+	}
+}
+
 __device__ __forceinline__ void lazy_tap_src(int p, int d, int n, int &lo, int &hi, float &frac, bool interior) {
 	if (interior) { lo = hi = p - d; frac = 0.0f; return; }
 	const int dim_end = n - 1;
@@ -611,8 +802,15 @@
 	const bool lazy = L.lazy_src != nullptr && lazy_taps != nullptr && b.prov != nullptr;
 	if (lazy) (void)hipMemsetAsync(b.prov_count, 0, sizeof(unsigned), st);
 	const size_t mask_lds = sizeof(unsigned long long) * (kThreads / 64) * (kRows / 4) * (size_t)std::min((nx + 63) >> 6, 64);
-	hipLaunchKernelGGL(k_mark, dim3(nblocks), dim3(kThreads), mask_lds, st, L, nx, ny, zr, nyb, peak_thresh, b.masks, b.block_counts, b.prov,
-	                   b.prov_count, b.prov_cap, b.total);
+	if (L.gpairs && nlevels == 2)
+		hipLaunchKernelGGL(k_mark_g<2>, dim3((unsigned)(nzl * nyb)), dim3(kThreads), 2 * mask_lds, st, L, nx, ny, zr, nyb, peak_thresh, b.masks, b.block_counts,
+		                   b.prov, b.prov_count, b.prov_cap, b.total);
+	else if (L.gpairs && nlevels == 3)
+		hipLaunchKernelGGL(k_mark_g<3>, dim3((unsigned)(nzl * nyb)), dim3(kThreads), 3 * mask_lds, st, L, nx, ny, zr, nyb, peak_thresh, b.masks, b.block_counts,
+		                   b.prov, b.prov_count, b.prov_cap, b.total);
+	else
+		hipLaunchKernelGGL(k_mark, dim3(nblocks), dim3(kThreads), mask_lds, st, L, nx, ny, zr, nyb, peak_thresh, b.masks, b.block_counts, b.prov,
+		                   b.prov_count, b.prov_cap, b.total);
 	if (lazy) {
 		const bool wave_form = lazy_taps->hw == 8 && !hook(SIFT3D_HOOK_LAZY_GENERIC) && (size_t)nx * (size_t)ny * 17u * sizeof(float) < ((size_t)1 << 32);
 		auto grid = [&](unsigned full, unsigned per_wg) { return dim3(std::max(1u, std::min(full, (nblocks + per_wg - 1) / per_wg))); };
diff --git a/3dsift_amd/csrc/kernels_march.hip b/3dsift_amd/csrc/kernels_march.hip
--- a/3dsift_amd/csrc/kernels_march.hip
+++ b/3dsift_amd/csrc/kernels_march.hip
@@ -348,7 +348,7 @@
 			}
 
 			if (DOG && CR && !(S3D_MDIAG & 512)) cen = cring[(j % KL) * C::NT + tid];
-			nst = __any(emit && !((S3D_MDIAG & 2) && out[0] != 12345.678f)) ? (DOG ? 2 : 1) : 0;
+			nst = __any(emit && !((S3D_MDIAG & 2) && out[0] != 12345.678f)) ? ((DOG && dog != nullptr) ? 2 : 1) : 0;
 			if (half != nullptr && (p_loc & 1) == 0) {
 				const int hy = (y0 + ty) >> 1, hx = (x0 + 4 * xq) >> 1, hz = p_loc >> 1;
 				const bool hs = emit && ((y0 + ty) & 1) == 0 && hy < hny && hx < hnx && hz < hnz;
@@ -368,7 +368,7 @@
 					float dg[4];
 					dg[0] = (out[0] - cen.x) * (-1.0f); dg[1] = (out[1] - cen.y) * (-1.0f);
 					dg[2] = (out[2] - cen.z) * (-1.0f); dg[3] = (out[3] - cen.w) * (-1.0f);
-					m_store16(dog + (size_t)sz * (size_t)p_loc, out_voff, mf4{dg[0], dg[1], dg[2], dg[3]});
+					if (dog != nullptr) m_store16(dog + (size_t)sz * (size_t)p_loc, out_voff, mf4{dg[0], dg[1], dg[2], dg[3]});
 #pragma unroll
 					for (int c = 0; c < 4; c++) mx = m_absmax(mx, dg[c]);
 				}
@@ -417,7 +417,7 @@
 }
 
 template <int HW>
-static void launch_march_hw(const float *src, float *dst, float *dog, unsigned *dogmax, int nx, int ny, const ZRange &zr, const Taps &tg,
+static void launch_march_hw(const float *src, float *dst, float *dog_st, unsigned *dogmax, int nx, int ny, const ZRange &zr, const Taps &tg,
                             hipStream_t st, int plan_slots, int prio, const MarchHalf &hf) {
 	using C = MCfg<HW>;
 	MTaps t;
@@ -425,6 +425,8 @@
 	const int nzo = zr.zo1 - zr.zo0;
 	if (nzo <= 0) return;
 	const int ntx = (nx + C::TX - 1) / C::TX, nty = (ny + C::TY - 1) / C::TY, ntiles = ntx * nty;
+	float *const dog_out = dog_st;
+	const bool dog = dog_st != nullptr || dogmax != nullptr;
 	constexpr bool kHasCR = HW <= kMarchCrMaxHW;
 	const int ramp = 2 * HW + 1;
 	const int sat = (dog && kHasCR) ? 3 : march_occ<HW, false>();
@@ -458,9 +460,9 @@
 	march_edge_fractions(ny, HW, ef.f[1]);
 	march_edge_fractions(zr.nzg, HW, ef.f[2]);
 	const dim3 grid((unsigned)(ntiles * nchunks)), block(C::NT);
-	if (dog && use_cr) hipLaunchKernelGGL((k_march_level<HW, true, kHasCR>), grid, block, 0, st, src, dst, dog, dogmax, nx, ny, zr, t, ef, ntx, nty, cz, prio, hf.d, hf.nx, hf.ny, hf.nz);
-	else if (dog) hipLaunchKernelGGL((k_march_level<HW, true, false>), grid, block, 0, st, src, dst, dog, dogmax, nx, ny, zr, t, ef, ntx, nty, cz, prio, hf.d, hf.nx, hf.ny, hf.nz);
-	else hipLaunchKernelGGL((k_march_level<HW, false, false>), grid, block, 0, st, src, dst, dog, dogmax, nx, ny, zr, t, ef, ntx, nty, cz, prio, hf.d, hf.nx, hf.ny, hf.nz);
+	if (dog && use_cr) hipLaunchKernelGGL((k_march_level<HW, true, kHasCR>), grid, block, 0, st, src, dst, dog_out, dogmax, nx, ny, zr, t, ef, ntx, nty, cz, prio, hf.d, hf.nx, hf.ny, hf.nz);
+	else if (dog) hipLaunchKernelGGL((k_march_level<HW, true, false>), grid, block, 0, st, src, dst, dog_out, dogmax, nx, ny, zr, t, ef, ntx, nty, cz, prio, hf.d, hf.nx, hf.ny, hf.nz);
+	else hipLaunchKernelGGL((k_march_level<HW, false, false>), grid, block, 0, st, src, dst, dog_out, dogmax, nx, ny, zr, t, ef, ntx, nty, cz, prio, hf.d, hf.nx, hf.ny, hf.nz);
 }
 
 static bool march_wide_ok(int nx, int ny, int nzo, int hw, int plan_slots) {
@@ -472,13 +474,14 @@
 	return mode == 1 || (ntiles >= kMarchWideMinTiles && nzo / std::max(1, 512 / ntiles) >= 24);
 }
 template <int HW>
-static void launch_march_wide(const float *src, float *dst, float *dog, unsigned *dogmax, int nx, int ny, const ZRange &zr, const Taps &tg,
+static void launch_march_wide(const float *src, float *dst, float *dog_st, unsigned *dogmax, int nx, int ny, const ZRange &zr, const Taps &tg,
                               hipStream_t st, int prio, const MarchHalf &hf) {
 	using C = MCfg<HW, 64>;
 	MTaps t;
 	for (int i = 0; i < 2 * kMarchMaxHW + 1; i++) t.w[i] = i < 2 * HW + 1 ? tg.w[i] : 0.0f;
 	const int nzo = zr.zo1 - zr.zo0;
 	if (nzo <= 0) return;
+	const bool dog = dog_st != nullptr || dogmax != nullptr;
 	const int ntx = (nx + C::TX - 1) / C::TX, nty = (ny + C::TY - 1) / C::TY, ntiles = ntx * nty;
 	const int ramp = 2 * HW + 1, cap = 512;
 	int cz = nzo;
@@ -504,9 +507,9 @@
 	march_edge_fractions(zr.nzg, HW, ef.f[2]);
 	const dim3 grid((unsigned)(ntiles * nchunks)), block(C::NT);
 	constexpr int kKR = HW == 4 ? 1 : (HW == 5 ? 3 : 0);
-	if (!dog) hipLaunchKernelGGL((k_march_level<HW, false, false, 64, 0>), grid, block, 0, st, src, dst, dog, dogmax, nx, ny, zr, t, ef, ntx, nty, cz, prio, hf.d, hf.nx, hf.ny, hf.nz);
-	else if (HW <= 5) hipLaunchKernelGGL((k_march_level<HW, true, (HW <= 5), 64, kKR>), grid, block, 0, st, src, dst, dog, dogmax, nx, ny, zr, t, ef, ntx, nty, cz, prio, hf.d, hf.nx, hf.ny, hf.nz);
-	else hipLaunchKernelGGL((k_march_level<HW, true, false, 64, 0>), grid, block, 0, st, src, dst, dog, dogmax, nx, ny, zr, t, ef, ntx, nty, cz, prio, hf.d, hf.nx, hf.ny, hf.nz);
+	if (!dog) hipLaunchKernelGGL((k_march_level<HW, false, false, 64, 0>), grid, block, 0, st, src, dst, dog_st, dogmax, nx, ny, zr, t, ef, ntx, nty, cz, prio, hf.d, hf.nx, hf.ny, hf.nz);
+	else if (HW <= 5) hipLaunchKernelGGL((k_march_level<HW, true, (HW <= 5), 64, kKR>), grid, block, 0, st, src, dst, dog_st, dogmax, nx, ny, zr, t, ef, ntx, nty, cz, prio, hf.d, hf.nx, hf.ny, hf.nz);
+	else hipLaunchKernelGGL((k_march_level<HW, true, false, 64, 0>), grid, block, 0, st, src, dst, dog_st, dogmax, nx, ny, zr, t, ef, ntx, nty, cz, prio, hf.d, hf.nx, hf.ny, hf.nz);
 }
 
 bool march_half_ok(int nx, int ny, const ZRange &zr) { return (nx & 3) == 0 && zr.zoff == 0 && zr.nz == zr.nzg; }
diff --git a/3dsift_amd/csrc/sift3d_internal.h b/3dsift_amd/csrc/sift3d_internal.h
--- a/3dsift_amd/csrc/sift3d_internal.h
+++ b/3dsift_amd/csrc/sift3d_internal.h
@@ -138,6 +138,9 @@
 	const float *nextl_hi, *nextl_lo;
 	int nextl_slot;
 	const float *lazy_src;
+	int gpairs;
+	const float *g[kMaxKpLevels + 1];
+	float *park_val;
 	const unsigned *absmax_bits[kMaxKpLevels];
 	int level_id[kMaxKpLevels];
 	float scale[kMaxKpLevels];
```

After: 19700. 0.987x the previous value.
